# fujii-team/Henbun

Measured on AMD Instinct MI355X. Metric: elbo_samples_per_sec, higher is better.
Workload: dtype f32; 1 GPU; cfg2 SVGP ELBO step: 1-D UnitRBF, N=1e6, M=512 inducing, minibatch 8192 per GPU, diag Normal q(u), diagonal residual, Adam lr 1e-3; global_batch=8192, per_gpu_batch=8192, parallelism=dp1, N=1000000, M=512, dp_exchange=none, dp_ranks=1, contraction=native, tri_pack=False

## Files before the change

### henbun_amd/_lib.py

```python
from __future__ import annotations

import ctypes
import os
from ctypes import c_char_p, c_double, c_int, c_long, c_uint64, c_void_p

_HERE = os.path.dirname(os.path.abspath(__file__))
LIB_PATH = os.path.join(_HERE, "libhenbun_hip.so")


class HipBackendError(RuntimeError):
    """A libhenbun_hip.so entry point returned a non-zero status."""


P, L, I, D, U64 = c_void_p, c_long, c_int, c_double, c_uint64

_SIGS = {
    "hb_version": [],
    "hb_debug_set": [c_char_p, L],
    "hb_debug_clear": [],
    "hb_cholesky_inverse_ws_elems": [L, L, I],
    "hb_cholesky_persistent_shape": [L, L, I],
    "hb_mlp2_sample_supported": [L, L, L, L, L, I],
    "hb_mlp2_sample_ws_elems": [L, L, L],
    "hb_mlp2_sample_fwd_f32": [P, P, P, P, P, I, P, P, L, P, P, P, P, L, L, L, P, P],
    "hb_mlp2_sample_bwd_f32": [P, P, P, P, I, P, P, P, P, P, P, P, P, P, L, L, L, P, P],
    "hb_gram_cholesky_inverse_f32": [I, P, L, P, L, L, L, D, P, P, L, L, P, P, P, I, P],
    "hb_last_error_string": [],
    "hb_device_info": [P, I, P],
    "hb_graph_begin_capture": [P],
    "hb_graph_end_capture": [P, P],
    "hb_graph_launch": [P, P],
    "hb_graph_destroy": [P],
    "hb_rng_init": [P, L, U64, U64, P],
    "hb_rng_randint": [P, L, P, L, L, L, P],
    "hb_sgp_ws_elems": [L, L, L, L, L],
    "hb_sgp_strip_path": [L, L, L, L, L, I],
    "hb_sgp_head_units": [L, L, L, L, L, I, I, I, L],
    "hb_sgp_rider_supported": [L, L, L, L, L, I, I, I, L],
    "hb_sgp_predict_ws_elems": [L, L, L, L, L, I, I, I],
    "hb_sgp_predict_cov_ws_elems": [L, L, L, L, I, I],
    "hb_matmul_gauss_units": [L, L, L],
    "hb_matmul_gram_vjp_ok": [L, L, L, L],
    "hb_matmul_gram_vjp_ws_elems": [L, L, L],
    "hb_matmul_gram_vjp_f32": [P, P, P, L, L, L, L, L, L, L, L, L, I, I, P, L, P, L, L, L, P, P, P, P, P],
    "hb_fullrank_one_launch_shape": [L, L],
    "hb_matmul_gauss_f32": [P, L, P, L, P, P, P, P, D, P, P, P, L, L, L, L, P],
    "hb_sgp_rider_begin": [],
    "hb_sgp_rider_pending": [],
    "hb_sgp_rider_flush": [P],
    "hb_sgp_fwd_gauss_f32": [I, I, P, L, P, P, L, P, P, I, P, P, P, L, P, P, P, P, P, L, L, L, L, L, P, P, P, P, D, P, P, P, L, P],
    "hb_ewise_prog_image_bytes": [],
    "hb_ewise_prog_build": [I, P, P, I, P, P, I, P, P, P, I, P, P, P, P],
    "hb_ewise_jit_available": [],
    "hb_ewise_jit_run": [P, P],
    "hb_ewise_jit_destroy": [P],
    "hb_side_push_gather_draw_f32": [I, P, P, P, L, P, L, L, L, P, P, L, P, P],
    "hb_side_push_diag_fwd_f32": [P, P, P, P, L, P, P, P, L, L, L, L, P, P],
    "hb_side_push_diag_bwd_f32": [P, P, P, P, P, P, P, L, L, L, L, P],
    "hb_side_pending": [],
    "hb_side_flush": [P],
    "hb_side_discard": [],
    "hb_chain_begin": [],
    "hb_chain_end": [P],
    "hb_chain_discard": [],
    "hb_chain_source": [P, L],
    "hb_chain_compile_dry": [],
    "hb_comm_available": [],
    "hb_comm_unique_id": [P],
    "hb_comm_init": [P, I, I, P],
    "hb_comm_destroy": [P],
}
_RESTYPES = {"hb_last_error_string": c_char_p, "hb_sgp_ws_elems": c_long, "hb_ewise_prog_image_bytes": c_long,
             "hb_sgp_head_units": c_long, "hb_matmul_gauss_units": c_long, "hb_matmul_gram_vjp_ws_elems": c_long, "hb_cholesky_inverse_ws_elems": c_long, "hb_mlp2_sample_ws_elems": c_long,
             "hb_sgp_predict_ws_elems": c_long, "hb_sgp_predict_cov_ws_elems": c_long}

_TYPED = {
    "hb_ewise": [I, I, P, P, I, P, I, P, P, P],
    "hb_ewise_prog": [I, P, P, I, P, P, I, P, P, P, I, P, P],
    "hb_ewise_prog_run": [P, L, I, P],
    "hb_ewise_jit_build": [I, P, P, I, P, P, I, P, P, P, I, P, P, P, P, P, L],
    "hb_ewise_colprog_build": [I, P, P, I, P, P, I, P, P, P, L, L, P, P, L],
    "hb_gauss_ll": [P, P, P, P, L, P, P, P, P, P, L, P],
    "hb_gauss_ll_post": [P, P, P, P, L, P, P, P, P, D, P, P, L, P],
    "hb_gauss_ll_fold": [P, L, P, P, P, P],
    "hb_reduce": [I, P, P, L, L, L, P, L, P],
    "hb_copy_nd": [P, P, P, P, I, P, P],
    "hb_fill": [P, L, D, P],
    "hb_gather_rows": [P, L, L, P, P, L, P, P, P],
    "hb_gather_rows_multi": [I, P, P, P, L, P, P, L, P, P],
    "hb_gather_rows_multi_draw": [I, P, P, P, L, P, L, L, L, P, P, L, P, P],
    "hb_matutil": [P, P, L, L, L, I, L, L, D, P],
    "hb_rng_normal": [P, L, P, L, P],
    "hb_diag_sample_kl_fwd": [P, P, P, P, L, P, P, P, L, L, L, L, P, P],
    "hb_diag_sample_kl_bwd": [P, P, P, P, P, P, P, L, L, L, L, P],
    "hb_fullrank_sample_kl_fwd": [P, P, P, P, L, P, P, P, L, L, I, P, P],
    "hb_fullrank_sample_kl_fwd1": [P, P, P, P, L, P, P, P, L, L, I, P, P, P],
    "hb_fullrank_sample_kl_bwd": [P, P, P, P, P, P, P, L, L, I, P],
    "hb_vec_to_tri": [P, P, L, L, P],
    "hb_tri_to_vec": [P, P, L, L, P],
    "hb_gram_fwd": [I, P, L, P, L, P, L, L, P, L, L, L, L, D, P],
    "hb_gram_bwd": [I, P, L, P, L, P, L, L, P, P, P, P, L, L, L, L, P, P],
    "hb_gram_ell_fold": [P, L, L, L, L, P, P],
    "hb_matmul": [P, P, P, L, L, L, L, L, L, L, L, L, L, I, I, D, D, P, L, I, I, P, L, P],
    "hb_matmul_colsum": [P, P, P, P, L, L, L, L, L, L, P, L, P],
    "hb_cholesky": [P, P, L, L, P, P],
    "hb_cholesky_inverse": [P, P, P, L, L, P, P, P, I, P],
    "hb_trinv": [P, P, L, L, P, P],
    "hb_sgp_A": [I, P, L, P, P, L, P, P, I, P, L, L, L, L, P],
    "hb_sgp_fwd": [I, I, P, L, P, P, L, P, P, I, P, P, P, L, P, P, P, P, P, L, L, L, L, L, P, P],
    "hb_sgp_bwd": [I, I, P, L, P, P, L, P, P, I, P, P, P, P, P, P, P, P, P, P, P, P, P, L, L, L, L, L, P, P],
    "hb_sgp_predict": [I, P, L, P, P, L, P, P, P, P, I, I, D, P, P, L, L, L, L, L, P, P],
    "hb_sgp_predict_cov": [I, P, L, P, P, L, P, P, P, I, I, D, P, L, L, L, L, L, P, P],
    "hb_adam_step": [P, P, P, P, L, D, D, D, D, D, P, I, P, L, P, P, P],
    "hb_allreduce_sum": [P, L, P, P],
    "hb_dp_pack": [P, P, P, L, P],
}


def declared_symbols():
    names = list(_SIGS)
    for base in _TYPED:
        names += [base + "_f32", base + "_f64"]
    return names


class _Lib:
    def __init__(self, path: str):
        if not os.path.exists(path):
            raise ImportError(
                "henbun_amd: %s is missing.  Build it with `python -m henbun_amd._build` "
                "(hipcc, gfx950).  There is no CPU fallback." % path
            )
        import torch

        self._dll = ctypes.CDLL(path)
        self._fns = {}
        for name, args in _SIGS.items():
            self._bind(name, args, _RESTYPES.get(name, c_int))
        for base, args in _TYPED.items():
            for suf in ("_f32", "_f64"):
                self._bind(base + suf, args, c_int)
        if self.raw("hb_version")() != 2:
            raise ImportError("henbun_amd: ABI version mismatch in " + path)

    def _bind(self, name, args, restype):
        fn = getattr(self._dll, name)
        fn.argtypes = args
        fn.restype = restype
        self._fns[name] = fn

    def raw(self, name):
        return self._fns[name]

    def last_error(self) -> str:
        s = self._fns["hb_last_error_string"]()
        return s.decode() if s else ""

    def call(self, name, *args):
        rc = self._fns[name](*args)
        if rc != 0:
            raise HipBackendError("%s failed (status %d): %s" % (name, rc, self.last_error()))
        return 0


_lib = None


def lib() -> _Lib:
    global _lib
    if _lib is None:
        _lib = _Lib(LIB_PATH)
    return _lib
```

### henbun_amd/csrc/sgp.hip

```cpp
#include "common.cuh"
#include "sgp_strip.cuh"
#include "chain.cuh"
#include "chol_persist.cuh"
#include <type_traits>
#include "gemm_tile.cuh"
#include "rng_pairs.cuh"
#include "../../include/henbun_hip.h"

#define SGP_BM 64
#define SGP_BN 128
#define SGP_DREG 4

extern "C" int hb_matmul_f32(const float*, const float*, float*, long, long, long, long, long, long, long, long, long,
                             long, int, int, double, double, const float*, long, int, int, float*, long, void*);
extern "C" int hb_matmul_f64(const double*, const double*, double*, long, long, long, long, long, long, long, long,
                             long, long, int, int, double, double, const double*, long, int, int, double*, long,
                             void*);

template <typename T>
struct SgpArgs {
  const T* x;
  long sx;
  const T* z;
  const T* ell;
// ... 540 lines not shown
    const int c = tid & 31, kq = tid >> 5;
    const int cc = col0 + c < n ? col0 + c : n - 1;
    float sc[D], xs[D];
#pragma unroll
    for (int dd = 0; dd < D; ++dd) {
      sc[dd] = float(SGP_EXP2_SCALE) / ell[a.dl == 1 ? 0 : dd];
      xs[dd] = x[cc * D + dd];
    }
    constexpr int NTH = SGP_STRIP_THREADS;
    constexpr int ZIT = (SGP_SM_MAX * D) / NTH, UIT = SGP_SM_MAX / NTH;
    float zt[ZIT], ut[4][UIT];
    const int npu = a.part ? ((int)a.P < 4 ? (int)a.P : 4) : 0;
#pragma unroll
    for (int it = 0; it < ZIT; ++it) {
      const int i = tid + NTH * it;
      zt[it] = z[i < M * D ? i : 0];
    }
#pragma unroll
    for (int p = 0; p < 4; ++p)
#pragma unroll
      for (int it = 0; it < UIT; ++it) {
        const int i = tid + NTH * it;
        ut[p][it] = p < npu ? a.u[e * a.P * a.M + (long)p * M + (i < M ? i : 0)] : 0.f;
      }
#pragma unroll
    for (int it = 0; it < ZIT; ++it) {
      const int i = tid + NTH * it;
      if (i < M * D) zs[i] = zt[it];
    }
#pragma unroll
    for (int p = 0; p < 4; ++p)
#pragma unroll
      for (int it = 0; it < UIT; ++it) {
        const int i = tid + NTH * it;
        if (p < npu && i < M) us[p][i] = ut[p][it];
      }
    __syncthreads();
#pragma unroll 4
    for (int k4 = kq * 4; k4 < M; k4 += NTH / 8) {
      float zq[4 * D];
#pragma unroll
      for (int q = 0; q < 4 * D; q += 4) {
        const V4 zz = *reinterpret_cast<const V4*>(&zs[k4 * D + q]);
#pragma unroll
        for (int s = 0; s < 4; ++s) zq[q + s] = zz[s];
      }
      V4 v;
#pragma unroll
      for (int q = 0; q < 4; ++q) {
        float r2 = 0.f;
#pragma unroll
        for (int dd = 0; dd < D; ++dd) {
          const float tt = (zq[q * D + dd] - xs[dd]) * sc[dd];
          r2 += tt * tt;
        }
        v[q] = hb_exp2_neg<float>(r2);
      }
      *reinterpret_cast<V4*>(&Ks[c][k4]) = v;
    }
  }
  __syncthreads();
  HB_SSTAMP(1);

  const int nT = M / 32;
  const int t1 = nT - 1 - w, t0 = w;
  const int d0 = w < t1 ? w + 1 : 0;
  const int d1 = w <= t1 ? t1 + 1 : 0;
  const int nts = d0 + d1;
  const int npart = a.part ? (int)a.P : 0;
  float cs[5] = {0.f, 0.f, 0.f, 0.f, 0.f};
  const int gc = col0 + li;
  typename MM::Acc acc;
#pragma unroll
  for (int r = 0; r < 16; ++r) acc[r] = 0.f;

  auto load = [&](V4 (&f)[4], int ts) {
    const int tc = ts < nts ? ts : nts - 1;
    const int tile = tc < d0 ? t0 : t1, Q = tc < d0 ? tc : tc - d0;
    const float* p = Wf + ((long)(tile * nT + Q) << 10) + 4 * lane;
#pragma unroll
    for (int v = 0; v < 4; ++v) f[v] = *reinterpret_cast<const V4*>(p + 256 * v);
  };
  auto compute = [&](const V4 (&f)[4], int ts) {
    if (ts >= nts) return;
    const int tile = ts < d0 ? t0 : t1, Q = ts < d0 ? ts : ts - d0;
    V4 bv[4];
#pragma unroll
    for (int v = 0; v < 4; ++v) bv[v] = *reinterpret_cast<const V4*>(&Ks[li][32 * Q + 16 * h + 4 * v]);
#pragma unroll
    for (int v = 0; v < 4; ++v)
#pragma unroll
      for (int s = 0; s < 4; ++s) acc = MM::mma(f[v][s], bv[v][s], acc);
    if (ts == d0 - 1 || ts == nts - 1) {
      if (a.Af) sgp_store_frag_tile(a.Af, Tw[w], acc, e, nT, (n + SGP_SN - 1) / SGP_SN, tile, bx, col0, n, lane);
#pragma unroll
      for (int r = 0; r < 16; ++r) {
        const int row = 32 * tile + MM::acc_row(lane, r);
        const float v = acc[r];
        if (a.A && gc < n) A[(long)row * n + gc] = v;
        if (a.part) {
          cs[0] += v * v;
#pragma unroll
          for (int p = 0; p < 4; ++p)
            if (p < npart) cs[1 + p] += us[p][row] * v;
        }
        acc[r] = 0.f;
      }
    }
  };
  if (nts > 0) {
    V4 fa[4], fb[4];
    load(fa, 0);
#pragma nounroll
    for (int ts = 0; ts < nts; ts += 2) {
      load(fb, ts + 1);
      __builtin_amdgcn_sched_barrier(0);
      compute(fa, ts);
      __builtin_amdgcn_sched_barrier(0);
      load(fa, ts + 2);
      __builtin_amdgcn_sched_barrier(0);
      compute(fb, ts + 1);
      __builtin_amdgcn_sched_barrier(0);
    }
  }
  HB_SSTAMP(2);

  if (a.part) {
#pragma unroll
    for (int q = 0; q < 5; ++q) cs[q] += __shfl_xor(cs[q], 32);
    __syncthreads();
    float* red = &Ks[0][0];
    if (lane < 32) {
#pragma unroll
      for (int q = 0; q < 5; ++q) red[(w * 5 + q) * 32 + lane] = cs[q];
    }
    __syncthreads();
    if (tid < 32 && col0 + tid < n) {
      float* pp = a.part + e * 5 * a.n + col0 + tid;
      for (int q = 0; q < 1 + npart; ++q) {
        float sum = 0.f;
#pragma unroll
        for (int ww = 0; ww < SGP_STRIP_THREADS / 64; ++ww) sum += red[(ww * 5 + q) * 32 + tid];
        pp[(long)q * n] = sum;
      }
    }
  }
  HB_SSTAMP(3);
}

__device__ __forceinline__ float sgp_ag_load(const float* p) {
  return __hip_atomic_load(const_cast<float*>(p), __ATOMIC_RELAXED, __HIP_MEMORY_SCOPE_AGENT);
}

#define SGP_RED_LD 260
template <bool AG, bool L16 = false>
__device__ __forceinline__ void sgp_2t_epilogue(const SgpArgs<float>& a, float* lds_raw, const float (&csq)[16], const float (&cu)[16],
                                                const long e, const int bx, const int col0, const int n, const bool means) {
  typedef float V4 __attribute__((ext_vector_type(4)));
  const int tid = threadIdx.x, lane = tid & 63, w = __builtin_amdgcn_readfirstlane(tid >> 6), li = lane & 31, h = lane >> 5;
  if (a.part) {
    __syncthreads();
    float* red = lds_raw;
    if (L16) {
#pragma unroll
      for (int r = 0; r < 8; ++r) {
        const int c = 16 * (r >> 2) + 4 * (lane >> 4) + (r & 3);
        red[(0 * SGP_SN + c) * SGP_RED_LD + 16 * w + (lane & 15)] = csq[r];
        if (means) red[(1 * SGP_SN + c) * SGP_RED_LD + 16 * w + (lane & 15)] = cu[r];
      }
    } else {
#pragma unroll
      for (int r = 0; r < 16; ++r) {
        const int c = (r & 3) + 8 * (r >> 2) + 4 * h;
        red[(0 * SGP_SN + c) * SGP_RED_LD + 32 * w + li] = csq[r];
        if (means) red[(1 * SGP_SN + c) * SGP_RED_LD + 32 * w + li] = cu[r];
      }
    }
    __syncthreads();
    if (L16 && tid >= 512) return;
    const int pair = tid >> 3, g = tid & 7;
    const float* rp = red + pair * SGP_RED_LD + 32 * g;
    float sum = 0.f;
#pragma unroll
    for (int i = 0; i < 8; ++i) {
      const V4 q = *reinterpret_cast<const V4*>(rp + 4 * i);
      sum += (q[0] + q[1]) + (q[2] + q[3]);
    }
    sum += __shfl_xor(sum, 1);
    sum += __shfl_xor(sum, 2);
    sum += __shfl_xor(sum, 4);
    const int q = pair >> 5, c = pair & 31;
    if (!a.fin) {
      if (g == 0 && col0 + c < n && (q == 0 || means)) a.part[e * 5 * a.n + (long)q * n + col0 + c] = sum;
      return;
    }
    __syncthreads();
    float* tot = lds_raw;
    if (g == 0) tot[q * 32 + c] = (q == 0 || means) ? sum : 0.f;
    __syncthreads();
    float h_ll = 0.f, h_sc = 0.f, h_vr = 0.f;
    if (tid < 16) {
      const long j0 = col0 + 2 * tid;
      if (j0 < n) {
        const long idx0 = e * (long)a.n + j0, pidx = idx0 >> 1;
        float z0 = 0.f, z1 = 0.f;
        if (a.fin_rng) {
          HbRng gen = rng_load(a.fin_rng, a.fin_lanes, pidx);
          gen.normal2(z0, z1);
          rng_store(a.fin_rng, a.fin_lanes, pidx, gen);
        } else if (a.fin_eps_in) {
          z0 = AG ? sgp_ag_load(a.fin_eps_in + idx0) : a.fin_eps_in[idx0];
          z1 = AG ? sgp_ag_load(a.fin_eps_in + idx0 + 1) : a.fin_eps_in[idx0 + 1];
        }
#pragma unroll
        for (int i = 0; i < 2; ++i) {
          const float s2 = 0.f + tot[2 * tid + i];
          const float vv = 1.f - s2;
          const float zi = i ? z1 : z0;
          a.fin_v[idx0 + i] = vv;
          if (a.fin_eps_out && a.fin_eps_out != a.fin_eps_in) a.fin_eps_out[idx0 + i] = zi;
          const float scale = a.fin_diag ? hb_sqrt(hb_abs(vv)) * zi : 0.f;
          const float fj = (0.f + tot[32 + 2 * tid + i]) + scale;
          if (a.P > 0) a.fin_f[(e * a.P) * (long)a.n + j0 + i] = fj;
          if (a.head) {
            const float hs = a.hscale ? a.hscale[0] : 1.f, hv = a.hvar[0];
            const float iv = 1.f / hv, lc = -0.91893853320467274178f - 0.5f * hb_log(hv);
            float gg;
            hb_gauss_point<float>(AG ? sgp_ag_load(a.hy + idx0 + i) : a.hy[idx0 + i], fj, hs, iv, lc, gg, h_ll, h_sc, h_vr);
            a.hdmu[idx0 + i] = gg;
            if (a.hfbar) a.hfbar[idx0 + i] = hs * (a.hpost * gg);
          }
        }
      }
    }
    if (a.head && tid < 64) {
#pragma unroll
      for (int off = 8; off > 0; off >>= 1) {
        h_ll += __shfl_xor(h_ll, off, 16);
        h_sc += __shfl_xor(h_sc, off, 16);
        h_vr += __shfl_xor(h_vr, off, 16);
      }
      if (tid == 0) {
        const long unit = e * (long)((n + SGP_SN - 1) / SGP_SN) + bx;
        a.hpart[unit] = h_ll;
        a.hpart[a.hunits + unit] = h_sc;
        a.hpart[2 * a.hunits + unit] = h_vr;
      }
    }
  }
}

template <int D>
__global__ void __launch_bounds__(SGP_STRIP_THREADS, 4) sgp_A_strip2t_kernel(SgpArgs<float> a) {
  typedef float V4 __attribute__((ext_vector_type(4)));
  typedef Mma<float> MM;
  constexpr int KS_FLOATS = SGP_SN * SGP_SLD, RED_FLOATS = 2 * SGP_SN * SGP_RED_LD;
  __shared__ __attribute__((aligned(16))) float lds_raw[KS_FLOATS > RED_FLOATS ? KS_FLOATS : RED_FLOATS];
  __shared__ __attribute__((aligned(16))) float zs[SGP_SM_MAX * D];
  float (*Ks)[SGP_SLD] = reinterpret_cast<float (*)[SGP_SLD]>(lds_raw);
  long e;
  int bx;
  sgp_block(a.efast, e, bx);
  const float* __restrict__ x = a.x + e * a.sx;
  const float* __restrict__ z = a.z + e * a.M * D;
  const float* __restrict__ ell = a.ell + e * a.dl;
  const float* __restrict__ Wf = a.Wf + e * a.M * a.M;
  float* __restrict__ A = a.A ? a.A + e * a.M * a.n : nullptr;
  const int M = (int)a.M, n = (int)a.n;
  const int col0 = bx * SGP_SN;
  const int tid = threadIdx.x, lane = tid & 63, w = __builtin_amdgcn_readfirstlane(tid >> 6), li = lane & 31, h = lane >> 5;
  const int nT = M / 32;
  const int t1 = nT - 1 - w, t0 = w;
  const int d0 = w < t1 ? w + 1 : 0;
  const int d1 = w <= t1 ? t1 + 1 : 0;
  const int nts = d0 + d1;
  const bool means = a.part && a.P > 0;
  HB_SSTAMP(0);
  float u0 = 0.f, u1 = 0.f;
  if (means) {
    const float* up = a.u + e * a.P * a.M;
    if (d0) u0 = up[32 * t0 + li];
    if (d1) u1 = up[32 * t1 + li];
  }
  {
    const int c = tid & 31, kq = tid >> 5;
    const int cc = col0 + c < n ? col0 + c : n - 1;
    float sc[D], xs[D];
#pragma unroll
    for (int dd = 0; dd < D; ++dd) {
      sc[dd] = float(SGP_EXP2_SCALE) / ell[a.dl == 1 ? 0 : dd];
      xs[dd] = x[cc * D + dd];
    }
    constexpr int NTH = SGP_STRIP_THREADS;
    constexpr int ZIT = (SGP_SM_MAX * D) / NTH;
    float zt[ZIT];
#pragma unroll
    for (int it = 0; it < ZIT; ++it) {
      const int i = tid + NTH * it;
      zt[it] = z[i < M * D ? i : 0];
    }
#pragma unroll
    for (int it = 0; it < ZIT; ++it) {
      const int i = tid + NTH * it;
      if (i < M * D) zs[i] = zt[it];
    }
    __syncthreads();
#pragma unroll 4
    for (int k4 = kq * 4; k4 < M; k4 += NTH / 8) {
      float zq[4 * D];
#pragma unroll
      for (int q = 0; q < 4 * D; q += 4) {
        const V4 zz = *reinterpret_cast<const V4*>(&zs[k4 * D + q]);
#pragma unroll
        for (int s = 0; s < 4; ++s) zq[q + s] = zz[s];
      }
      V4 v;
#pragma unroll
      for (int q = 0; q < 4; ++q) {
        float r2 = 0.f;
#pragma unroll
        for (int dd = 0; dd < D; ++dd) {
          const float tt = (zq[q * D + dd] - xs[dd]) * sc[dd];
          r2 += tt * tt;
        }
        v[q] = hb_exp2_neg<float>(r2);
      }
      *reinterpret_cast<V4*>(&Ks[c][k4]) = v;
    }
  }
  __syncthreads();
  HB_SSTAMP(1);

  float csq[16], cu[16];
#pragma unroll
  for (int r = 0; r < 16; ++r) csq[r] = 0.f, cu[r] = 0.f;
  typename MM::Acc acc;
#pragma unroll
  for (int r = 0; r < 16; ++r) acc[r] = 0.f;
  const int nS = (n + SGP_SN - 1) / SGP_SN;

  auto load = [&](V4 (&f)[4], int ts) {
    const int tc = ts < nts ? ts : nts - 1;
    const int tile = tc < d0 ? t0 : t1, Q = tc < d0 ? tc : tc - d0;
    const float* p = Wf + ((long)(tile * nT + Q) << 10) + 4 * lane;
#pragma unroll
    for (int v = 0; v < 4; ++v) f[v] = *reinterpret_cast<const V4*>(p + 256 * v);
  };
  auto compute = [&](const V4 (&f)[4], int ts) {
    if (ts >= nts) return;
    const int tile = ts < d0 ? t0 : t1, Q = ts < d0 ? ts : ts - d0;
    V4 bv[4];
#pragma unroll
    for (int v = 0; v < 4; ++v) bv[v] = *reinterpret_cast<const V4*>(&Ks[li][32 * Q + 16 * h + 4 * v]);
#pragma unroll
    for (int v = 0; v < 4; ++v)
#pragma unroll
      for (int s = 0; s < 4; ++s) acc = MM::mma(bv[v][s], f[v][s], acc);
    if (ts == d0 - 1 || ts == nts - 1) {
      if (a.part) {
        typedef float V2 __attribute__((ext_vector_type(2)));
        const float um = ts < d0 ? u0 : u1;
        const V2 um2 = {um, um};
#pragma unroll
        for (int r = 0; r < 16; r += 2) {
          const V2 av = {acc[r], acc[r + 1]};
          const V2 q2 = __builtin_elementwise_fma(av, av, V2{csq[r], csq[r + 1]});
          const V2 m2 = __builtin_elementwise_fma(um2, av, V2{cu[r], cu[r + 1]});
          csq[r] = q2[0], csq[r + 1] = q2[1];
          cu[r] = m2[0], cu[r + 1] = m2[1];
        }
      }
      sgp_acc_t_settle(acc);
      float row16[16];
      sgp_acc_t_rows(acc, row16);
      if (a.Af) sgp_store_frag_rows(a.Af, row16, e, nT, nS, tile, bx, col0, n, lane);
      if (A) {
        float* ap = A + (long)(32 * tile + li) * n + col0 + 16 * h;
        if ((n & 3) == 0 && col0 + SGP_SN <= n) {
#pragma unroll
          for (int v = 0; v < 4; ++v) {
            V4 q;
#pragma unroll
            for (int s2 = 0; s2 < 4; ++s2) q[s2] = row16[4 * v + s2];
            *reinterpret_cast<V4*>(ap + 4 * v) = q;
          }
        } else {
#pragma unroll
          for (int i = 0; i < 16; ++i)
            if (col0 + 16 * h + i < n) ap[i] = row16[i];
        }
      }
#pragma unroll
      for (int r = 0; r < 16; ++r) acc[r] = 0.f;
    }
  };
  if (nts > 0) {
    V4 fa[4], fb[4];
    load(fa, 0);
#pragma nounroll
    for (int ts = 0; ts < nts; ts += 2) {
      load(fb, ts + 1);
      __builtin_amdgcn_sched_barrier(0);
      compute(fa, ts);
      __builtin_amdgcn_sched_barrier(0);
      load(fa, ts + 2);
      __builtin_amdgcn_sched_barrier(0);
      compute(fb, ts + 1);
      __builtin_amdgcn_sched_barrier(0);
    }
  }

  HB_SSTAMP(2);
  sgp_2t_epilogue<false>(a, lds_raw, csq, cu, e, bx, col0, n, means);
  HB_SSTAMP(3);
}

#define SGP_S16_THREADS 1024
template <int D>
__global__ void __launch_bounds__(SGP_S16_THREADS, 4) sgp_A_strip16_kernel(SgpArgs<float> a) {
  typedef float V4 __attribute__((ext_vector_type(4)));
  constexpr int KS_FLOATS = SGP_SN * SGP_SLD, RED_FLOATS = 2 * SGP_SN * SGP_RED_LD;
  __shared__ __attribute__((aligned(16))) float lds_raw[KS_FLOATS > RED_FLOATS ? KS_FLOATS : RED_FLOATS];
  __shared__ __attribute__((aligned(16))) float zs[SGP_SM_MAX * D];
  float (*Ks)[SGP_SLD] = reinterpret_cast<float (*)[SGP_SLD]>(lds_raw);
  long e;
  int bx;
  sgp_block(a.efast, e, bx);
  const float* __restrict__ x = a.x + e * a.sx;
  const float* __restrict__ z = a.z + e * a.M * D;
  const float* __restrict__ ell = a.ell + e * a.dl;
  const float* __restrict__ Wf = a.Wf + e * a.M * a.M;
  float* __restrict__ A = a.A ? a.A + e * a.M * a.n : nullptr;
  const int M = (int)a.M, n = (int)a.n;
  const int col0 = bx * SGP_SN;
  const int tid = threadIdx.x, lane = tid & 63, m16 = lane & 15, g4 = lane >> 4;
  const int w = __builtin_amdgcn_readfirstlane(tid >> 6);
  const int nT = M / 32, nS16 = M / 16;
  const bool means = a.part && a.P > 0;
  const int nS = (n + SGP_SN - 1) / SGP_SN;

  {
    const int c = tid & 31, kq = tid >> 5;
    const int cc = col0 + c < n ? col0 + c : n - 1;
    float sc[D], xs[D];
#pragma unroll
    for (int dd = 0; dd < D; ++dd) {
      sc[dd] = float(SGP_EXP2_SCALE) / ell[a.dl == 1 ? 0 : dd];
      xs[dd] = x[cc * D + dd];
    }
    constexpr int NTH = SGP_S16_THREADS;
    for (int i = tid; i < M * D; i += NTH) zs[i] = z[i];
    __syncthreads();
#pragma unroll 4
    for (int k4 = kq * 4; k4 < M; k4 += NTH / 8) {
      float zq[4 * D];
#pragma unroll
      for (int q = 0; q < 4 * D; q += 4) {
        const V4 zz = *reinterpret_cast<const V4*>(&zs[k4 * D + q]);
#pragma unroll
        for (int s2 = 0; s2 < 4; ++s2) zq[q + s2] = zz[s2];
      }
      V4 v;
#pragma unroll
      for (int q = 0; q < 4; ++q) {
        float r2 = 0.f;
#pragma unroll
        for (int dd = 0; dd < D; ++dd) {
          const float tt = (zq[q * D + dd] - xs[dd]) * sc[dd];
          r2 += tt * tt;
        }
        v[q] = hb_exp2_neg<float>(r2);
      }
      *reinterpret_cast<V4*>(&Ks[c][k4]) = v;
    }
  }
  __syncthreads();

  float csq[16], cu[16];
#pragma unroll
  for (int r = 0; r < 16; ++r) csq[r] = 0.f, cu[r] = 0.f;
  V4 acc[2];
  const V4 zero4 = {0.f, 0.f, 0.f, 0.f};
  acc[0] = zero4, acc[1] = zero4;

  auto load = [&](V4 (&f)[2], int s, int Q) {
    const float* p = Wf + ((long)((s >> 1) * nT + Q) << 10) + (g4 * 64 + 16 * (s & 1) + m16) * 4;
    f[0] = *reinterpret_cast<const V4*>(p);
    f[1] = *reinterpret_cast<const V4*>(p + 128);
  };
  auto mma_step = [&](const V4 (&f)[2], int Q) {
    V4 kf[2][2];
#pragma unroll
    for (int jb = 0; jb < 2; ++jb)
#pragma unroll
      for (int b = 0; b < 2; ++b) kf[jb][b] = *reinterpret_cast<const V4*>(&Ks[16 * jb + m16][32 * Q + 16 * b + 4 * g4]);
#pragma unroll
    for (int b = 0; b < 2; ++b)
#pragma unroll
      for (int ee = 0; ee < 4; ++ee) {
        acc[0] = __builtin_amdgcn_mfma_f32_16x16x4f32(kf[0][b][ee], f[b][ee], acc[0], 0, 0, 0);
        acc[1] = __builtin_amdgcn_mfma_f32_16x16x4f32(kf[1][b][ee], f[b][ee], acc[1], 0, 0, 0);
      }
  };
  auto retire = [&](int s) {
    const int T = s >> 1, li = 16 * (s & 1) + m16;
    if (a.part) {
      const float um = means ? (a.u + e * a.P * a.M)[16 * s + m16] : 0.f;
#pragma unroll
      for (int jb = 0; jb < 2; ++jb)
#pragma unroll
        for (int r = 0; r < 4; ++r) {
          csq[4 * jb + r] += acc[jb][r] * acc[jb][r];
          cu[4 * jb + r] += um * acc[jb][r];
        }
    }
#pragma unroll
    for (int jb = 0; jb < 2; ++jb) {
      V4 q = acc[jb];
#pragma unroll
      for (int r = 0; r < 4; ++r)
        if (col0 + 16 * jb + 4 * g4 + r >= n) q[r] = 0.f;
      if (a.Af) *reinterpret_cast<V4*>(a.Af + ((((long)e * nT + T) * nS + bx) << 10) + (g4 * 64 + 32 * jb + li) * 4) = q;
      if (A) {
        float* ap = A + (long)(32 * T + li) * n + col0 + 16 * jb + 4 * g4;
        if ((n & 3) == 0 && col0 + SGP_SN <= n) {
          *reinterpret_cast<V4*>(ap) = q;
        } else {
#pragma unroll
          for (int r = 0; r < 4; ++r)
            if (col0 + 16 * jb + 4 * g4 + r < n) ap[r] = q[r];
        }
      }
    }
    acc[0] = zero4, acc[1] = zero4;
  };
#pragma unroll 1
  for (int pr = w; pr < nS16 / 2; pr += SGP_S16_THREADS / 64) {
    const int s0 = pr, s1 = nS16 - 1 - pr;
    const int d0 = (s0 >> 1) + 1, nts = d0 + (s1 >> 1) + 1;
    auto at = [&](int ts, int& s, int& Q) {
      const int tc = ts < nts ? ts : nts - 1;
      s = tc < d0 ? s0 : s1;
      Q = tc < d0 ? tc : tc - d0;
    };
    V4 fa[2], fb[2];
    int s, Q;
    at(0, s, Q);
    load(fa, s, Q);
#pragma nounroll
    for (int ts = 0; ts < nts; ts += 2) {
      at(ts + 1, s, Q);
      load(fb, s, Q);
      __builtin_amdgcn_sched_barrier(0);
      at(ts, s, Q);
      mma_step(fa, Q);
      if (ts == d0 - 1 || ts == nts - 1) retire(s);
      __builtin_amdgcn_sched_barrier(0);
      at(ts + 2, s, Q);
      load(fa, s, Q);
      __builtin_amdgcn_sched_barrier(0);
      if (ts + 1 < nts) {
        at(ts + 1, s, Q);
        mma_step(fb, Q);
        if (ts + 1 == d0 - 1 || ts + 1 == nts - 1) retire(s);
      }
      __builtin_amdgcn_sched_barrier(0);
    }
// ... 539 lines not shown
      hipLaunchKernelGGL((sgp_A_strip2_kernel<D_>), grid, dim3(SGP_STRIP_THREADS), 0, stream, a);             \
    else                                                                                                      \
      hipLaunchKernelGGL((sgp_A_strip_kernel<D_, false>), grid, dim3(SGP_STRIP_THREADS), 0, stream, a);       \
  } while (0)
  if (a.d == 1)
    HB_STRIP(1);
  else if (a.d == 2)
    HB_STRIP(2);
  else if (a.d == 3)
    HB_STRIP(3);
  else
    HB_STRIP(4);
#undef HB_STRIP
  HB_LAUNCH_CHECK();
  return 0;
}
static int sgp_A_strip_launch(SgpArgs<double>, long, hipStream_t) { return -1; }

template <typename T>
static int sgp_A_launch(const SgpArgs<T>& a, dim3 grid, hipStream_t stream) {
  const bool lds_z = a.d <= SGP_DREG && a.M * a.d <= SGP_ZS_MAX;
  const bool vec = lds_z && a.M % 16 == 0 && ((uintptr_t)a.W % 16 == 0);
#define HB_SGP_A(D_)                                                                          \
  do {                                                                                        \
    if (vec)                                                                                  \
      hipLaunchKernelGGL((sgp_A_kernel<T, D_, true>), grid, dim3(256), 0, stream, a);         \
    else                                                                                      \
      hipLaunchKernelGGL((sgp_A_kernel<T, D_, false>), grid, dim3(256), 0, stream, a);        \
  } while (0)
  if (lds_z && a.d == 1)
    HB_SGP_A(1);
  else if (lds_z && a.d == 2)
    HB_SGP_A(2);
  else if (lds_z && a.d == 3)
    HB_SGP_A(3);
  else if (lds_z && a.d == 4)
    HB_SGP_A(4);
  else
    hipLaunchKernelGGL((sgp_A_kernel<T, 0, false>), grid, dim3(256), 0, stream, a);
#undef HB_SGP_A
  HB_LAUNCH_CHECK();
  return 0;
}

template <typename T>
__global__ void __launch_bounds__(256) sgp_finish_kernel(const T* __restrict__ A, const T* __restrict__ u,
                                                         const T* __restrict__ eps, T* __restrict__ f,
                                                         T* __restrict__ v, long n, long M, long P, int mode) {
  __shared__ T red[5][8][33];
  const long e = blockIdx.y;
  A += e * M * n;
  u += e * P * M;
  f += e * P * n;
  v += e * n;
  if (eps) eps += e * n;
  const int cx = threadIdx.x & 31, ry = threadIdx.x >> 5;
  const long j = (long)blockIdx.x * 32 + cx;
  const bool ok = j < n;
  const long jc = ok ? j : n - 1;
  T scale = T(0);
  for (long p0 = 0; p0 < P || p0 == 0; p0 += 4) {
    const int np = (int)((P - p0) < 4 ? (P - p0) : 4);
    T sq = T(0), mac[4] = {T(0), T(0), T(0), T(0)};
#pragma unroll 4
    for (long m = ry; m < M; m += 8) {
      const T av = A[m * n + jc];
      sq += av * av;
#pragma unroll
      for (int q = 0; q < 4; ++q)
        if (q < np) mac[q] += u[(p0 + q) * M + m] * av;
    }
    red[4][ry][cx] = sq;
#pragma unroll
    for (int q = 0; q < 4; ++q) red[q][ry][cx] = mac[q];
    __syncthreads();
    if (ry == 0 && ok) {
      if (p0 == 0) {
        T ssum = T(0);
#pragma unroll
        for (int q = 0; q < 8; ++q) ssum += red[4][q][cx];
        const T vv = T(1) - ssum;
        v[j] = vv;
        if (mode == HB_SGP_DIAGONAL) scale = hb_sqrt(hb_abs(vv)) * eps[j];
      }
      for (int q = 0; q < np; ++q) {
        T mean = T(0);
#pragma unroll
        for (int w = 0; w < 8; ++w) mean += red[q][w][cx];
        f[(p0 + q) * n + j] = mean + scale;
      }
    }
    __syncthreads();
  }
}

template <typename T>
__global__ void __launch_bounds__(256) sgp_finish_part_kernel(const T* __restrict__ part, int gy,
                                                              const T* __restrict__ eps_in, uint64_t* rng,
                                                              long nlanes, T* __restrict__ eps_out, T* __restrict__ f,
                                                              T* __restrict__ v, long total, long n, long P, int mode) {
  hb_sgp_finish_body<T>(part, gy, eps_in, rng, nlanes, eps_out, f, v, total, n, P, mode == HB_SGP_DIAGONAL,
                        (long)blockIdx.x * blockDim.x + threadIdx.x, (long)gridDim.x * blockDim.x);
}

template <typename T>
__global__ void __launch_bounds__(256) sgp_rng_fill_kernel(uint64_t* state, long nlanes, T* out, long n) {
  const long t = (long)blockIdx.x * blockDim.x + threadIdx.x;
  const long npairs = (n + 1) / 2;
  if (t >= nlanes || t >= npairs) return;
  HbRng g = rng_load(state, nlanes, t);
  for (long p = t; p < npairs; p += nlanes) {
    T z0, z1;
    g.normal2(z0, z1);
    out[2 * p] = (T)z0;
    if (2 * p + 1 < n) out[2 * p + 1] = (T)z1;
  }
  rng_store(state, nlanes, t, g);
}

extern "C" long hb_sgp_ws_elems(long E, long n, long M, long d, long P) {
  (void)P;
  const long gy = (M + SGP_BM - 1) / SGP_BM;
  const long mm = 32 * E * M * M, part = 5 * E * gy * n;
  return E * n + E * M * d + (mm > part ? mm : part);
}

static inline int sgp_grid_y(long E, long n, int nRB) {
  const long paired = (long)hb_cdiv(n, SGP_BN) * ((nRB + 1) / 2) * E;
  return (paired < 384 && nRB > 1) ? nRB : (nRB + 1) / 2;
}

template <typename T>
struct SgpHead {
  const T* y = nullptr;
  const T* scale = nullptr;
  const T* var = nullptr;
  double post = 0.0;
  T* dmu = nullptr;
  T* fbar = nullptr;
  T* part = nullptr;
  long units = 0;
};
static inline bool sgp_fused_finish_ok(long E, long n, long M, long d, long P, int prec, bool has_wfrag, bool draw, long rng_lanes) {
  const bool nofuse = hb_debug_get("sgp_no_fused_finish", 0) != 0 || hb_debug_get("sgp_strip_form2", 0) != 0;
  return !nofuse && has_wfrag && prec == HB_PREC_NATIVE && hb_sgp_strip_path(E, n, M, d, P, prec) && P <= 1 && n % 2 == 0 &&
         (!draw || rng_lanes >= (E * n + 1) / 2);
}
extern "C" long hb_sgp_head_units(long E, long n, long M, long d, long P, int prec, int has_wfrag, int draw, long rng_lanes) {
  if (P != 1 || !sgp_fused_finish_ok(E, n, M, d, P, prec, has_wfrag != 0, draw != 0, rng_lanes)) return 0;
  return E * hb_cdiv(n, SGP_SN);
}

template <typename T>
static int sgp_fwd(int kind, int mode, const T* x, long sx, const T* z, const T* ell, long dl, const T* W, const T* Wf,
                   int prec, const T* u, const T* eps_in, uint64_t* rng, long rng_lanes, T* eps_out, T* A, T* A_frag, T* f,
                   T* v, long E, long n, long M, long d, long P, T* ws, hipStream_t stream, const SgpHead<T>* head = nullptr) {
  HB_REQUIRE(!A_frag || (sizeof(T) == 4 && Wf && ws && hb_sgp_strip_path(E, n, M, d, P, prec)),
             "hb_sgp_fwd: a fragment-major A needs the column-strip form (fp32, Wfrag, hb_sgp_strip_path)");
  if (hb_chain_recording()) {
    const int crc = hb_chain_flush(stream);
    if (crc) return crc;
  }
  HB_REQUIRE(prec == HB_PREC_NATIVE || prec == HB_PREC_BF16X3, "hb_sgp_fwd: unknown precision %d", prec);
  HB_REQUIRE(prec == HB_PREC_NATIVE || (sizeof(T) == 4 && Wf && M % 32 == 0 && M <= SGP_SM_MAX && d <= SGP_DREG && P <= 4 && ws),
             "hb_sgp_fwd: bf16x3 needs fp32, the bf16 images in Wfrag, M %% 32 == 0, M <= %d, d <= %d, P <= 4", SGP_SM_MAX, SGP_DREG);
  HB_REQUIRE(kind == HB_KERN_RBF, "hb_sgp_fwd: only the UnitRBF kernel is fused (kind=%d)", kind);
  HB_REQUIRE(mode == HB_SGP_NEGLECTED || mode == HB_SGP_DIAGONAL, "hb_sgp_fwd: unknown mode %d", mode);
  HB_REQUIRE(E >= 0 && n >= 0 && M >= 0 && d >= 1 && P >= 0, "hb_sgp_fwd: bad extents");
  HB_REQUIRE(dl == 1 || dl == d, "hb_sgp_fwd: lengthscales must have 1 or d entries");
  HB_REQUIRE(x && z && ell && W && u && (A || A_frag) && f && v, "hb_sgp_fwd: NULL pointer");
  HB_REQUIRE(E <= 65535, "hb_sgp_fwd: too many experts");
  HB_REQUIRE(M * n < 2147483647L && M * M < 2147483647L && n * d < 2147483647L, "hb_sgp_fwd: matrix too large for 32-bit indexing");
  if (E * n == 0) return 0;
  const bool draw = mode == HB_SGP_DIAGONAL && !eps_in;
  if (draw) HB_REQUIRE(rng && rng_lanes > 0 && eps_out, "hb_sgp_fwd: need eps_in, or rng and eps_out");
  HB_REQUIRE(!head || (M > 0 && P == 1 && ws && Wf), "hb_sgp_fwd_gauss: needs Wfrag, a workspace and P == 1");
  const int nRB = hb_cdiv(M, SGP_BM);
  const int gy = sgp_grid_y(E, n, nRB);
  if (M > 0 && P <= 4 && ws) {
    SgpArgs<T> a;
    a.x = x; a.sx = sx; a.z = z; a.ell = ell; a.dl = dl; a.W = W; a.Wf = Wf; a.u = u; a.A = A;
    a.n = n; a.M = M; a.d = d; a.P = P;
    a.W3 = prec == HB_PREC_BF16X3 ? (const void*)(Wf + 2 * E * M * M) : nullptr;
    a.plane3 = E * M * M;
    a.Af = A_frag;
    a.part = ws + E * n + E * M * d;
    const bool strip = sizeof(T) == 4 && ((Wf && hb_sgp_strip_path(E, n, M, d, P, prec)) ||
                                          (sgp_strip_ok(E, n, M, d, W) && !hb_sgp_no_strip()));
    const int gyp = strip ? 1 : gy;
    int rc;
    a.fin = 0;
    if (strip) {
      if (sizeof(T) == 4 && sgp_fused_finish_ok(E, n, M, d, P, prec, a.Wf != nullptr && !a.W3, draw, rng_lanes)) {
        a.fin = 1;
        a.fin_diag = mode == HB_SGP_DIAGONAL;
        a.fin_eps_in = mode == HB_SGP_DIAGONAL ? eps_in : (const T*)nullptr;
        a.fin_rng = draw ? rng : (uint64_t*)nullptr;
        a.fin_lanes = rng_lanes;
        a.fin_eps_out = mode == HB_SGP_DIAGONAL ? eps_out : (T*)nullptr;
        a.fin_f = f;
        a.fin_v = v;
        if (head) {
          HB_REQUIRE(P == 1 && head->units == E * hb_cdiv(n, SGP_SN), "hb_sgp_fwd_gauss: units must be hb_sgp_head_units(...)");
          a.head = 1;
          a.hy = head->y, a.hscale = head->scale, a.hvar = head->var;
          a.hdmu = head->dmu, a.hfbar = head->fbar, a.hpost = (T)head->post;
          a.hpart = head->part, a.hunits = head->units;
        }
      }
      HB_REQUIRE(!head || a.fin, "hb_sgp_fwd_gauss: this call cannot carry the head (hb_sgp_head_units(...) == 0)");
      if constexpr (std::is_same<T, float>::value) {
        if (g_rider.armed) {
          HB_REQUIRE(a.fin && !a.W3 && d <= SGP_E_DMAX, "hb_sgp_fwd after hb_sgp_rider_begin: this call cannot ride (hb_sgp_rider_supported)");
          sgp_grid(hb_cdiv(a.n, SGP_SN), 1, E, a.efast);
          g_rider.a = a, g_rider.E = E, g_rider.valid = true, g_rider.armed = false;
          return 0;
        }
      }
      rc = sgp_A_strip_launch(a, E, stream);
      if (rc) return rc;
      if (a.fin) return 0;
    } else {
      dim3 grid = sgp_grid(hb_cdiv(n, SGP_BN), gy, E, a.efast);
      rc = sgp_A_launch<T>(a, grid, stream);
    }
    if (rc) return rc;
    const long total = E * n;
    if (hb_chain_recording() && total <= HB_CHAIN_FINISH_MAX_N) {
      HbChainJob j;
      j.kind = HB_CHAIN_SGP_FINISH;
      j.is64 = sizeof(T) == 8;
      j.p[0] = a.part;
      j.p[1] = mode == HB_SGP_DIAGONAL ? eps_in : (const T*)nullptr;
      j.p[2] = draw ? rng : (uint64_t*)nullptr;
      j.p[3] = mode == HB_SGP_DIAGONAL ? eps_out : (T*)nullptr;
      j.p[4] = f;
      j.p[5] = v;
      j.l[0] = gyp, j.l[1] = rng_lanes, j.l[2] = total, j.l[3] = n, j.l[4] = P, j.l[5] = mode == HB_SGP_DIAGONAL;
      return hb_chain_push(j, stream);
    }
    const int fgrid = draw ? hb_cdiv(rng_lanes, 256) : hb_stream_grid((total + 1) / 2, 256);
    hipLaunchKernelGGL(sgp_finish_part_kernel<T>, dim3(fgrid), dim3(256), 0, stream, a.part, gyp,
                       mode == HB_SGP_DIAGONAL ? eps_in : (const T*)nullptr, draw ? rng : (uint64_t*)nullptr, rng_lanes,
                       mode == HB_SGP_DIAGONAL ? eps_out : (T*)nullptr, f, v, total, n, P, mode);
    HB_LAUNCH_CHECK();
    return 0;
  }
  const T* eps = eps_in;
  if (mode == HB_SGP_DIAGONAL) {
    if (draw) {
      hipLaunchKernelGGL(sgp_rng_fill_kernel<T>, dim3(hb_cdiv(rng_lanes, 256)), dim3(256), 0, stream, rng, rng_lanes,
                         eps_out, E * n);
      HB_LAUNCH_CHECK();
      eps = eps_out;
    } else if (eps_out && eps_out != eps_in) {
      HB_HIP(hb_copy_async(eps_out, eps_in, sizeof(T) * E * n, stream));
    }
  }
  if (M > 0) {
    SgpArgs<T> a;
    a.x = x; a.sx = sx; a.z = z; a.ell = ell; a.dl = dl; a.W = W; a.Wf = nullptr; a.u = u; a.A = A;
    a.n = n; a.M = M; a.d = d; a.P = P;
    a.W3 = nullptr; a.plane3 = 0; a.Af = nullptr;
    a.part = nullptr;
    dim3 grid = sgp_grid(hb_cdiv(n, SGP_BN), gy, E, a.efast);
    int rc = sgp_A_launch<T>(a, grid, stream);
    if (rc) return rc;
  }
  hipLaunchKernelGGL(sgp_finish_kernel<T>, dim3(hb_cdiv(n, 32), (unsigned)E), dim3(256), 0, stream, A, u, eps, f, v, n,
                     M, P, mode);
  HB_LAUNCH_CHECK();
  return 0;
}

template <typename T>
static int sgp_A_only(int kind, const T* x, long sx, const T* z, const T* ell, long dl, const T* W, const T* Wf, int prec,
                      T* A, long E, long n, long M, long d, hipStream_t stream) {
  HB_REQUIRE(prec == HB_PREC_NATIVE || prec == HB_PREC_BF16X3, "hb_sgp_A: unknown precision %d", prec);
  HB_REQUIRE(prec == HB_PREC_NATIVE || (sizeof(T) == 4 && Wf && M % 32 == 0 && M <= SGP_SM_MAX && d <= SGP_DREG),
             "hb_sgp_A: bf16x3 needs fp32, the bf16 images in Wfrag, M %% 32 == 0, M <= %d, d <= %d", SGP_SM_MAX, SGP_DREG);
  HB_REQUIRE(kind == HB_KERN_RBF, "hb_sgp_A: only the UnitRBF kernel is fused (kind=%d)", kind);
  HB_REQUIRE(E >= 0 && n >= 0 && M >= 0 && d >= 1, "hb_sgp_A: bad extents");
  HB_REQUIRE(dl == 1 || dl == d, "hb_sgp_A: lengthscales must have 1 or d entries");
  HB_REQUIRE(x && z && ell && W && A, "hb_sgp_A: NULL pointer");
  HB_REQUIRE(E <= 65535, "hb_sgp_A: too many experts");
  HB_REQUIRE(M * n < 2147483647L && M * M < 2147483647L && n * d < 2147483647L, "hb_sgp_A: matrix too large");
  if (E * n * M == 0) return 0;
  SgpArgs<T> a;
  a.x = x; a.sx = sx; a.z = z; a.ell = ell; a.dl = dl; a.W = W; a.Wf = Wf; a.u = nullptr; a.A = A;
  a.n = n; a.M = M; a.d = d; a.P = 0;
  a.W3 = prec == HB_PREC_BF16X3 ? (const void*)(Wf + 2 * E * M * M) : nullptr;
  a.plane3 = E * M * M;
  a.Af = nullptr;
  a.part = nullptr;
  if (sizeof(T) == 4 && ((sgp_strip_ok(E, n, M, d, W) && !hb_sgp_no_strip()) || prec == HB_PREC_BF16X3))
    return sgp_A_strip_launch(a, E, stream);
  const int nRB = hb_cdiv(M, SGP_BM);
  dim3 grid = sgp_grid(hb_cdiv(n, SGP_BN), sgp_grid_y(E, n, nRB), E, a.efast);
  return sgp_A_launch<T>(a, grid, stream);
}
extern "C" int hb_sgp_A_f32(int kind, const float* x, long sx, const float* z, const float* ell, long dl,
                            const float* W, const float* Wfrag, int prec, float* A, long E, long n, long M, long d,
                            void* stream) {
  return sgp_A_only<float>(kind, x, sx, z, ell, dl, W, Wfrag, prec, A, E, n, M, d, (hipStream_t)stream);
}
extern "C" int hb_sgp_A_f64(int kind, const double* x, long sx, const double* z, const double* ell, long dl,
                            const double* W, const double* Wfrag, int prec, double* A, long E, long n, long M, long d,
                            void* stream) {
  return sgp_A_only<double>(kind, x, sx, z, ell, dl, W, Wfrag, prec, A, E, n, M, d, (hipStream_t)stream);
}

extern "C" int hb_sgp_fwd_f32(int kind, int mode, const float* x, long sx, const float* z, const float* ell, long dl,
                              const float* W, const float* Wfrag, int prec, const float* u, const float* eps_in,
                              uint64_t* rng, long rng_lanes, float* eps_out, float* A, float* A_frag, float* f, float* v,
                              long E, long n, long M, long d, long P, float* ws, void* stream) {
  return sgp_fwd<float>(kind, mode, x, sx, z, ell, dl, W, Wfrag, prec, u, eps_in, rng, rng_lanes, eps_out, A, A_frag, f, v,
                        E, n, M, d, P, ws, (hipStream_t)stream);
}
extern "C" int hb_sgp_fwd_f64(int kind, int mode, const double* x, long sx, const double* z, const double* ell,
                              long dl, const double* W, const double* Wfrag, int prec, const double* u,
                              const double* eps_in, uint64_t* rng, long rng_lanes, double* eps_out, double* A,
                              double* A_frag, double* f, double* v, long E, long n, long M, long d, long P, double* ws,
                              void* stream) {
  return sgp_fwd<double>(kind, mode, x, sx, z, ell, dl, W, Wfrag, prec, u, eps_in, rng, rng_lanes, eps_out, A, A_frag, f,
                         v, E, n, M, d, P, ws, (hipStream_t)stream);
}

extern "C" int hb_sgp_fwd_gauss_f32(int kind, int mode, const float* x, long sx, const float* z, const float* ell, long dl,
                                    const float* W, const float* Wfrag, int prec, const float* u, const float* eps_in,
                                    uint64_t* rng, long rng_lanes, float* eps_out, float* A, float* A_frag, float* f, float* v,
                                    long E, long n, long M, long d, long P, float* ws, const float* y, const float* scale,
                                    const float* var, double post, float* dmu, float* fbar, float* head_part, long units,
                                    void* stream) {
  HB_REQUIRE(y && var && dmu && head_part && units > 0, "hb_sgp_fwd_gauss: NULL pointer");
  SgpHead<float> h;
  h.y = y, h.scale = scale, h.var = var, h.post = post, h.dmu = dmu, h.fbar = fbar, h.part = head_part, h.units = units;
  return sgp_fwd<float>(kind, mode, x, sx, z, ell, dl, W, Wfrag, prec, u, eps_in, rng, rng_lanes, eps_out, A, A_frag, f, v,
                        E, n, M, d, P, ws, (hipStream_t)stream, &h);
}

template <typename T>
__device__ __forceinline__ T sgp_resid_coef(const T* __restrict__ eps, const T* __restrict__ v,
                                            const T* __restrict__ fbar, long n, long P, int mode, long j) {
  if (mode != HB_SGP_DIAGONAL) return T(0);
  T cs = T(0);
  for (long p = 0; p < P; ++p) cs += fbar[p * n + j];
  const T vv = v[j];
  const T av = hb_abs(vv);
  return av > T(0) ? -eps[j] * hb_sign(vv) / hb_sqrt(av) * cs : T(0);
}

template <typename T>
struct SgpBwdArgs {
  const T* W;
  const T* u;
  const T* A;
  const T* fbar;
  const T* eps;
  const T* v;
  T* Kbar;
  long n, M, P;
  int mode;
  long efast;
  const T* x;
  long sx;
  const T* z;
  const T* ell;
  long dl, d;
  const T* WTf;
  const void* WT3;
  long plane3;
  T* part;
  const T* Af;
  T* Kf;
};

template <typename T>
struct SgpRawB {
  T a, u;
};
template <typename T>
struct SgpRawB4 {
  typedef T VT __attribute__((ext_vector_type(16 / sizeof(T))));
  VT a;
  T u;
};

template <typename T, bool FAST>
__global__ void __launch_bounds__(256) sgp_kbar_kernel(SgpBwdArgs<T> a) {
  typedef TileGemm<T, SGP_BM, SGP_BN, 16, 2, 2> G;
  __shared__ __attribute__((aligned(16))) T lds[G::LDS_ELEMS];
  long e;
  int bx;
  sgp_block(a.efast, e, bx);
  const T* W = a.W + e * a.M * a.M;
  const T* u = a.u + e * a.P * a.M;
  const T* A = a.A + e * a.M * a.n;
  const T* fbar = a.fbar + e * a.P * a.n;
  const T* eps = a.eps ? a.eps + e * a.n : nullptr;
  const T* vres = a.v + e * a.n;
  T* Kbar = a.Kbar + e * a.M * a.n;
  const int M = (int)a.M, n = (int)a.n;
  const int col0 = bx * SGP_BN;
  const int nRB = (M + SGP_BM - 1) / SGP_BM;
  const int jcol = col0 + (threadIdx.x % SGP_BN);
  const bool jok = jcol < n;
  const int jc = jok ? jcol : n - 1;
  const int Mm1 = M - 1;
  const T cj = sgp_resid_coef<T>(eps, vres, fbar, a.n, a.P, a.mode, jc);
  const bool preg = a.P == 1;
  const T fb0 = a.P > 0 ? fbar[jc] : T(0);
  constexpr int VECK = TileGemm<T, SGP_BM, SGP_BN, 16, 2, 2>::VEC;
  const int n4 = col0 + (threadIdx.x % (SGP_BN / VECK)) * VECK;
  const int n4c = n4 + VECK <= n ? n4 : (n >= VECK ? n - VECK : 0);
  T c4[VECK], f4[VECK];
#pragma unroll
  for (int q = 0; q < VECK; ++q) {
    const bool ok = FAST && (n4 + q < n);
    c4[q] = ok ? sgp_resid_coef<T>(eps, vres, fbar, a.n, a.P, a.mode, n4 + q) : T(0);
    f4[q] = ok ? fbar[n4 + q] : T(0);
  }

  for (int half = 0; half < 2; ++half) {
    int rb;
    if (!sgp_row_block(half, nRB, rb)) break;
    const int row0 = rb * SGP_BM;
    G g;
    g.zero();
    auto la = [&](int m, int k) -> T {
      const int r = row0 + m;
      return W[k * M + (r < M ? r : Mm1)];
    };
    auto fa = [&](T raw, int m, int k) -> T {
      const int r = row0 + m;
      return ((r < M) & (k >= r)) ? raw : T(0);
    };
    auto lb = [&](int k, int nn) -> SgpRawB<T> {
      SgpRawB<T> r;
      r.a = A[k * n + jc];
      r.u = u[k];
      return r;
    };
    auto fb = [&](SgpRawB<T> raw, int k, int nn) -> T {
      T val = raw.a * cj;
      if (preg) {
        val += raw.u * fb0;
      } else {
        for (long p = 0; p < a.P; ++p) val += u[p * M + k] * fbar[p * n + jc];
      }
      return jok ? val : T(0);
    };
    if constexpr (FAST) {
      typedef typename G::VT VT;
      constexpr int VEC = G::VEC;
      auto la4 = [&](int m, int k) -> VT {
        const int r = row0 + m;
        return *reinterpret_cast<const VT*>(&W[k * M + (r < M ? r : M - VEC)]);
      };
      auto fa4 = [&](VT raw, int m, int k) -> VT {
        VT v;
#pragma unroll
        for (int q = 0; q < VEC; ++q) v[q] = ((row0 + m + q < M) & (k >= row0 + m + q)) ? raw[q] : T(0);
        return v;
      };
      auto lb4 = [&](int k, int nn) -> SgpRawB4<T> {
        SgpRawB4<T> r;
        r.a = *reinterpret_cast<const typename SgpRawB4<T>::VT*>(&A[k * n + n4c]);
        r.u = u[k];
        return r;
      };
      auto fb4 = [&](SgpRawB4<T> raw, int k, int nn) -> VT {
        VT v;
#pragma unroll
        for (int q = 0; q < VEC; ++q) v[q] = raw.a[q] * c4[q] + raw.u * f4[q];
        return v;
      };
      g.template run_vec<HB_MC, HB_MC>(row0, M, la4, fa4, lb4, fb4, lds);
    } else {
      g.template run<false, false>(row0, M, la, fa, lb, fb, lds);
    }
    g.for_each([&](int row, int col, T v) {
      const int r = row0 + row, cc = col0 + col;
      if (r < M && cc < n) Kbar[(long)r * n + cc] = v;
    });
  }
}

__device__ __forceinline__ float hb_half_wave_sum_dpp(float v) {
  auto dpp = [](float x, int ctrl_unused) { return x; };
  (void)dpp;
  int vi;
#define HB_DPP_ADD(CTRL, ROWMASK)                                                                        \
  vi = __builtin_amdgcn_update_dpp(0, __builtin_bit_cast(int, v), CTRL, ROWMASK, 0xF, true);             \
  v += __builtin_bit_cast(float, vi);
  HB_DPP_ADD(0xB1, 0xF)
  HB_DPP_ADD(0x4E, 0xF)
  HB_DPP_ADD(0x141, 0xF)
  HB_DPP_ADD(0x140, 0xF)
  HB_DPP_ADD(0x142, 0xA)
#undef HB_DPP_ADD
  return v;
}

template <int D, bool BF3>
__global__ void __launch_bounds__(SGP_STRIP_THREADS, (BF3 || D >= 3) ? 2 : 4) sgp_kbar_strip_kernel(SgpBwdArgs<float> a) {
  typedef float V4 __attribute__((ext_vector_type(4)));
  typedef __bf16 B8 __attribute__((ext_vector_type(8)));
  typedef Mma<float> MM;
  constexpr int KS_BYTES = BF3 ? 3 * SGP_SN * SGP_S3LD * 2 : SGP_SN * SGP_SLD * 4;
  __shared__ __attribute__((aligned(16))) unsigned char ks_raw[KS_BYTES];
  __shared__ float lred[(SGP_STRIP_THREADS / 64) * D];
  __shared__ __attribute__((aligned(16))) float zs[SGP_SM_MAX * D];
  __shared__ __attribute__((aligned(16))) float xss[SGP_SN * D];
  __shared__ float us[4][SGP_SM_MAX];
  __shared__ float cjs[SGP_SN], fbs[4][SGP_SN];
  float (*Ks)[SGP_SLD] = reinterpret_cast<float (*)[SGP_SLD]>(ks_raw);
  __bf16 (*K3)[SGP_SN][SGP_S3LD] = reinterpret_cast<__bf16 (*)[SGP_SN][SGP_S3LD]>(ks_raw);
  long e;
  int bx;
  sgp_block(a.efast, e, bx);
  const float* __restrict__ x = a.x + e * a.sx;
  const float* __restrict__ z = a.z + e * a.M * D;
  const float* __restrict__ ell = a.ell + e * a.dl;
  const float* __restrict__ A = a.A ? a.A + e * a.M * a.n : nullptr;
  const float* __restrict__ fbar = a.fbar + e * a.P * a.n;
  float* __restrict__ Kbar = a.Kbar ? a.Kbar + e * a.M * a.n : nullptr;
  const int M = (int)a.M, n = (int)a.n, P = (int)a.P;
  const int col0 = bx * SGP_SN, nS = (n + SGP_SN - 1) / SGP_SN;
  const int tid = threadIdx.x, lane = tid & 63, w = __builtin_amdgcn_readfirstlane(tid >> 6), li = lane & 31, h = lane >> 5;
  const int nq = 2 * D + P;
  float* __restrict__ part = a.part + ((e * nS + bx) * (long)nq) * M;

  float sc[D];
#pragma unroll
  for (int dd = 0; dd < D; ++dd) sc[dd] = float(SGP_EXP2_SCALE) / ell[a.dl == 1 ? 0 : dd];
  {
    constexpr int NTH = SGP_STRIP_THREADS;
    constexpr int ZIT = (SGP_SM_MAX * D) / NTH, UIT = SGP_SM_MAX / NTH;
    float zt[ZIT], ut[4][UIT];
#pragma unroll
    for (int it = 0; it < ZIT; ++it) {
      const int i = tid + NTH * it;
      zt[it] = z[i < M * D ? i : 0];
    }
#pragma unroll
    for (int p = 0; p < 4; ++p)
#pragma unroll
      for (int it = 0; it < UIT; ++it) {
        const int i = tid + NTH * it;
        ut[p][it] = p < P ? a.u[e * a.P * a.M + (long)p * M + (i < M ? i : 0)] : 0.f;
      }
    if (tid < SGP_SN) {
      const int cc = col0 + tid;
      const bool ok = cc < n;
      const int cj = ok ? cc : n - 1;
      cjs[tid] = ok ? sgp_resid_coef<float>(a.eps ? a.eps + e * a.n : nullptr, a.v + e * a.n, fbar, a.n, a.P, a.mode, cj) : 0.f;
#pragma unroll
      for (int p = 0; p < 4; ++p) fbs[p][tid] = (ok && p < P) ? fbar[(long)p * n + cj] : 0.f;
#pragma unroll
      for (int dd = 0; dd < D; ++dd) xss[tid * D + dd] = x[cj * D + dd];
    }
#pragma unroll
    for (int it = 0; it < ZIT; ++it) {
      const int i = tid + NTH * it;
      if (i < M * D) zs[i] = zt[it];
    }
#pragma unroll
    for (int p = 0; p < 4; ++p)
#pragma unroll
      for (int it = 0; it < UIT; ++it) {
        const int i = tid + NTH * it;
        if (p < P && i < M) us[p][i] = ut[p][it];
      }
  }
  __syncthreads();

  if (a.Af) {
    const int nTp = M / 32;
    const long fplane = (long)a.plane3 / a.M * 32 * nS;
    for (int t = w; t < nTp; t += SGP_STRIP_THREADS / 64) {
      float avals[16];
      if (BF3) {
        const __bf16* blk = reinterpret_cast<const __bf16*>(a.Af) + ((((long)e * nTp + t) * nS + bx) << 10) + 8 * lane;
        B8 pl[3][2];
#pragma unroll
        for (int p = 0; p < 3; ++p)
#pragma unroll
          for (int q = 0; q < 2; ++q) pl[p][q] = *reinterpret_cast<const B8*>(blk + p * fplane + 512 * q);
#pragma unroll
        for (int q = 0; q < 2; ++q)
#pragma unroll
          for (int j = 0; j < 8; ++j) avals[8 * q + j] = ((float)pl[2][q][j] + (float)pl[1][q][j]) + (float)pl[0][q][j];
      } else {
        const float* blk = a.Af + ((((long)e * nTp + t) * nS + bx) << 10) + 4 * lane;
        V4 av[4];
#pragma unroll
        for (int v = 0; v < 4; ++v) av[v] = *reinterpret_cast<const V4*>(blk + 256 * v);
#pragma unroll
        for (int v = 0; v < 4; ++v)
#pragma unroll
          for (int s2 = 0; s2 < 4; ++s2) avals[4 * v + s2] = av[v][s2];
      }
      const int k = 32 * t + li;
      float uk[4], usum[4] = {0.f, 0.f, 0.f, 0.f};
#pragma unroll
      for (int p = 0; p < 4; ++p) uk[p] = p < P ? us[p][k] : 0.f;
#pragma unroll
      for (int v = 0; v < 4; ++v) {
        const V4 cj4 = *reinterpret_cast<const V4*>(&cjs[16 * h + 4 * v]);
        V4 fb4[4];
#pragma unroll
        for (int p = 0; p < 4; ++p) fb4[p] = *reinterpret_cast<const V4*>(&fbs[p][16 * h + 4 * v]);
#pragma unroll
        for (int s2 = 0; s2 < 4; ++s2) {
          const int c = 16 * h + 4 * v + s2;
          const float aval = avals[4 * v + s2];
          float val = aval * cj4[s2];
#pragma unroll
          for (int p = 0; p < 4; ++p)
            if (p < P) {
              val += uk[p] * fb4[p][s2];
              usum[p] += fb4[p][s2] * aval;
            }
          if (BF3) {
            const __bf16 b0 = (__bf16)val;
            const float r1 = val - (float)b0;
            const __bf16 b1 = (__bf16)r1;
            K3[0][c][k] = b0, K3[1][c][k] = b1, K3[2][c][k] = (__bf16)(r1 - (float)b1);
          } else {
            Ks[c][k] = val;
          }
        }
      }
#pragma unroll
      for (int p = 0; p < 4; ++p)
        if (p < P) {
          const float tsum = usum[p] + __shfl_xor(usum[p], 32);
          if (h == 0) part[(long)(2 * D + p) * M + k] = tsum;
        }
    }
  } else {
    constexpr int G = BF3 ? 8 : 4;
    const int c = tid & 31, kq = tid >> 5;
    const bool cok = col0 + c < n;
    const int cc = cok ? col0 + c : n - 1;
    const float cj = cjs[c];
    float fb[4];
#pragma unroll
    for (int p = 0; p < 4; ++p) fb[p] = fbs[p][c];
    constexpr int NG = SGP_SM_MAX / (16 * G);
    float av[NG][G];
#pragma unroll
    for (int it = 0; it < NG; ++it)
#pragma unroll
      for (int i = 0; i < G; ++i) {
        const int k = G * (kq + 16 * it) + i;
// ... 63 lines not shown
    sgp_acc_t_settle(acc);
    float kb[16];
    sgp_acc_t_rows(acc, kb);
    if (col0 + SGP_SN > n) {
#pragma unroll
      for (int i = 0; i < 16; ++i)
        if (col0 + 16 * h + i >= n) kb[i] = 0.f;
    }
    if (a.Kbar) {
      float* kp = Kbar + (long)(32 * tile + li) * n + col0 + 16 * h;
      if ((n & 3) == 0 && col0 + SGP_SN <= n) {
#pragma unroll
        for (int v = 0; v < 4; ++v) {
          V4 q;
#pragma unroll
          for (int s2 = 0; s2 < 4; ++s2) q[s2] = kb[4 * v + s2];
          *reinterpret_cast<V4*>(kp + 4 * v) = q;
        }
      } else {
#pragma unroll
        for (int i = 0; i < 16; ++i)
          if (col0 + 16 * h + i < n) kp[i] = kb[i];
      }
    }
    if (a.Kf && !BF3) sgp_store_frag_rows(a.Kf, kb, e, nT, nS, tile, bx, col0, n, lane);
    if (BF3 && a.Kf)
      sgp_store_frag3_row(reinterpret_cast<__bf16*>(a.Kf), (long)a.plane3 / a.M * 32 * nS, kb, e, nT, nS, tile, bx, lane);
    const int row = 32 * tile + li;
    float zr[D], zacc[D], lacc[D];
#pragma unroll
    for (int dd = 0; dd < D; ++dd) zr[dd] = zs[row * D + dd], zacc[dd] = 0.f, lacc[dd] = 0.f;
#pragma unroll
    for (int i = 0; i < 16; ++i) {
      const int c = 16 * h + i;
      float tt[D], r2 = 0.f;
#pragma unroll
      for (int dd = 0; dd < D; ++dd) {
        tt[dd] = (zr[dd] - xss[c * D + dd]) * sc[dd];
        r2 += tt[dd] * tt[dd];
      }
      const float gk = kb[i] * hb_exp2_neg<float>(r2);
#pragma unroll
      for (int dd = 0; dd < D; ++dd) {
        zacc[dd] -= gk * tt[dd];
        lacc[dd] += gk * tt[dd] * tt[dd];
      }
    }
#pragma unroll
    for (int dd = 0; dd < D; ++dd) {
      zacc[dd] += __shfl_xor(zacc[dd], 32);
      if (h == 0) part[(long)dd * M + row] = zacc[dd] * sc[dd] * float(1.0 / (SGP_EXP2_SCALE * SGP_EXP2_SCALE));
      lwave[dd] += lacc[dd];
    }
#pragma unroll
    for (int r = 0; r < 16; ++r) acc[r] = 0.f;
  };

  if (!BF3) {
    const float* __restrict__ Wf = a.WTf + e * a.M * a.M;
    auto load = [&](V4 (&f)[4], int ts) {
      const int tc = ts < nts ? ts : nts - 1;
      const float* p = Wf + ((long)(tile_of(tc) * nT + chunk_of(tc)) << 10) + 4 * lane;
#pragma unroll
      for (int v = 0; v < 4; ++v) f[v] = *reinterpret_cast<const V4*>(p + 256 * v);
    };
    auto compute = [&](const V4 (&f)[4], int ts) {
      if (ts >= nts) return;
      const int Q = chunk_of(ts);
      V4 bv[4];
#pragma unroll
      for (int v = 0; v < 4; ++v) bv[v] = *reinterpret_cast<const V4*>(&Ks[li][32 * Q + 16 * h + 4 * v]);
#pragma unroll
      for (int v = 0; v < 4; ++v)
#pragma unroll
        for (int s2 = 0; s2 < 4; ++s2) acc = MM::mma(bv[v][s2], f[v][s2], acc);
      if (ts == d0 - 1 || ts == nts - 1) retire(tile_of(ts));
    };
    if (nts > 0) {
      V4 fa[4], fb2[4];
      load(fa, 0);
#pragma nounroll
      for (int ts = 0; ts < nts; ts += 2) {
        load(fb2, ts + 1);
        __builtin_amdgcn_sched_barrier(0);
        compute(fa, ts);
        __builtin_amdgcn_sched_barrier(0);
        load(fa, ts + 2);
        __builtin_amdgcn_sched_barrier(0);
        compute(fb2, ts + 1);
        __builtin_amdgcn_sched_barrier(0);
      }
    }
  } else {
    const __bf16* __restrict__ W3 = reinterpret_cast<const __bf16*>(a.WT3) + e * a.M * a.M;
    struct Frag {
      B8 f[3][2];
    };
    auto load = [&](Frag& fr, int ts) {
      const int tc = ts < nts ? ts : nts - 1;
      const __bf16* p = W3 + ((long)(tile_of(tc) * nT + chunk_of(tc)) << 10) + 8 * lane;
#pragma unroll
      for (int t = 0; t < 3; ++t)
#pragma unroll
        for (int q = 0; q < 2; ++q) fr.f[t][q] = *reinterpret_cast<const B8*>(p + (long)t * a.plane3 + 512 * q);
    };
    auto compute = [&](const Frag& fr, int ts) {
      if (ts >= nts) return;
      const int Q = chunk_of(ts);
#pragma unroll
      for (int q = 0; q < 2; ++q) {
        B8 b[3];
#pragma unroll
        for (int t = 0; t < 3; ++t) b[t] = *reinterpret_cast<const B8*>(&K3[t][li][32 * Q + 16 * q + 8 * h]);
        acc = __builtin_amdgcn_mfma_f32_32x32x16_bf16(b[0], fr.f[2][q], acc, 0, 0, 0);
        acc = __builtin_amdgcn_mfma_f32_32x32x16_bf16(b[2], fr.f[0][q], acc, 0, 0, 0);
        acc = __builtin_amdgcn_mfma_f32_32x32x16_bf16(b[1], fr.f[1][q], acc, 0, 0, 0);
        acc = __builtin_amdgcn_mfma_f32_32x32x16_bf16(b[0], fr.f[1][q], acc, 0, 0, 0);
        acc = __builtin_amdgcn_mfma_f32_32x32x16_bf16(b[1], fr.f[0][q], acc, 0, 0, 0);
        acc = __builtin_amdgcn_mfma_f32_32x32x16_bf16(b[0], fr.f[0][q], acc, 0, 0, 0);
      }
      if (ts == d0 - 1 || ts == nts - 1) retire(tile_of(ts));
    };
    if (nts > 0) {
      Frag fa, fb2;
      load(fa, 0);
#pragma nounroll
      for (int ts = 0; ts < nts; ts += 2) {
        load(fb2, ts + 1);
        __builtin_amdgcn_sched_barrier(0);
        compute(fa, ts);
        __builtin_amdgcn_sched_barrier(0);
        load(fa, ts + 2);
        __builtin_amdgcn_sched_barrier(0);
        compute(fb2, ts + 1);
        __builtin_amdgcn_sched_barrier(0);
      }
    }
  }
  __syncthreads();
  float* red = lred;
#pragma unroll
  for (int dd = 0; dd < D; ++dd) {
    const float t = wave_sum(lwave[dd]);
    if (lane == 0) red[w * D + dd] = t;
  }
  __syncthreads();
#pragma unroll
  for (int dd = 0; dd < D; ++dd)
    if (tid == dd) {
      float t = 0.f;
      for (int ww = 0; ww < SGP_STRIP_THREADS / 64; ++ww) t += red[ww * D + dd];
      part[(long)(D + dd) * M] = t * sc[dd] * float(1.0 / (SGP_EXP2_SCALE * SGP_EXP2_SCALE * SGP_EXP2_SCALE));
    }
}

#ifndef HB_LSTAMP
#define HB_LSTAMP(i)
#endif
template <bool BF3>
__global__ void __launch_bounds__(256) sgp_lbar_frag_kernel(const float* __restrict__ Kf, const float* __restrict__ Af,
                                                            float* __restrict__ slabs, int M, int nS, int S, long E,
                                                            int pairs) {
  typedef __bf16 B8 __attribute__((ext_vector_type(8)));
  typedef float V4 __attribute__((ext_vector_type(4)));
  typedef Mma<float> MM;
  __shared__ float red[4][32][33];
  const int nT = M / 32, nB = (nT + 1) / 2;
  const int U = gridDim.x, xcd = blockIdx.x & 7, kx = blockIdx.x >> 3;
  const int uq = U >> 3, ur = U & 7;
  const int unit = xcd * uq + (xcd < ur ? xcd : ur) + kx;
  const int group = unit / pairs, pair = unit - group * pairs;
  const int slab = group % S;
  const long e = group / S;
  int bi = (int)((sqrtf(8.f * (float)pair + 1.f) - 1.f) * 0.5f);
  while (bi * (bi + 1) / 2 > pair) --bi;
  while ((bi + 1) * (bi + 2) / 2 <= pair) ++bi;
  const int bj = pair - bi * (bi + 1) / 2;
  (void)nB;
  const int tid = threadIdx.x, lane = tid & 63, w = __builtin_amdgcn_readfirstlane(tid >> 6);
  const int base = nS / S, rem = nS % S;
  const int sb = slab * base + (slab < rem ? slab : rem), se = sb + base + (slab < rem ? 1 : 0);
  const int cnt = se - sb, wq = cnt / 4, wr = cnt % 4;
  const int s0 = sb + w * wq + (w < wr ? w : wr), s1 = s0 + wq + (w < wr ? 1 : 0);
  const int ti0 = 2 * bi, ti1 = 2 * bi + 1 < nT ? 2 * bi + 1 : ti0, tj0 = 2 * bj, tj1 = 2 * bj + 1 < nT ? 2 * bj + 1 : tj0;
  const bool has_i1 = 2 * bi + 1 < nT, has_j1 = 2 * bj + 1 < nT;
  const bool upper01 = bi == bj;
  const long tstride = (long)nS << 10;
  const float* __restrict__ kbase = Kf + (long)e * nT * tstride + 4 * lane;
  const float* __restrict__ abase = Af + (long)e * nT * tstride + 4 * lane;
  HB_LSTAMP(0);
  typename MM::Acc acc[4];
#pragma unroll
  for (int q = 0; q < 4; ++q)
#pragma unroll
    for (int r = 0; r < 16; ++r) acc[q][r] = 0.f;
  if (!BF3) {
    struct Frag {
      V4 a0[4], a1[4], b0[4], b1[4];
    };
    auto load = [&](Frag& f, int sidx) {
      const int sc = sidx < s1 ? sidx : (s1 > s0 ? s1 - 1 : s0);
      const long off = (long)sc << 10;
#pragma unroll
      for (int v = 0; v < 4; ++v) {
        f.a0[v] = *reinterpret_cast<const V4*>(kbase + ti0 * tstride + off + 256 * v);
        f.a1[v] = *reinterpret_cast<const V4*>(kbase + ti1 * tstride + off + 256 * v);
        f.b0[v] = *reinterpret_cast<const V4*>(abase + tj0 * tstride + off + 256 * v);
        f.b1[v] = *reinterpret_cast<const V4*>(abase + tj1 * tstride + off + 256 * v);
      }
    };
    auto compute = [&](const Frag& f, int sidx) {
      if (sidx >= s1) return;
#pragma unroll
      for (int v = 0; v < 4; ++v)
#pragma unroll
        for (int s2 = 0; s2 < 4; ++s2) {
          acc[0] = MM::mma(f.a0[v][s2], f.b0[v][s2], acc[0]);
          acc[2] = MM::mma(f.a1[v][s2], f.b0[v][s2], acc[2]);
          acc[3] = MM::mma(f.a1[v][s2], f.b1[v][s2], acc[3]);
        }
      if (!upper01) {
#pragma unroll
        for (int v = 0; v < 4; ++v)
#pragma unroll
          for (int s2 = 0; s2 < 4; ++s2) acc[1] = MM::mma(f.a0[v][s2], f.b1[v][s2], acc[1]);
      }
    };
    if (s1 > s0) {
      Frag fa, fb;
      load(fa, s0);
#pragma nounroll
      for (int sidx = s0; sidx < s1; sidx += 2) {
        load(fb, sidx + 1);
        __builtin_amdgcn_sched_barrier(0);
        compute(fa, sidx);
        __builtin_amdgcn_sched_barrier(0);
        load(fa, sidx + 2);
        __builtin_amdgcn_sched_barrier(0);
        compute(fb, sidx + 1);
        __builtin_amdgcn_sched_barrier(0);
      }
    }
  } else {
    const long plane = (long)E * nT * tstride;
    const __bf16* __restrict__ k3 = reinterpret_cast<const __bf16*>(Kf) + (long)e * nT * tstride + 8 * lane;
    const __bf16* __restrict__ a3 = reinterpret_cast<const __bf16*>(Af) + (long)e * nT * tstride + 8 * lane;
    struct Frag3 {
      B8 a0[3][2], a1[3][2], b0[3][2], b1[3][2];
    };
    auto load = [&](Frag3& f, int sidx) {
      const int sc = sidx < s1 ? sidx : (s1 > s0 ? s1 - 1 : s0);
      const long off = (long)sc << 10;
#pragma unroll
      for (int p = 0; p < 3; ++p)
#pragma unroll
        for (int q = 0; q < 2; ++q) {
          f.a0[p][q] = *reinterpret_cast<const B8*>(k3 + p * plane + ti0 * tstride + off + 512 * q);
          f.a1[p][q] = *reinterpret_cast<const B8*>(k3 + p * plane + ti1 * tstride + off + 512 * q);
          f.b0[p][q] = *reinterpret_cast<const B8*>(a3 + p * plane + tj0 * tstride + off + 512 * q);
          f.b1[p][q] = *reinterpret_cast<const B8*>(a3 + p * plane + tj1 * tstride + off + 512 * q);
        }
    };
    auto six = [&](const B8 (&x)[3][2], const B8 (&y)[3][2], int q, typename MM::Acc c) {
      c = __builtin_amdgcn_mfma_f32_32x32x16_bf16(x[2][q], y[0][q], c, 0, 0, 0);
      c = __builtin_amdgcn_mfma_f32_32x32x16_bf16(x[0][q], y[2][q], c, 0, 0, 0);
      c = __builtin_amdgcn_mfma_f32_32x32x16_bf16(x[1][q], y[1][q], c, 0, 0, 0);
      c = __builtin_amdgcn_mfma_f32_32x32x16_bf16(x[1][q], y[0][q], c, 0, 0, 0);
      c = __builtin_amdgcn_mfma_f32_32x32x16_bf16(x[0][q], y[1][q], c, 0, 0, 0);
      c = __builtin_amdgcn_mfma_f32_32x32x16_bf16(x[0][q], y[0][q], c, 0, 0, 0);
      return c;
    };
    auto compute = [&](const Frag3& f, int sidx) {
      if (sidx >= s1) return;
#pragma unroll
      for (int q = 0; q < 2; ++q) {
        acc[0] = six(f.a0, f.b0, q, acc[0]);
        acc[2] = six(f.a1, f.b0, q, acc[2]);
        acc[3] = six(f.a1, f.b1, q, acc[3]);
        if (!upper01) acc[1] = six(f.a0, f.b1, q, acc[1]);
      }
    };
    if (s1 > s0) {
      Frag3 fa, fb;
      load(fa, s0);
#pragma nounroll
      for (int sidx = s0; sidx < s1; sidx += 2) {
        load(fb, sidx + 1);
        __builtin_amdgcn_sched_barrier(0);
        compute(fa, sidx);
        __builtin_amdgcn_sched_barrier(0);
        load(fa, sidx + 2);
        __builtin_amdgcn_sched_barrier(0);
        compute(fb, sidx + 1);
        __builtin_amdgcn_sched_barrier(0);
      }
    }
  }
  HB_LSTAMP(1);
  float* out = slabs + (((long)slab * E + e) * M) * M;
#pragma unroll
  for (int q = 0; q < 4; ++q) {
    const int ti = (q >> 1) ? ti1 : ti0, tj = (q & 1) ? tj1 : tj0;
    const bool live = ((q >> 1) == 0 || has_i1) && ((q & 1) == 0 || has_j1) && !(q == 1 && upper01);
    if (!live) continue;
#pragma unroll
    for (int r = 0; r < 16; ++r) red[w][MM::acc_row(lane, r)][lane & 31] = acc[q][r];
// ... 306 lines not shown
  }
  T uacc[4] = {T(0), T(0), T(0), T(0)};
  T zacc[D], lacc[D];
#pragma unroll
  for (int q = 0; q < D; ++q) zacc[q] = lacc[q] = T(0);
  const long ngroups = n / VEC;
#pragma unroll 4
  for (long g = threadIdx.x; g < ngroups; g += 256) {
    const long j0 = g * VEC;
    const VT av = *reinterpret_cast<const VT*>(A + j0);
    const VT kv = *reinterpret_cast<const VT*>(Kbar + j0);
    T xq[VEC][D];
    if (D == 1) {
      const VT xv = *reinterpret_cast<const VT*>(x + j0);
#pragma unroll
      for (int c = 0; c < VEC; ++c) xq[c][0] = xv[c];
    } else {
#pragma unroll
      for (int c = 0; c < VEC; ++c)
#pragma unroll
        for (int q = 0; q < D; ++q) xq[c][q] = x[(j0 + c) * D + q];
    }
#pragma unroll
    for (int p = 0; p < 4; ++p)
      if (p < np) {
        const VT fv = *reinterpret_cast<const VT*>(fbar + p * n + j0);
#pragma unroll
        for (int c = 0; c < VEC; ++c) uacc[p] += fv[c] * av[c];
      }
#pragma unroll
    for (int c = 0; c < VEC; ++c) {
      T tt[D], r2 = T(0);
#pragma unroll
      for (int q = 0; q < D; ++q) {
        tt[q] = zm[q] - xq[c][q] * il[q];
        r2 += tt[q] * tt[q];
      }
      const T gk = kv[c] * hb_exp_fast<T>(T(-0.5) * r2);
#pragma unroll
      for (int q = 0; q < D; ++q) {
        zacc[q] -= gk * tt[q];
        lacc[q] += gk * tt[q] * tt[q];
      }
    }
  }
  for (int p = 0; p < np; ++p) {
    const T us = block_sum(uacc[p], smem);
    if (threadIdx.x == 0) ubar[(e * P + p) * M + m] = us;
  }
#pragma unroll
  for (int q = 0; q < D; ++q) {
    const T zs = block_sum(zacc[q], smem) * il[q];
    const T ls = block_sum(lacc[q], smem) * il[q];
    if (threadIdx.x == 0) {
      zbar[(e * M + m) * D + q] = zs;
      ellpart[(e * M + m) * D + q] = ls;
    }
  }
}

template <typename T>
__global__ void __launch_bounds__(256) sgp_ell_finish_kernel(const T* __restrict__ part, long M, long d, long dl,
                                                             T* __restrict__ ellbar) {
  __shared__ T smem[16];
  const long e = blockIdx.y, c = blockIdx.x;
  part += e * M * d;
  T acc = T(0);
  if (dl == 1) {
#pragma unroll 4
    for (long t = threadIdx.x; t < M * d; t += blockDim.x) acc += part[t];
  } else {
#pragma unroll 4
    for (long m = threadIdx.x; m < M; m += blockDim.x) acc += part[m * d + c];
  }
  acc = block_sum(acc, smem);
  if (threadIdx.x == 0) ellbar[e * dl + c] = acc;
}

template <typename T>
__global__ void __launch_bounds__(256) sgp_xbar_kernel(const T* __restrict__ x, long sx, const T* __restrict__ z,
                                                       const T* __restrict__ ell, long dl, const T* __restrict__ Kbar,
                                                       T* __restrict__ xbar, long n, long M, long d) {
  const long e = blockIdx.y;
  x += e * sx;
  z += e * M * d;
  ell += e * dl;
  Kbar += e * M * n;
  xbar += e * n * d;
  const long j = (long)blockIdx.x * blockDim.x + threadIdx.x;
  if (j >= n) return;
  const T* xj = x + j * d;
  for (long q0 = 0; q0 < d; q0 += SGP_DREG) {
    T acc[SGP_DREG];
#pragma unroll
    for (int q = 0; q < SGP_DREG; ++q) acc[q] = T(0);
    for (long m = 0; m < M; ++m) {
      const T* zm = z + m * d;
      T r2 = T(0);
      for (long q = 0; q < d; ++q) {
        const T t = (zm[q] - xj[q]) / ell[dl == 1 ? 0 : q];
        r2 += t * t;
      }
      const T gk = Kbar[m * n + j] * hb_exp(T(-0.5) * r2);
#pragma unroll
      for (int q = 0; q < SGP_DREG; ++q) {
        if (q0 + q < d) {
          const T il = T(1) / ell[dl == 1 ? 0 : q0 + q];
          acc[q] += gk * (zm[q0 + q] - xj[q0 + q]) * il * il;
        }
      }
    }
#pragma unroll
    for (int q = 0; q < SGP_DREG; ++q)
      if (q0 + q < d) xbar[j * d + q0 + q] = acc[q];
  }
}

static inline int sgp_matmul(const float* A, const float* B, float* C, long batch, long M, long N, long K, long lda,
                             long ldb, long ldc, long sA, long sB, long sC, int tA, int tB, double alpha, int flags,
                             float* ws, long wse, void* stream) {
  return hb_matmul_f32(A, B, C, batch, M, N, K, lda, ldb, ldc, sA, sB, sC, tA, tB, alpha, 0.0, nullptr, 0, HB_ACT_NONE,
                       flags, ws, wse, stream);
}
static inline int sgp_matmul(const double* A, const double* B, double* C, long batch, long M, long N, long K, long lda,
                             long ldb, long ldc, long sA, long sB, long sC, int tA, int tB, double alpha, int flags,
                             double* ws, long wse, void* stream) {
  return hb_matmul_f64(A, B, C, batch, M, N, K, lda, ldb, ldc, sA, sB, sC, tA, tB, alpha, 0.0, nullptr, 0, HB_ACT_NONE,
                       flags, ws, wse, stream);
}

static int sgp_bwd_strip_launch(SgpBwdArgs<float> a, long E, long nS, hipStream_t stream) {
  dim3 grid = sgp_grid(nS, 1, E, a.efast);
#define HB_KBS(D_)                                                                                               \
  do {                                                                                                           \
    if (a.WT3)                                                                                                   \
      hipLaunchKernelGGL((sgp_kbar_strip_kernel<D_, true>), grid, dim3(SGP_STRIP_THREADS), 0, stream, a);        \
    else                                                                                                         \
      hipLaunchKernelGGL((sgp_kbar_strip_kernel<D_, false>), grid, dim3(SGP_STRIP_THREADS), 0, stream, a);       \
  } while (0)
  if (a.d == 1)
    HB_KBS(1);
  else if (a.d == 2)
    HB_KBS(2);
  else if (a.d == 3)
    HB_KBS(3);
  else
    HB_KBS(4);
#undef HB_KBS
  HB_LAUNCH_CHECK();
  return 0;
}
static int sgp_bwd_strip_launch(SgpBwdArgs<double>, long, long, hipStream_t) { return -1; }

static int sgp_lbar_frag_launch(const float* Kf, const float* Af, float* slabs, long slab_cap, long E, long M, long nS,
                                int prec, int* S_out, hipStream_t stream) {
  const int nT = (int)(M / 32);
  const long nB = (nT + 1) / 2, pairs = nB * (nB + 1) / 2;
  long S = 256 / (pairs * E);
  if (S < 1) S = hb_cdiv(2048, pairs * E);
  if (S > nS / 8) S = nS / 8;
  if (S > slab_cap) S = slab_cap;
  if (S < 1) S = 1;
  {
    const long fs = hb_debug_get("lbar_force_s", 0);
    if (fs) S = fs;
  }
  {
    const bool nolds = hb_debug_get("lbar_no_lds", 0) != 0;
    const long nB2 = (nT + 3) / 4, pairs2 = nB2 * (nB2 + 1) / 2;
    if (prec != HB_PREC_BF16X3 && !nolds && pairs * E >= 256 && nS >= 64) {
      long S2 = 512 / (pairs2 * E);
      if (S2 > nS / 8) S2 = nS / 8;
      if (S2 > slab_cap) S2 = slab_cap;
      if (S2 >= 1) {
        dim3 grid2((unsigned)(pairs2 * S2 * E), 1, 1);
        hipLaunchKernelGGL(sgp_lbar_lds_kernel, grid2, dim3(256), 0, stream, Kf, Af, slabs, (int)M, (int)nS, (int)S2, E, (int)pairs2);
        HB_LAUNCH_CHECK();
        *S_out = (int)S2;
        return 0;
      }
    }
  }
  dim3 grid((unsigned)(pairs * S * E), 1, 1);
  if (prec == HB_PREC_BF16X3)
    hipLaunchKernelGGL(sgp_lbar_frag_kernel<true>, grid, dim3(256), 0, stream, Kf, Af, slabs, (int)M, (int)nS, (int)S, E,
                       (int)pairs);
  else
    hipLaunchKernelGGL(sgp_lbar_frag_kernel<false>, grid, dim3(256), 0, stream, Kf, Af, slabs, (int)M, (int)nS, (int)S, E,
                       (int)pairs);
  HB_LAUNCH_CHECK();
  *S_out = (int)S;
  return 0;
}
static int sgp_lbar_frag_launch(const double*, const double*, double*, long, long, long, long, int, int*, hipStream_t) { return -1; }

template <typename T>
static int sgp_bwd(int kind, int mode, const T* x, long sx, const T* z, const T* ell, long dl, const T* W,
                   const T* Wfrag, int prec, const T* u, const T* eps, const T* A, const T* A_frag, const T* v,
                   const T* fbar, T* Kbar, T* Kbar_frag, T* Lbar, T* ubar, T* zbar, T* ellbar, T* xbar, long E, long n,
                   long M, long d, long P, T* ws, hipStream_t stream) {
  HB_REQUIRE(prec == HB_PREC_NATIVE || prec == HB_PREC_BF16X3, "hb_sgp_bwd: unknown precision %d", prec);
  HB_REQUIRE(kind == HB_KERN_RBF, "hb_sgp_bwd: only the UnitRBF kernel is fused (kind=%d)", kind);
  HB_REQUIRE(mode == HB_SGP_NEGLECTED || mode == HB_SGP_DIAGONAL, "hb_sgp_bwd: unknown mode %d", mode);
  HB_REQUIRE(E >= 0 && n >= 0 && M >= 0 && d >= 1 && P >= 0, "hb_sgp_bwd: bad extents");
  HB_REQUIRE(dl == 1 || dl == d, "hb_sgp_bwd: lengthscales must have 1 or d entries");
  HB_REQUIRE(x && z && ell && W && u && (A || A_frag) && v && fbar && (Kbar || Kbar_frag) && Lbar && ubar && zbar && ellbar && ws,
             "hb_sgp_bwd: NULL pointer");
  HB_REQUIRE((A_frag != nullptr) == (Kbar_frag != nullptr), "hb_sgp_bwd: A_frag and Kbar_frag go together");
  HB_REQUIRE(mode == HB_SGP_NEGLECTED || eps, "hb_sgp_bwd: eps required for the diagonal mode");
  HB_REQUIRE(E <= 65535, "hb_sgp_bwd: too many experts");
  HB_REQUIRE(M * n < 2147483647L && M * M < 2147483647L && n * d < 2147483647L, "hb_sgp_bwd: matrix too large for 32-bit indexing");
  if (E * M == 0) return 0;
  T* ellpart = ws + E * n;
  T* mmws = ellpart + E * M * d;
  const long mmws_elems = 32 * E * M * M;
  const long nS = hb_cdiv(n, SGP_SN);
  const bool strip = sizeof(T) == 4 && Wfrag && !xbar && hb_sgp_strip_path(E, n, M, d, P, prec) &&
                     nS * (2 * d + P) * M * E <= mmws_elems;
  HB_REQUIRE(!A_frag || strip, "hb_sgp_bwd: fragment-major A / Kbar need the column-strip form (see hb_sgp_strip_path)");
  HB_REQUIRE(strip || (A && Kbar), "hb_sgp_bwd: row-major A and Kbar required outside the column-strip form");
  HB_REQUIRE(prec == HB_PREC_NATIVE || strip, "hb_sgp_bwd: bf16x3 needs the column-strip form (fp32, Wfrag, M %% 32 == 0, M <= %d, "
             "d <= %d, P <= 4, no xbar)", SGP_SM_MAX, SGP_DREG);
  if (strip) {
    SgpBwdArgs<T> a;
    a.W = W; a.u = u; a.A = A; a.fbar = fbar; a.eps = eps; a.v = v; a.Kbar = Kbar;
    a.n = n; a.M = M; a.P = P; a.mode = mode;
    a.x = x; a.sx = sx; a.z = z; a.ell = ell; a.dl = dl; a.d = d;
    a.WTf = Wfrag + E * M * M;
    a.WT3 = prec == HB_PREC_BF16X3 ? (const void*)(reinterpret_cast<const unsigned short*>(Wfrag + 2 * E * M * M) + 3 * E * M * M)
                                   : nullptr;
    a.plane3 = E * M * M;
    a.part = mmws;
    a.Af = A_frag; a.Kf = Kbar_frag;
    if (A_frag) a.Kbar = nullptr;
    int rc = sgp_bwd_strip_launch(a, E, nS, stream);
    if (rc) return rc;
    if (A_frag) {
      const long npart = ((nS * (2 * d + P) * M * E + 63) / 64) * 64;
      const long slab_cap = (mmws_elems - npart) / (E * M * M);
      HB_REQUIRE(slab_cap >= 1, "hb_sgp_bwd: workspace too small for the Lbar slabs");
      int S = 0;
      rc = sgp_lbar_frag_launch(Kbar_frag, A_frag, mmws + npart, slab_cap > 32 ? 32 : slab_cap, E, M, nS, prec, &S, stream);
      if (rc) return rc;
      const int nbx = (int)hb_cdiv(M, 64), nb_strip = nbx * (int)(2 * d + P) * (int)E;
      hipLaunchKernelGGL(sgp_bwd_finish_kernel<T>, dim3((unsigned)(nb_strip + hb_stream_grid(E * M * M, 256))), dim3(256), 0, stream,
                         mmws, (int)nS, M, d, dl, P, zbar, ellbar, ubar, nb_strip, nbx, mmws + npart, S, E, Lbar);
      HB_LAUNCH_CHECK();
      return 0;
    }
    hipLaunchKernelGGL(sgp_strip_finish_kernel<T>, dim3((unsigned)hb_cdiv(M, 64), (unsigned)(2 * d + P), (unsigned)E), dim3(256), 0,
                       stream, mmws, (int)nS, M, d, dl, P, zbar, ellbar, ubar);
    HB_LAUNCH_CHECK();
    int rc2 = sgp_matmul(Kbar, A, Lbar, E, M, M, n, n, n, M, M * n, M * n, M * M, 0, 1, -1.0, HB_MM_TRIL_OUT, mmws, mmws_elems,
                         (void*)stream);
    return rc2;
  }
  if (n > 0) {
    SgpBwdArgs<T> a;
    a.W = W; a.u = u; a.A = A; a.fbar = fbar; a.eps = eps; a.v = v; a.Kbar = Kbar;
    a.n = n; a.M = M; a.P = P; a.mode = mode;
    a.x = nullptr; a.sx = 0; a.z = nullptr; a.ell = nullptr; a.dl = 0; a.d = d; a.WTf = nullptr; a.WT3 = nullptr;
    a.plane3 = 0; a.part = nullptr; a.Af = nullptr; a.Kf = nullptr;
    const int nRB = hb_cdiv(M, SGP_BM);
    dim3 grid = sgp_grid(hb_cdiv(n, SGP_BN), sgp_grid_y(E, n, nRB), E, a.efast);
    constexpr long VECH = 16 / sizeof(T);
    const bool vec = P == 1 && M % 16 == 0 && n % VECH == 0 && ((uintptr_t)W % 16 == 0) && ((uintptr_t)A % 16 == 0);
    if (vec)
      hipLaunchKernelGGL((sgp_kbar_kernel<T, true>), grid, dim3(256), 0, stream, a);
    else
      hipLaunchKernelGGL((sgp_kbar_kernel<T, false>), grid, dim3(256), 0, stream, a);
    HB_LAUNCH_CHECK();
  }
  {
    constexpr long VECR = 16 / sizeof(T);
    const bool rvec = d <= SGP_DREG && P <= 4 && n > 0 && n % VECR == 0 && ((uintptr_t)A % 16 == 0) &&
                      ((uintptr_t)Kbar % 16 == 0) && ((uintptr_t)fbar % 16 == 0) && ((uintptr_t)x % 16 == 0) &&
                      (sx * (long)sizeof(T)) % 16 == 0;
    dim3 rgrid((unsigned)M, (unsigned)E);
#define HB_SGP_ROWGRAD(D_)                                                                                           \
  hipLaunchKernelGGL((sgp_rowgrad_vec_kernel<T, D_>), rgrid, dim3(256), 0, stream, x, sx, z, ell, dl, Kbar, A, fbar, \
                     zbar, ellpart, ubar, n, M, P)
    if (rvec && d == 1)
      HB_SGP_ROWGRAD(1);
    else if (rvec && d == 2)
      HB_SGP_ROWGRAD(2);
    else if (rvec && d == 3)
      HB_SGP_ROWGRAD(3);
    else if (rvec && d == 4)
      HB_SGP_ROWGRAD(4);
    else
      hipLaunchKernelGGL(sgp_rowgrad_kernel<T>, rgrid, dim3(256), 0, stream, x, sx, z, ell, dl, Kbar, A, fbar, zbar,
                         ellpart, ubar, n, M, d, P);
#undef HB_SGP_ROWGRAD
  }
  HB_LAUNCH_CHECK();
  hipLaunchKernelGGL(sgp_ell_finish_kernel<T>, dim3((unsigned)dl, (unsigned)E), dim3(256), 0, stream, ellpart, M, d, dl,
                     ellbar);
  HB_LAUNCH_CHECK();
  if (xbar && n > 0) {
    hipLaunchKernelGGL(sgp_xbar_kernel<T>, dim3(hb_cdiv(n, 256), (unsigned)E), dim3(256), 0, stream, x, sx, z, ell, dl,
                       Kbar, xbar, n, M, d);
    HB_LAUNCH_CHECK();
  }
  if (n > 0) {
    int rc = sgp_matmul(Kbar, A, Lbar, E, M, M, n, n, n, M, M * n, M * n, M * M, 0, 1, -1.0, HB_MM_TRIL_OUT, mmws,
                        mmws_elems, (void*)stream);
    if (rc) return rc;
  } else {
    HB_HIP(hb_zero_async(Lbar, sizeof(T) * E * M * M, stream));
  }
  return 0;
}

extern "C" int hb_sgp_bwd_f32(int kind, int mode, const float* x, long sx, const float* z, const float* ell, long dl,
                              const float* W, const float* Wfrag, int prec, const float* u, const float* eps,
                              const float* A, const float* A_frag, const float* v, const float* fbar, float* Kbar,
                              float* Kbar_frag, float* Lbar, float* ubar, float* zbar, float* ellbar, float* xbar, long E,
                              long n, long M, long d, long P, float* ws, void* stream) {
  return sgp_bwd<float>(kind, mode, x, sx, z, ell, dl, W, Wfrag, prec, u, eps, A, A_frag, v, fbar, Kbar, Kbar_frag, Lbar,
                        ubar, zbar, ellbar, xbar, E, n, M, d, P, ws, (hipStream_t)stream);
}
extern "C" int hb_sgp_bwd_f64(int kind, int mode, const double* x, long sx, const double* z, const double* ell,
                              long dl, const double* W, const double* Wfrag, int prec, const double* u, const double* eps,
                              const double* A, const double* A_frag, const double* v, const double* fbar, double* Kbar,
                              double* Kbar_frag, double* Lbar, double* ubar, double* zbar, double* ellbar, double* xbar,
                              long E, long n, long M, long d, long P, double* ws, void* stream) {
  return sgp_bwd<double>(kind, mode, x, sx, z, ell, dl, W, Wfrag, prec, u, eps, A, A_frag, v, fbar, Kbar, Kbar_frag, Lbar,
                         ubar, zbar, ellbar, xbar, E, n, M, d, P, ws, (hipStream_t)stream);
}
```

### henbun_amd/graph.py

```python
from __future__ import annotations

import itertools
import math
from typing import Dict, List, Optional, Sequence, Tuple

import numpy as np

from ._lib import HipBackendError as _HipBackendError

_uid = itertools.count()



class Node:
    __slots__ = ("op", "inputs", "attrs", "outputs", "id")

    def __init__(self, op, inputs, attrs, out_shapes):
        self.op = op
        self.inputs = tuple(inputs)
        self.attrs = attrs
        self.id = next(_uid)
        self.outputs = [Tensor(self, i, tuple(int(d) for d in s)) for i, s in enumerate(out_shapes)]


# ... 1443 lines not shown
    plan.buf(node.inputs[0]), plan.out(node.outputs[0])), lambda node, gs: [None if gs[0] is None else tri_to_vec(gs[0])])
defop("tri_to_vec", lambda plan, node: (lambda a, o: plan.steps.append(lambda: plan.H.tri_to_vec(a, out=o)))(
    plan.buf(node.inputs[0]), plan.out(node.outputs[0])), lambda node, gs: [None if gs[0] is None else vec_to_tri(gs[0])])

KERN_KINDS = {"rbf": 0, "csym_rbf": 1, "sqdist": 2}


def gram(X, X2, ell, kind="rbf") -> Tensor:
    X, X2, ell = as_tensor(X), as_tensor(X2), as_tensor(ell)
    if X.shape[-1] != X2.shape[-1]:
        raise ValueError("gram: input dimensions differ")
    lead = X.shape[:-2] if len(X.shape) >= len(X2.shape) else X2.shape[:-2]
    if len(ell.shape) == 2 and ell.shape[0] > 1:
        if lead and int(np.prod(lead)) != ell.shape[0]:
            raise ValueError("gram: %d lengthscale sets for a batch of %s" % (ell.shape[0], lead))
        lead = lead or (ell.shape[0],)
    return make("gram", (X, X2, ell), {"kind": kind}, [tuple(lead) + (X.shape[-2], X2.shape[-2])]).outputs[0]


def _gram_layout(tX, tX2, tell):
    n, d = tX.shape[-2], tX.shape[-1]
    n2 = tX2.shape[-2]
    BX = int(np.prod(tX.shape[:-2])) if len(tX.shape) > 2 else 1
    BX2 = int(np.prod(tX2.shape[:-2])) if len(tX2.shape) > 2 else 1
    BE = tell.shape[0] if (len(tell.shape) == 2 and tell.shape[0] > 1) else 1
    B = max(BX, BX2, BE)
    sX = n * d if (BX == B and B > 1) else 0
    sX2 = n2 * d if (BX2 == B and B > 1) else 0
    dl = tell.size // BE
    sEll = dl if BE > 1 else 0
    return B, BX, BX2, n, n2, d, sX, sX2, sEll, dl


def _gram_emit(plan, node):
    H = plan.H
    X, X2, ell = (plan.buf(t) for t in node.inputs)
    k = KERN_KINDS[node.attrs["kind"]]
    y = node.outputs[0]
    cons = plan._consumers.get(y, [])
    if (len(cons) == 1 and cons[0].op == "matutil" and cons[0].attrs["mode"] == 1 and y.shape[-1] == y.shape[-2]
            and y not in plan.outputs and y not in plan._bind):
        jit = cons[0].attrs["alpha"]
        kj = cons[0].outputs[0]
        cc = plan._consumers.get(kj, [])
        M = y.shape[-1]
        Bk = int(np.prod(y.shape[:-2])) if len(y.shape) > 2 else 1
        from ._settings import settings as _st

        if (bool(getattr(_st.runtime, "fold_gram", True)) and node.inputs[0] is node.inputs[1] and len(cc) == 1
                and cc[0].op == "cholesky" and kj not in plan.outputs
                and kj not in plan._bind and plan.dtype == plan.torch.float32 and k in (H.KERN_RBF, H.KERN_CSYM_RBF)
                and any(c.op == "trinv" for c in plan._consumers.get(cc[0].outputs[0], ()))
                and H.cholesky_persistent_shape(Bk, M, plan.dtype)):
            plan._fused_matutil.add(cons[0].id)
            plan._gram_for_chol[cc[0].id] = (X, ell, k, jit)
            plan.note("Gram folded into the persistent Cholesky (hb_gram_cholesky_inverse)", node, True)
            return
        plan.note("Gram folded into the persistent Cholesky (hb_gram_cholesky_inverse)", node, False,
                  "needs fp32, K(z, z) with one reader (a factor + inverse), an RBF-family kernel, M % 64 == 0 and "
                  "settings.runtime.fold_gram")
        out = plan.out(cons[0].outputs[0])
        plan._fused_matutil.add(cons[0].id)
        plan.steps.append(lambda: H.gram_fwd(X, X2, ell, kind=k, out=out, diag_add=jit))
        return
    out = plan.out(y)
    plan.steps.append(lambda: H.gram_fwd(X, X2, ell, kind=k, out=out))


def _gram_vjp(node, gs):
    g = gs[0]
    if g is None:
        return [None, None, None]
    X, X2, ell = node.inputs
    if X is X2:
        n = make("gram_grad", (X, X2, ell, g), {"kind": node.attrs["kind"], "sym": True}, [X.shape, ell.shape])
        return [n.outputs[0], None, n.outputs[1]]
    n = make("gram_grad", (X, X2, ell, g), {"kind": node.attrs["kind"], "sym": False}, [X.shape, X2.shape, ell.shape])
    return list(n.outputs)


def _gram_grad_emit(plan, node):
    H = plan.H
    fused = plan._gram_in_mm.get(node.id)
    if fused is not None:
        lws, rows, d_, dl_, groups = fused
        oL = plan.out(node.outputs[1])
        plan.out(node.outputs[0])
        fold = lambda: H.gram_ell_fold(lws, rows, d_, dl_, groups, oL)
        plan.steps.append(fold)
        plan.chain_kind[id(fold)] = "full"
        return
    tX, tX2, tell, tg = node.inputs
    X, X2, ell, g = (plan.buf(t) for t in node.inputs)
    k = KERN_KINDS[node.attrs["kind"]]
    B, BX, BX2, n, n2, d, sX, sX2, sEll, dl = _gram_layout(tX, tX2, tell)
    if node.attrs.get("sym"):
        oX, oL = [plan.out(t) for t in node.outputs]
        tmp = plan.scratch((B, n, d)) if (BX == 1 and B > 1) else None
        ws = plan.scratch((max(B * n * d, 1),))

        ksym = k | (H.KERN_KBAR_SYMMETRIC if tg.node.attrs.get("sym_result") else 0)

        def sym_step():
            dst = tmp if tmp is not None else oX
            H.gram_bwd_raw(ksym, X, sX, X2, sX2, ell, sEll, dl, g, dst, dst, oL, B, n, n2, d, ws)
            if tmp is not None:
                H.reduce_mid(tmp, 1, B, n * d, out=oX)

        plan.steps.append(sym_step)
        if tmp is None:
            plan.chain_kind[id(sym_step)] = "tail"
        return
    oX, oX2, oL = [plan.out(t) for t in node.outputs]
    tmpX = plan.scratch((B, n, d)) if (BX == 1 and B > 1) else None
    tmpX2 = plan.scratch((B, n2, d)) if (BX2 == 1 and B > 1) else None
    ws = plan.scratch((max(B * n * d, 1),))

    def step():
        H.gram_bwd_raw(k, X, sX, X2, sX2, ell, sEll, dl, g, tmpX if tmpX is not None else oX,
                       tmpX2 if tmpX2 is not None else oX2, oL, B, n, n2, d, ws)
        if tmpX is not None:
            H.reduce_mid(tmpX, 1, B, n * d, out=oX)
        if tmpX2 is not None:
            H.reduce_mid(tmpX2, 1, B, n2 * d, out=oX2)

    plan.steps.append(step)
    if tmpX is None and tmpX2 is None:
        plan.chain_kind[id(step)] = "tail"


defop("gram", _gram_emit, _gram_vjp)
defop("gram_grad", _gram_grad_emit, None)

SGP_MODES = {"neglected": 0, "diagonal": 1}


def sgp_samples(x, z, ell, L, u, mode="diagonal", eps=None) -> Tuple[Tensor, Tensor, Tensor, Tensor]:
    x, z, ell, L, u = (as_tensor(t) for t in (x, z, ell, L, u))
    W = stop_gradient(trinv(L))
    M, n, P = z.shape[-2], x.shape[-2], u.shape[-2]
    lead = z.shape[:-2]
    ins = [x, z, ell, L, W, u] + ([as_tensor(eps)] if eps is not None else [])
    nd = make("sgp", tuple(ins), {"mode": mode}, [lead + (P, n), lead + (M, n), lead + (n,), lead + (n,)],
              unique=(eps is None and mode == "diagonal"))
    return tuple(nd.outputs)


def _through_stop_gradient(t):
    while t.node.op == "stop_gradient":
        t = t.node.inputs[0]
    return t


def _sgp_emit(plan, node):
    H = plan.H
    x, z, ell, L, W, u = (plan.buf(t) for t in node.inputs[:6])
    eps_in = plan.buf(node.inputs[6]) if len(node.inputs) > 6 else None
    outs = tuple(plan.out(t) for t in node.outputs)
    mode = SGP_MODES[node.attrs["mode"]]
    rng = plan.rng("local") if (eps_in is None and mode == 1) else None
    wfrag, bf3 = plan._wfrag.get(_through_stop_gradient(node.inputs[4]), (None, False))
    bf3 = bf3 and node.inputs[0].shape[-1] <= 4 and node.inputs[5].shape[-2] <= 4
    prec = H.PREC_BF16X3 if bf3 else H.PREC_NATIVE
    zsh, xsh = node.inputs[1].shape, node.inputs[0].shape
    E, M, n, d, P = int(np.prod(zsh[:-2])) if len(zsh) > 2 else 1, zsh[-2], xsh[-2], xsh[-1], node.inputs[5].shape[-2]
    a_frag, skip_a = None, False
    if wfrag is not None and _sgp_frag_exchange(plan, node, prec):
        a_frag = plan.scratch((H.sgp_frag_elems(E, n, M, prec),))
        plan._afrag[node.outputs[1]] = (a_frag, prec)
        skip_a = node.outputs[1] not in plan.outputs
    head = None
    g = plan._sgp_head.get(node.id)
    if g is not None and wfrag is not None:
        units = H.sgp_head_units(x, z, u, prec, True, eps_in is None and mode == 1, rng)
        if units > 0:
            post = plan._gll_post.get(g.id)
            def early(t):
                shp = t.shape
                while t.node.op == "reshape" and t not in plan._buf:
                    t = t.node.inputs[0]
                return plan.buf(t).view(shp)

            head = dict(y=early(g.inputs[0]), var=early(g.inputs[2]),
                        scale=early(g.inputs[3]) if len(g.inputs) > 3 else None,
                        dmu=plan.out(g.outputs[1]), post=post[0] if post else 0.0,
                        fbar=plan.out(post[1]) if post else None,
                        part=plan.scratch((3 * units,)), units=units)
            plan._gll_fused[g.id] = (head["part"], units)
            plan.pin_side_reads([g.inputs[0], g.inputs[2]] + ([g.inputs[3]] if len(g.inputs) > 3 else []))
    step = lambda: H.sgp_fwd(x, z, ell, W, u, eps_in=eps_in, rng=rng, mode=mode, out=outs, wfrag=wfrag,
                             prec=prec, a_frag=a_frag, skip_a=skip_a, head=head)
    ep = "forward contraction starts inside the persistent Cholesky's launch (hb_sgp_rider_begin)"
    cell = plan._chol_rider.get(_through_stop_gradient(node.inputs[4]))
    from ._settings import settings as _st
    if not bool(getattr(_st.runtime, "early_forward", False)):
        cell = None
    if cell is not None and cell["rider"] is None:
        if not H.sgp_rider_supported(x, z, u, prec, wfrag is not None, eps_in is None and mode == 1, rng):
            plan.note(ep, node, False, "needs the fused finishing pass (fp32, one latent function, d <= 2, M % 64 == 0)")
        else:
            reads = [node.inputs[0], node.inputs[1], node.inputs[2], node.inputs[5]] + list(node.inputs[6:])
            if head is not None:
                reads += [g.inputs[0], g.inputs[2]] + list(g.inputs[3:4])
            early_nodes = {id(nd) for nd in plan._emitted[:cell["epos"]]}

            def ready(t):
                while t.node.op in ("reshape", "stop_gradient") and t.node.inputs:
                    t = t.node.inputs[0]
                return t.node.op.startswith("leaf:") or id(t.node) in early_nodes

            if all(ready(t) for t in reads):
                cell["rider"] = step
                plan.step_labels[id(cell["step"])] = "cholesky+sgp"
                plan.step_riders[id(cell["step"])] = node
                plan.note(ep, node, True)
                return
            plan.note(ep, node, False, "an operand is produced after the factorisation has been launched")
    plan.steps.append(step)
    plan.chain_kind[id(step)] = "tail"


def _sgp_vjp(node, gs):
    gf = gs[0]
    if gf is None:
        return [None] * len(node.inputs)
    if any(g is not None for g in gs[1:3]):
        raise NotImplementedError("gradients through the A / v outputs of sgp_samples")
    x, z, ell, L, W, u = node.inputs[:6]
    f, A, v, eps = node.outputs
    n = make("sgp_grad", (x, z, ell, W, u, eps, A, v, gf), {"mode": node.attrs["mode"]},
             [L.shape, u.shape, z.shape, ell.shape, x.shape])
    Lb, ub, zb, lb, xb = n.outputs
    return [xb, zb, lb, Lb, None, ub] + [None] * (len(node.inputs) - 6)


def _sgp_grad_emit(plan, node):
    H = plan.H
    x, z, ell, W, u, eps, A, v, gf = (plan.buf(t) for t in node.inputs)
    Lb, ub, zb, lb, xb = (plan.out(t) for t in node.outputs)
    mode = SGP_MODES[node.attrs["mode"]]
    need_x = plan.needed(node.outputs[4])
    if need_x and len(node.inputs[1].shape) > 2 and len(node.inputs[0].shape) == 2:
        raise NotImplementedError("gradient w.r.t. an x shared by several experts")
    xbuf = xb.reshape((-1,) + tuple(xb.shape[-2:])) if need_x else None
    wfrag, bf3 = plan._wfrag.get(_through_stop_gradient(node.inputs[3]), (None, False))
    bf3 = bf3 and not need_x and node.inputs[0].shape[-1] <= 4 and node.inputs[4].shape[-2] <= 4
    prec = H.PREC_BF16X3 if bf3 else H.PREC_NATIVE
    a_frag, fprec = plan._afrag.get(node.inputs[6], (None, None))
    if a_frag is not None:
        prec = fprec
    kbar_frag = plan.scratch((a_frag.numel(),)) if a_frag is not None else None
    Kbar = plan.scratch(A.shape) if a_frag is None else None
    plan.steps.append(lambda: H.sgp_bwd(x, z, ell, W, u, eps, A, v, gf, mode=mode, need_xbar=need_x,
                                        out=(Kbar, Lb, ub, zb, lb, xbuf), wfrag=wfrag, prec=prec, a_frag=a_frag,
                                        kbar_frag=kbar_frag))


defop("sgp", _sgp_emit, _sgp_vjp)
defop("sgp_grad", _sgp_grad_emit, None)

SGP_PREDICT_MODES = {"neglected": 0, "diagonal": 1, "fullrank": 2}
SGP_PREDICT_S = {"diag": 0, "tril": 1}


def sgp_predict(x, z, ell, L, m, s, mode="diagonal", s_kind="diag", jitter=0.0) -> Tuple[Tensor, Tensor]:
    x, z, ell, L, m, s = (as_tensor(t) for t in (x, z, ell, L, m, s))
    W = stop_gradient(trinv(L))
    lead, P, n = z.shape[:-2], m.shape[-2], x.shape[-2]
    if tuple(m.shape) != tuple(lead) + (P, z.shape[-2]):
        raise ValueError("sgp_predict: m must be %s, got %s" % (tuple(lead) + (P, z.shape[-2]), tuple(m.shape)))
    nd = make("sgp_predict", (x, z, ell, L, W, m, s), {"mode": mode, "s_kind": s_kind, "jitter": float(jitter)},
              [lead + (P, n), lead + (P, n)])
    return nd.outputs[0], nd.outputs[1]


def _sgp_predict_emit(plan, node):
    H = plan.H
    x, z, ell, _, W, m, s = (plan.buf(t) for t in node.inputs)
    mean, var = (plan.out(t) for t in node.outputs)
    zsh, xsh = node.inputs[1].shape, node.inputs[0].shape
    E, M, n, d, P = int(np.prod(zsh[:-2])) if len(zsh) > 2 else 1, zsh[-2], xsh[-2], xsh[-1], node.inputs[5].shape[-2]
    s_kind = SGP_PREDICT_S[node.attrs["s_kind"]]
    wfrag, bf3 = plan._wfrag.get(_through_stop_gradient(node.inputs[4]), (None, False))
    from ._settings import settings as _st

    want = bool(getattr(_st.runtime, "fused_predict", True))
    fused = want and H.sgp_predict_fused(plan.dtype, E, n, M, d, P, s_kind, wfrag is not None)
    plan.note("fused streaming prediction (hb_sgp_predict, one strip kernel)", node, fused,
              "settings.runtime.fused_predict is off" if not want else
              "needs fp32, the fragment-major W images, M % 32 == 0, 32 <= M <= 512, d <= 4, P <= 4 and a full-rank S "
              "only for one latent function: column chunks (hb_sgp_A + hb_matmul + column statistics)")
    wf = wfrag if fused else None
    ws = plan.scratch((max(H.sgp_predict_ws_elems(plan.dtype, E, n, M, d, P, s_kind, wf is not None), 1),))
    mode, jit = SGP_PREDICT_MODES[node.attrs["mode"]], node.attrs["jitter"]
    plan.steps.append(lambda: H.sgp_predict(x, z, ell, W, m, s, s_kind=s_kind, mode=mode, jitter=jit, out=(mean, var),
                                            wfrag=wf, ws=ws))


def _sgp_predict_vjp(node, gs):
    if any(g is not None for g in gs):
        raise NotImplementedError("sgp_predict (SparseGP.predict_f) is forward-only: no gradient through its mean or variance")
    return [None] * len(node.inputs)


defop("sgp_predict", _sgp_predict_emit, _sgp_predict_vjp)


def sgp_predict_cov(x, z, ell, L, s, P, mode="diagonal", s_kind="diag", jitter=0.0) -> Tensor:
    x, z, ell, L, s = (as_tensor(t) for t in (x, z, ell, L, s))
    W = stop_gradient(trinv(L))
    lead, n, M = tuple(z.shape[:-2]), x.shape[-2], z.shape[-2]
    E = int(np.prod(lead)) if lead else 1
    if s_kind == "diag" and tuple(s.shape) != lead + (P, M):
        raise ValueError("sgp_predict_cov: s must be %s, got %s" % (lead + (P, M), tuple(s.shape)))
    if s_kind == "tril" and (E * P != 1 or tuple(s.shape) != (M, M)):
        raise ValueError("sgp_predict_cov: a full-rank S must be [%d, %d] for one latent function of one expert" % (M, M))
    nd = make("sgp_predict_cov", (x, z, ell, L, W, s), {"mode": mode, "s_kind": s_kind, "jitter": float(jitter), "P": int(P)},
              [lead + (P, n, n)])
    return nd.outputs[0]


def _sgp_predict_cov_emit(plan, node):
    H = plan.H
    x, z, ell, _, W, s = (plan.buf(t) for t in node.inputs)
    cov = plan.out(node.outputs[0])
    zsh, xsh = node.inputs[1].shape, node.inputs[0].shape
    E, M, n, P = int(np.prod(zsh[:-2])) if len(zsh) > 2 else 1, zsh[-2], xsh[-2], node.attrs["P"]
    s_kind = SGP_PREDICT_S[node.attrs["s_kind"]]
    wfrag, _ = plan._wfrag.get(_through_stop_gradient(node.inputs[4]), (None, False))
    plan.note("fused predictive covariance (hb_sgp_predict_cov: A, then one symmetric MFMA product)", node, True)
    ws = plan.scratch((max(H.sgp_predict_cov_ws_elems(plan.dtype, E, n, M, P, s_kind), 1),))
    mode, jit = SGP_PREDICT_MODES[node.attrs["mode"]], node.attrs["jitter"]
    plan.steps.append(lambda: H.sgp_predict_cov(x, z, ell, W, s, P, s_kind=s_kind, mode=mode, jitter=jit, out=cov,
                                                wfrag=wfrag, ws=ws))


def _sgp_predict_cov_vjp(node, gs):
    if any(g is not None for g in gs):
        raise NotImplementedError("sgp_predict_cov (SparseGP.predict_f(full_cov=True)) is forward-only: no gradient through "
                                  "the covariance or the draws built on it")
    return [None] * len(node.inputs)


defop("sgp_predict_cov", _sgp_predict_cov_emit, _sgp_predict_cov_vjp)


def topo_order(outputs: Sequence[Tensor]) -> List[Node]:
    seen, order = set(), []
    stack = [(t.node, False) for t in outputs]
    while stack:
        n, done = stack.pop()
        if done:
            order.append(n)
            continue
        if n.id in seen:
            continue
        seen.add(n.id)
        stack.append((n, True))
        for t in n.inputs:
            if t.node.id not in seen:
                stack.append((t.node, False))
    return order


def _scatter_partition(ts):
    if len(ts) < 2 or any(t.node.op != "scatter_strided" for t in ts):
        return None
    xshape = tuple(ts[0].node.attrs["xshape"])
    if len(xshape) < 1:
        return None
    cst = tuple(_contig_strides(xshape))
    parts, axis = [], None
    for t in ts:
        a = t.node.attrs
        if tuple(a["xshape"]) != xshape or len(a["shape"]) != len(xshape) or tuple(a["strides"]) != cst:
            return None
        diff = [i for i in range(len(xshape)) if a["shape"][i] != xshape[i]]
        if len(diff) != 1 or (axis is not None and diff[0] != axis):
            return None
        axis = diff[0]
        if a["offset"] % cst[axis] != 0:
            return None
        start = a["offset"] // cst[axis]
        if not 0 <= start or start + a["shape"][axis] > xshape[axis]:
            return None
        parts.append((start, a["shape"][axis], t.node.inputs[0]))
    parts.sort(key=lambda p: p[0])
    pos = 0
    for off, w, _ in parts:
        if off != pos:
            return None
        pos += w
    if pos != xshape[axis]:
        return None
    return concat([p[2] for p in parts], axis)


def add_n(ts: List[Tensor]) -> Tensor:
    packed = _scatter_partition(ts)
    if packed is not None:
# ... 194 lines not shown
    consumers = {}
    for nd in order:
        for t in nd.inputs:
            consumers.setdefault(t, []).append(nd)
    outputs = set(outputs)
    open_clusters = []

    def can_join(nd, c):
        R, n = c.R, c.n
        if len(c.nodes) >= EW_COL_MAX_NODES:
            return False
        fo = _colform(nd.outputs[0].shape, R, n)
        if nd.op == "ew":
            if nd.attrs["f"] == "GAUSS_LOGPDF_GRAD" or len(nd.outputs) != 1 or len(nd.inputs) > 3 or fo is None:
                return False
            forms = [_colform(t.shape, R, n) for t in nd.inputs]
            if any(f is None for f in forms):
                return False
            best = "full" if "full" in forms else ("row" if "row" in forms else "scalar")
            return best == fo
        if nd.op == "reduce":
            a = nd.attrs
            return (a["kind"] in ("sum", "max") and a["K1"] == 1 and a["R"] == R and a["K2"] == n
                    and _colform(nd.inputs[0].shape, R, n) == "full")
        if nd.op == "reshape":
            return member.get(nd.inputs[0].node.id) is c and fo is not None and fo == _colform(nd.inputs[0].shape, R, n)
        if nd.op == "bcast":
            return member.get(nd.inputs[0].node.id) is c and fo == "full" and _colform(nd.inputs[0].shape, R, n) in ("row", "scalar")
        if nd.op == "strided":
            return member.get(nd.inputs[0].node.id) is not c and _col_strided_view(nd, R, n) is not None
        return False

    def seed_space(nd):
        if nd.op == "ew" and nd.attrs["f"] != "GAUSS_LOGPDF_GRAD" and len(nd.outputs) == 1:
            return _col_space_of(nd.outputs[0].shape)
        if nd.op == "strided":
            sp = _col_space_of(nd.outputs[0].shape)
            return sp if sp and _col_strided_view(nd, sp[0], sp[1]) is not None else None
        if nd.op == "reduce" and nd.attrs["K1"] == 1 and nd.attrs["kind"] in ("sum", "max"):
            sp = _col_space_of(nd.inputs[0].shape)
            return sp if sp and sp == (nd.attrs["R"], nd.attrs["K2"]) else None
        return None

    for nd in order:
        joined = None
        if nd.id not in skip and nd.op in ("ew", "reduce", "reshape", "bcast", "strided"):
            cands = []
            for t in nd.inputs:
                c = member.get(t.node.id)
                if c is not None and not c.sealed and c not in cands:
                    cands.append(c)
            cands += [c for c in reversed(open_clusters) if not c.sealed and c not in cands]
            for c in cands:
                if can_join(nd, c):
                    joined = c
                    break
            if joined is None:
                sp = seed_space(nd)
                if sp is not None:
                    joined = _ColCluster(sp[0], sp[1])
                    open_clusters.append(joined)
                    if not can_join(nd, joined):
                        open_clusters.pop()
                        joined = None
            if joined is not None:
                joined.nodes.append(nd)
                member[nd.id] = joined
        for t in nd.inputs:
            c = member.get(t.node.id)
            if c is not None and c is not joined:
                c.sealed = True
    for c in open_clusters:
        changed = True
        while changed:
            changed = False
            for nd in list(c.nodes):
                if nd.op != "strided":
                    continue
                o = nd.outputs[0]
                if o in outputs or any(member.get(x.id) is not c for x in consumers.get(o, [])) or not consumers.get(o):
                    c.nodes.remove(nd)
                    del member[nd.id]
                    changed = True
        ids = {nd.id for nd in c.nodes}
        ext_in = {t for nd in c.nodes for t in nd.inputs if t.node.id not in ids}
        outs = [o for nd in c.nodes for o in nd.outputs if nd.op != "strided"
                and (o in outputs or any(x.id not in ids for x in consumers.get(o, [])))]
        keep = (any(nd.op in ("reduce", "strided") for nd in c.nodes) and sum(1 for nd in c.nodes if nd.op in ("ew", "reduce")) >= 2
                and len(ext_in) <= EW_COL_MAX_IN and 1 <= len(outs) <= EW_COL_MAX_OUT)
        if not keep:
            for nd in c.nodes:
                del member[nd.id]
            c.nodes = []
    return member


INFO_POOL_WORDS = 65536


class CholeskyError(ArithmeticError):
    """A Cholesky factorisation met a non-positive pivot (TensorFlow raises
    InvalidArgumentError from tf.cholesky at the same point)."""


class Plan:

    def __init__(self, outputs, dtype, device, leaf_resolver, rngs, binds=None, prologue=None, stream=None):
        from . import hip_ops

        import torch

        self.H = hip_ops
        self.torch = torch
        self.dtype, self.device = dtype, device
        self.outputs = list(outputs)
        self.steps: List = []
        self._buf: Dict[Tensor, object] = {}
        self._bind: Dict[Tensor, object] = {}
        self._rngs = rngs
        self._infos: List[Tuple[object, str]] = []
        self._nocap: List[str] = []
        self._graph = None
        self._graphs: Dict[object, object] = {}
        self._capture_enabled = False
        self._info_pool = None
        self._info_used = 0
        self.stream = stream
        self.side_effect_steps = set()
        self.explain = []
        self.param_only_steps = []
        self.prologue = []
        self.trail_version = None
        self.chain_kind: Dict[int, str] = {}
        self.chain_members: Dict[int, list] = {}
        self._chains_fused = False
        self.step_labels = {}
        self.step_nodes = {}
        self.noise_inputs: Dict[Tensor, object] = {}
        self._injected: Dict[Tensor, bool] = {}
        self._leaf_resolver = leaf_resolver
        order = topo_order(self.outputs)
        self._order_pos = {n.id: i for i, n in enumerate(order)}
        self._order = order
        self._needed = set()
        for n in order:
            for t in n.inputs:
                self._needed.add(t)
        for t in self.outputs:
            self._needed.add(t)
        self._extra_copies = []
        self._fused_trinv = set()
        self._wfrag: Dict[Tensor, object] = {}
        self._afrag: Dict[Tensor, object] = {}
        self._fused_matutil = set()
        self._fused_concat = set()
        self._lazy_cols: Dict[Tensor, object] = {}
        for t, b in (binds or []):
            self._prebind(t, b)
        if prologue:
            prologue(self)
        from ._settings import settings as _st

        fuse = bool(getattr(_st.runtime, "fuse_elementwise", True))
        consumers0 = {}
        for n in order:
            for t in n.inputs:
                consumers0.setdefault(t, []).append(n)
        self._gll_post: Dict[int, tuple] = {}
        self._absorbed = set()
        if fuse:
            outs_set = set(self.outputs)
            for n in order:
                if n.op == "gauss_ll":
                    post = _gauss_ll_post(n, consumers0, outs_set)
                    if post is not None and not any(m.id in self._absorbed for m in post[2]):
                        self._gll_post[n.id] = post
                        self._absorbed.update(m.id for m in post[2])
                        self.note("likelihood head writes dobjective/df (hb_gauss_ll_post)", n, True)
                    else:
                        self.note("likelihood head writes dobjective/df (hb_gauss_ll_post)", n, False,
                                  "dmu is not followed by exactly scale * (post * dmu) feeding nothing else" if post is None
                                  else "its elementwise tail is already absorbed by another head")
        else:
            self.note("elementwise fusion", None, False, "settings.runtime.fuse_elementwise is off")
        self._colclusters = cluster_columns(order, outputs=self.outputs, skip=self._absorbed,
                                            enabled=fuse and hip_ops.ewise_jit_enabled() and bool(getattr(_st.runtime, "column_programs", True)))
        self._clusters = cluster_elementwise(order, enabled=fuse, skip=set(self._colclusters) | self._absorbed,
                                             max_elems=EW_CLUSTER_MAX_ELEMS_JIT if hip_ops.ewise_jit_enabled() else EW_CLUSTER_MAX_ELEMS)
        consumers = {}
        for n in order:
            for t in n.inputs:
                consumers.setdefault(t, []).append(n)
        self._consumers = consumers
        self._sgp_head: Dict[int, Node] = {}
        self._gll_in_sgp: Dict[int, Node] = {}
        self._gll_fused: Dict[int, tuple] = {}
        self._pending: List[tuple] = []
        if fuse and bool(getattr(_st.runtime, "head_in_contraction", True)):
            hoist_mb = self.side_jobs_enabled()

            def emitted_before(t, pos):
                while t.node.op == "reshape":
                    t = t.node.inputs[0]
                nd = t.node
                if nd.op == "leaf:minibatch" and hoist_mb:
                    return True
                cl = self._clusters.get(nd.id) or self._colclusters.get(nd.id)
                last = cl.nodes[-1] if (cl is not None and len(cl.nodes) >= 2) else nd
                return self._order_pos[last.id] < pos
            for n in order:
                if n.op != "gauss_ll" or len(n.inputs[1].shape) == 0:
                    continue
                ft = n.inputs[1]
                while ft.node.op == "reshape":
                    ft = ft.node.inputs[0]
                sg = ft.node
                hp = "likelihood head inside the forward contraction (hb_sgp_fwd_gauss)"
                if sg.op != "sgp" or ft is not sg.outputs[0] or sg.id in self._sgp_head or sg.inputs[5].shape[-2] != 1:
                    self.note(hp, n, False, "f is not the single latent function of an sgp draw" if sg.op != "sgp" or ft is not sg.outputs[0]
                              else ("the draw already carries a head" if sg.id in self._sgp_head else "more than one latent function (P > 1)"))
                    continue
                if n.inputs[0].size != ft.size:
                    self.note(hp, n, False, "y and f differ in size (a broadcast)")
                    continue
                pos = self._order_pos[sg.id]
                others = [n.inputs[0], n.inputs[2]] + list(n.inputs[3:4])
                if all(emitted_before(t, pos) for t in others):
                    self._sgp_head[sg.id] = n
                    self._gll_in_sgp[n.id] = sg
                    self.note(hp, n, True)
                else:
                    self.note(hp, n, False, "y / var / scale are produced after the draw is launched")
            self._mm_head: Dict[int, Node] = {}
            if bool(getattr(_st.runtime, "head_in_decoder", True)):
                hp = "likelihood head inside the layer's product (hb_matmul_gauss)"
                for n in order:
                    if n.op != "gauss_ll" or n.id in self._gll_in_sgp or len(n.inputs[1].shape) != 2:
                        continue
                    ft, single = n.inputs[1], True
                    while ft.node.op == "reshape":
                        single = single and len(consumers.get(ft, [])) == 1
                        ft = ft.node.inputs[0]
                    mm = ft.node
                    if mm.op != "matmul" or ft is not mm.outputs[0]:
                        continue
                    at = mm.attrs
                    why = None
                    if at["ta"] or at["tb"] or at.get("actgrad") or at["act"] != "none" or len(mm.inputs[0].shape) != 2 or len(mm.inputs[1].shape) != 2:
                        why = "the product is transposed, batched or carries an activation"
                    elif not single or len(consumers.get(ft, [])) != 1 or ft in self.outputs or ft in self._bind:
                        why = "f is read by something else as well"
                    elif n.inputs[0].shape != n.inputs[1].shape or mm.id in self._mm_head:
                        why = "y and f differ in shape"
                    elif not all(emitted_before(t, self._order_pos[mm.id]) for t in [n.inputs[0], n.inputs[2]] + list(n.inputs[3:4])):
                        why = "y / var / scale are produced after the product is launched"
                    elif hip_ops.matmul_gauss_units(ft.shape[0], mm.inputs[0].shape[1], ft.shape[1], dtype) == 0:
                        why = "shape outside the row-streaming form (fp32, n >= 2048, 32 < N <= 256, K = 16 / 32 / 64 / 128)"
                    if why is None:
                        self._mm_head[mm.id] = n
                        self._gll_in_sgp[n.id] = mm
                    self.note(hp, n, why is None, why or "")
        self._place: Dict[Tensor, object] = {}
        for n in order:
            if n.op != "concat":
                continue
            o, ax = n.outputs[0], n.attrs["axis"]
            if any(d != 1 for d in o.shape[:ax]):
                continue
            dst, off = None, 0
            for t in n.inputs:
                tgt = self._place_target(t)
                if (tgt is not None and tgt not in self._bind and tgt not in self._place and tgt not in self.outputs
                        and len(consumers.get(tgt, [])) == 1):
                    if dst is None:
                        dst = self.out(o).reshape(-1)
                    self._place[tgt] = dst[off:off + t.size].view(tgt.shape)
                off += t.size
        self._gram_for_chol: Dict[int, tuple] = {}
        self._gram_in_mm: Dict[int, tuple] = {}
        self._chol_rider: Dict[Tensor, dict] = {}
        self.step_riders: Dict[int, Node] = {}
        self._mlp2: Dict[int, dict] = {}
        self._colsum_of: Dict[int, Node] = {}
        self._fused_colsum = set()
        for n in order:
            if (n.op != "matmul" or not n.attrs["ta"] or n.attrs["tb"] or n.attrs.get("actgrad") or len(n.inputs) != 2
                    or n.attrs["act"] != "none" or len(n.inputs[0].shape) != 2 or len(n.inputs[1].shape) != 2):
                continue
            gmat = n.inputs[1]
            for r in consumers.get(gmat, []):
                ra = r.attrs if r.op == "reduce" else None
                if (ra is None or r.id in self._fused_colsum or ra["kind"] != "sum" or ra["K1"] != 1
                        or ra["R"] != gmat.shape[0] or ra["K2"] != gmat.shape[1]):
                    continue
                cl = self._clusters.get(r.id)
                if cl is not None and len(cl.nodes) > 1:
                    continue
                rout = r.outputs[0]
                if any(self._order_pos[c.id] < self._order_pos[n.id] for c in consumers.get(rout, [])):
                    continue
                self._colsum_of[n.id] = r
                self._fused_colsum.add(r.id)
                self.note("weight + bias gradient from one pass (hb_matmul_colsum)", n, True)
                break
        self._emitted: List[Node] = []
        self._side_cands: List[dict] = []
# ... 543 lines not shown
```

### henbun_amd/hip_ops.py

```python
from __future__ import annotations

import ctypes
from ctypes import c_double, c_int, c_long, c_void_p

import numpy as np
import torch

from . import _lib

EW = dict(
    NEG=1, EXP=2, LOG=3, SQRT=4, SQUARE=5, ABS=6, SIGN=7, SIGMOID=8, RELU=9, SOFTPLUS=10, TANH=11,
    RECIP=12, RSQRT=13, STEP=14, AFFINE=15, CLIP=16, CLIPMASK=17, LGAMMA=18, POWC=19, LOG1P=20,
    COPY=21, DIGAMMA=22,
    ADD=32, SUB=33, MUL=34, DIV=35, MAX=36, MIN=37, POW=38, GT=39, GE=40, LT=41, LE=42, EQ=43,
    SIGMOID_GRAD=44, TANH_GRAD=45, RELU_GRAD=46, SOFTPLUS_GRAD=47, CLIP_GRAD=48,
    WHERE=64, FMA=65, GAUSS_LOGPDF=66,
    GAUSS_LOGPDF_GRAD=80,
)
RED_SUM, RED_MAX = 0, 1
KERN_RBF, KERN_CSYM_RBF, KERN_SQDIST = 0, 1, 2
KERN_KBAR_SYMMETRIC = 256
EW_PROG_SUM = 256
MM_LOWER_OUT = 1
MM_TRIL_OUT = 2
# ... 740 lines not shown
    assert X.dtype == torch.float32
    BX, M, d = _batch_view(X)
    B = BX
    if ell.dim() >= 2 and ell.shape[0] > 1:
        B = max(B, ell.shape[0])
    assert BX in (1, B)
    sX = M * d if (BX == B and B > 1) else 0
    sEll, dl = _ell_layout(ell, B, d)
    batched = X.dim() > 2 or sEll != 0
    shape = ((B,) if batched else ()) + (M, M)
    if out is None:
        out = _empty(shape, dtype=X.dtype, device=X.device)
    if inv is None:
        inv = _empty(shape, dtype=X.dtype, device=X.device)
    if info is None:
        info = _empty(max(B, 1), dtype=torch.int32, device=X.device)
    if ws is None:
        ws = cholesky_workspace(X.dtype, X.device, B, M)
    assert ws.numel() >= cholesky_ws_elems(B, M, X.dtype)
    if frag is not None:
        assert frag.numel() >= (5 if frag_bf16x3 else 2) * B * M * M and frag.dtype == X.dtype
    _lib.lib().call("hb_gram_cholesky_inverse_f32", kind, _p(X), sX, _p(ell), sEll, dl, d, float(diag_add), _p(out), _p(inv), B, M,
                    _p(info), _p(ws), _p(frag), int(bool(frag_bf16x3 and frag is not None)), stream())
    return out, inv, info


def trinv(L, out=None):
    _chk(L)
    M = L.shape[-1]
    B = L.numel() // max(M * M, 1)
    if out is None:
        out = _empty_like(L)
    ws = workspace(L.dtype, L.device, max(B * M * M, 1))
    _lib.lib().call("hb_trinv" + _suf(L), _p(L), _p(out), B, M, _p(ws), stream())
    return out


def _sgp_dims(x, z, u):
    E = z.shape[0] if z.dim() == 3 else 1
    M, d = z.shape[-2], z.shape[-1]
    n = x.shape[-2]
    P = u.shape[-2]
    sx = n * d if (x.dim() == 3 and x.shape[0] == E and E > 1) else 0
    return E, n, M, d, P, sx


def sgp_strip_path(E, n, M, d, P, prec=PREC_NATIVE):
    return bool(_lib.lib().raw("hb_sgp_strip_path")(E, n, M, d, P, int(prec)))


def sgp_frag_elems(E, n, M, prec=PREC_NATIVE):
    base = E * M * 32 * ((n + 31) // 32)
    return base * 3 // 2 if prec == PREC_BF16X3 else base


def sgp_head_units(x, z, u, prec, has_wfrag, draw, rng):
    E, n, M, d, P, _ = _sgp_dims(x, z, u)
    if x.dtype != torch.float32:
        return 0
    return int(_lib.lib().raw("hb_sgp_head_units")(E, n, M, d, P, int(prec), int(bool(has_wfrag)), int(bool(draw)),
                                                  rng.nlanes if rng is not None else 0))


def matmul_gram_vjp_ok(M, K, batch, d, dtype):
    if dtype != torch.float32:
        return False
    return bool(_lib.lib().raw("hb_matmul_gram_vjp_ok")(int(M), int(K), int(batch), int(d)))


def matmul_gram_vjp(a, b, out, transA, transB, X, sX, ell, sEll, dl, d, xbar, ell_partial, part, counters):
    M = out.shape[-1]
    batch = out.numel() // (M * M)
    K = a.shape[-2] if transA else a.shape[-1]
    sA = a.stride(0) if a.dim() == 3 and a.shape[0] > 1 else 0
    sB = b.stride(0) if b.dim() == 3 and b.shape[0] > 1 else 0
    _lib.lib().call("hb_matmul_gram_vjp_f32", _p(a), _p(b), _p(out), batch, M, K, a.stride(-2), b.stride(-2), out.stride(-2),
                    sA, sB, M * M, int(bool(transA)), int(bool(transB)), _p(X), int(sX), _p(ell), int(sEll), int(dl), int(d),
                    _p(xbar), _p(ell_partial), _p(part), _p(counters), stream())


def gram_ell_fold(partial, rows, d, dl, groups, ellbar):
    _lib.lib().call("hb_gram_ell_fold" + _suf(partial), _p(partial), int(rows), int(d), int(dl), int(groups), _p(ellbar), stream())


def matmul_gauss_units(n, K, N, dtype):
    if dtype != torch.float32:
        return 0
    return int(_lib.lib().raw("hb_matmul_gauss_units")(int(n), int(K), int(N)))


def matmul_gauss(x, w, bias, head):
    for t in (x, w):
        _chk(t)
    n, K = x.shape
    N = w.shape[1]
    _lib.lib().call("hb_matmul_gauss_f32", _p(x), x.stride(0), _p(w), w.stride(0), _p(bias), _p(head["y"]), _p(head.get("scale")),
                    _p(head["var"]), float(head.get("post") or 0.0), _p(head["dmu"]), _p(head.get("fbar")), _p(head["part"]),
                    int(head["units"]), int(n), int(K), int(N), stream())


def sgp_rider_supported(x, z, u, prec, has_wfrag, draw, rng):
    E, n, M, d, P, _ = _sgp_dims(x, z, u)
    if x.dtype != torch.float32:
        return False
    return bool(_lib.lib().raw("hb_sgp_rider_supported")(E, n, M, d, P, int(prec), int(bool(has_wfrag)), int(bool(draw)),
                                                         rng.nlanes if rng is not None else 0))


def sgp_rider_begin():
    _lib.lib().call("hb_sgp_rider_begin")


def sgp_rider_flush():
    _lib.lib().call("hb_sgp_rider_flush", stream())


def sgp_rider_pending():
    return int(_lib.lib().raw("hb_sgp_rider_pending")())


def gauss_ll_fold(part, nb, ll, ds, dv):
    _lib.lib().call("hb_gauss_ll_fold" + _suf(part), _p(part), int(nb), _p(ll), _p(ds), _p(dv), stream())


def sgp_fwd(x, z, ell, W, u, eps_in=None, rng=None, mode=SGP_DIAGONAL, out=None, wfrag=None, prec=PREC_NATIVE,
            a_frag=None, skip_a=False, head=None):
    for t in (x, z, ell, W, u):
        _chk(t)
    E, n, M, d, P, sx = _sgp_dims(x, z, u)
    lead = (E,) if z.dim() == 3 else ()
    dev, dt = x.device, x.dtype
    if out is None:
        f = _empty(lead + (P, n), dtype=dt, device=dev)
        A = _empty(lead + (M, n), dtype=dt, device=dev)
        v = _empty(lead + (n,), dtype=dt, device=dev)
        eps = _empty(lead + (n,), dtype=dt, device=dev)
    else:
        f, A, v, eps = out
    dl = ell.numel() // E
    rp, rl = _rng_args(rng)
    ws = workspace(dt, dev, int(_lib.lib().raw("hb_sgp_ws_elems")(E, n, M, d, P)))
    if head is not None:
        _lib.lib().call("hb_sgp_fwd_gauss_f32", KERN_RBF, mode, _p(x), sx, _p(z), _p(ell), dl, _p(W), _p(wfrag), int(prec), _p(u),
                        _p(eps_in), rp, rl, _p(eps), None if (skip_a and a_frag is not None) else _p(A), _p(a_frag), _p(f), _p(v),
                        E, n, M, d, P, _p(ws), _p(head["y"]), _p(head.get("scale")), _p(head["var"]), float(head.get("post") or 0.0),
                        _p(head["dmu"]), _p(head.get("fbar")), _p(head["part"]), int(head["units"]), stream())
        return f, A, v, eps
    _lib.lib().call("hb_sgp_fwd" + _suf(x), KERN_RBF, mode, _p(x), sx, _p(z), _p(ell), dl, _p(W), _p(wfrag), int(prec), _p(u), _p(eps_in),
                    rp, rl, _p(eps), None if (skip_a and a_frag is not None) else _p(A), _p(a_frag), _p(f), _p(v), E, n,
                    M, d, P, _p(ws), stream())
    return f, A, v, eps


def sgp_A(x, z, ell, W, out=None, wfrag=None, prec=PREC_NATIVE):
    E = z.shape[0] if z.dim() == 3 else 1
    M, d = z.shape[-2], z.shape[-1]
    n = x.shape[-2]
    sx = n * d if (x.dim() == 3 and x.shape[0] == E and E > 1) else 0
    if out is None:
        out = _empty(((E,) if z.dim() == 3 else ()) + (M, n), dtype=x.dtype, device=x.device)
    _lib.lib().call("hb_sgp_A" + _suf(x), KERN_RBF, _p(x), sx, _p(z), _p(ell), ell.numel() // E, _p(W), _p(wfrag), int(prec),
                    _p(out), E, n, M, d, stream())
    return out


def sgp_predict_fused(dtype, E, n, M, d, P, s_kind, has_wfrag):
    return (dtype == torch.float32 and bool(has_wfrag) and 32 <= M <= 512 and M % 32 == 0 and 1 <= d <= 4 and 1 <= P <= 4
            and n > 0 and 1 <= E <= 65535 and (s_kind == SGP_S_DIAG or E * P == 1))


def sgp_predict_ws_elems(dtype, E, n, M, d, P, s_kind, has_wfrag):
    return int(_lib.lib().raw("hb_sgp_predict_ws_elems")(int(E), int(n), int(M), int(d), int(P), int(s_kind),
                                                         int(bool(has_wfrag)), 4 if dtype == torch.float32 else 8))


def sgp_predict(x, z, ell, W, m, s, s_kind=SGP_S_DIAG, mode=SGP_DIAGONAL, jitter=0.0, out=None, wfrag=None, ws=None):
    for t in (x, z, ell, W, m, s):
        _chk(t)
    E, n, M, d, P, sx = _sgp_dims(x, z, m)
    lead = (E,) if z.dim() == 3 else ()
    dev, dt = x.device, x.dtype
    if out is None:
        mean = _empty(lead + (P, n), dtype=dt, device=dev)
        var = _empty(lead + (P, n), dtype=dt, device=dev)
    else:
        mean, var = out
    if ws is None:
        ws = workspace(dt, dev, max(sgp_predict_ws_elems(dt, E, n, M, d, P, s_kind, wfrag is not None), 1))
    _lib.lib().call("hb_sgp_predict" + _suf(x), KERN_RBF, _p(x), sx, _p(z), _p(ell), ell.numel() // E, _p(W), _p(wfrag), _p(m),
                    _p(s), int(s_kind), int(mode), float(jitter), _p(mean), _p(var), E, n, M, d, P, _p(ws), stream())
    return mean, var


def sgp_predict_cov_ws_elems(dtype, E, n, M, P, s_kind):
    return int(_lib.lib().raw("hb_sgp_predict_cov_ws_elems")(int(E), int(n), int(M), int(P), int(s_kind),
                                                             4 if dtype == torch.float32 else 8))


def sgp_predict_cov(x, z, ell, W, s, P, s_kind=SGP_S_DIAG, mode=SGP_DIAGONAL, jitter=0.0, out=None, wfrag=None, ws=None):
    for t in (x, z, ell, W, s):
        _chk(t)
    E, n, M, d, _, sx = _sgp_dims(x, z, s if s_kind == SGP_S_DIAG else z)
    lead = (E,) if z.dim() == 3 else ()
    dev, dt = x.device, x.dtype
    if out is None:
        out = _empty(lead + (int(P), n, n), dtype=dt, device=dev)
    if ws is None:
        ws = workspace(dt, dev, max(sgp_predict_cov_ws_elems(dt, E, n, M, P, s_kind), 1))
    _lib.lib().call("hb_sgp_predict_cov" + _suf(x), KERN_RBF, _p(x), sx, _p(z), _p(ell), ell.numel() // E, _p(W), _p(wfrag),
                    _p(s), int(s_kind), int(mode), float(jitter), _p(out), E, n, M, d, int(P), _p(ws), stream())
    return out


def sgp_bwd(x, z, ell, W, u, eps, A, v, fbar, mode=SGP_DIAGONAL, need_xbar=False, out=None, wfrag=None,
            prec=PREC_NATIVE, a_frag=None, kbar_frag=None):
    E, n, M, d, P, sx = _sgp_dims(x, z, u)
    dev, dt = x.device, x.dtype
    dl = ell.numel() // E
    if out is None:
        Kbar = _empty_like(A) if a_frag is None else None
        Lbar = _empty_like(W)
        ubar = _empty_like(u)
        zbar = _empty_like(z)
        ellbar = _empty_like(ell)
        xbar = _empty((E, n, d), dtype=dt, device=dev) if need_xbar else None
    else:
        Kbar, Lbar, ubar, zbar, ellbar, xbar = out
    wse = _lib.lib().raw("hb_sgp_ws_elems")(E, n, M, d, P)
    ws = workspace(dt, dev, wse)
    if a_frag is not None and kbar_frag is None:
        kbar_frag = _empty(a_frag.numel(), dtype=dt, device=dev)
    _lib.lib().call("hb_sgp_bwd" + _suf(x), KERN_RBF, mode, _p(x), sx, _p(z), _p(ell), dl, _p(W), _p(wfrag), int(prec), _p(u), _p(eps),
                    _p(A) if a_frag is None else None, _p(a_frag), _p(v), _p(fbar), _p(Kbar) if a_frag is None else None,
                    _p(kbar_frag), _p(Lbar), _p(ubar), _p(zbar), _p(ellbar), _p(xbar), E, n, M, d, P, _p(ws), stream())
    return Lbar, ubar, zbar, ellbar, xbar


def adam_step(theta, g, m, v, t, lr=1e-3, b1=0.9, b2=0.999, eps=1e-8, gscale=1.0, tick=True, info=None, dpflag=None,
              fail=None):
    assert t.dtype == torch.int64
    n_info = 0
    if info is not None:
        assert info.dtype == torch.int32 and info.is_contiguous()
        n_info = info.numel()
    if fail is not None:
        assert fail.dtype == torch.int64 and fail.numel() == 2
    if dpflag is not None:
        assert dpflag.dtype == theta.dtype and dpflag.numel() == 1
    _lib.lib().call("hb_adam_step" + _suf(theta), _p(theta), _p(g), _p(m), _p(v), theta.numel(), float(lr), float(b1),
                    float(b2), float(eps), float(gscale), _p(t), int(bool(tick)), _p(info) if n_info else None, n_info,
                    _p(dpflag) if dpflag is not None else None, _p(fail) if fail is not None else None, stream())


def allreduce_sum(flat, comm_handle):
    _chk(flat)
    _lib.lib().call("hb_allreduce_sum" + _suf(flat), _p(flat), flat.numel(), comm_handle, stream())


def dp_pack(tail, objective, info):
    assert tail.numel() == 2
    n_info = 0 if info is None else info.numel()
    _lib.lib().call("hb_dp_pack" + _suf(tail), _p(tail), _p(objective), _p(info) if n_info else None, n_info, stream())


class CapturedGraph:

    def __init__(self):
        self._exec = c_void_p(None)

    def begin(self):
        _lib.lib().call("hb_graph_begin_capture", stream())
        set_capturing(True)

    def end(self):
        set_capturing(False)
        _lib.lib().call("hb_graph_end_capture", stream(), ctypes.byref(self._exec))

    def launch(self):
        _lib.lib().call("hb_graph_launch", self._exec, stream())

    def __del__(self):
        try:
            if self._exec:
                _lib.lib().raw("hb_graph_destroy")(self._exec)
        except Exception:
            pass


def device_info():
    buf = ctypes.create_string_buffer(256)
    cus = ctypes.c_int(0)
    _lib.lib().call("hb_device_info", buf, 256, ctypes.byref(cus))
    return buf.value.decode(), cus.value
```

### include/henbun_hip.h

```cpp
#ifndef HENBUN_HIP_H
#define HENBUN_HIP_H

#include <stdint.h>

#ifdef __cplusplus
extern "C" {
#endif

#define HB_ABI_VERSION 2

int hb_version(void);
const char* hb_last_error_string(void);
int hb_debug_set(const char* key, long value);
int hb_debug_clear(void);
int hb_device_info(char* buf, int buflen, int* cu_count);

int hb_graph_begin_capture(void* stream);
int hb_graph_end_capture(void* stream, void** exec_out);
int hb_graph_launch(void* exec, void* stream);
int hb_graph_destroy(void* exec);

enum {
  HB_EW_NEG = 1, HB_EW_EXP, HB_EW_LOG, HB_EW_SQRT, HB_EW_SQUARE, HB_EW_ABS, HB_EW_SIGN,
  HB_EW_SIGMOID, HB_EW_RELU, HB_EW_SOFTPLUS, HB_EW_TANH, HB_EW_RECIP, HB_EW_RSQRT,
// ... 73 lines not shown

int hb_fill_f32(float* out, long n, double v, void* stream);
int hb_fill_f64(double* out, long n, double v, void* stream);

int hb_gather_rows_f32(const float* src, long nsrc, long row, const long* idx, const long* perm,
                       long n, float* dst, int* err, void* stream);
int hb_gather_rows_f64(const double* src, long nsrc, long row, const long* idx, const long* perm,
                       long n, double* dst, int* err, void* stream);
int hb_gather_rows_multi_f32(int narr, const float* const* srcs, const long* rows, float* const* dsts,
                             long nsrc, const long* idx, const long* perm, long n, int* err, void* stream);
int hb_gather_rows_multi_f64(int narr, const double* const* srcs, const long* rows, double* const* dsts,
                             long nsrc, const long* idx, const long* perm, long n, int* err, void* stream);

int hb_gather_rows_multi_draw_f32(int narr, const float* const* srcs, const long* rows, float* const* dsts,
                                  long nsrc, uint64_t* state, long nlanes, long lo, long hi, long* idx_out,
                                  const long* perm, long n, int* err, void* stream);
int hb_gather_rows_multi_draw_f64(int narr, const double* const* srcs, const long* rows, double* const* dsts,
                                  long nsrc, uint64_t* state, long nlanes, long lo, long hi, long* idx_out,
                                  const long* perm, long n, int* err, void* stream);

int hb_matutil_f32(const float* in, float* out, long B, long R, long C, int mode, long lower,
                   long upper, double alpha, void* stream);
int hb_matutil_f64(const double* in, double* out, long B, long R, long C, int mode, long lower,
                   long upper, double alpha, void* stream);

int hb_rng_init(uint64_t* state, long nlanes, uint64_t seed, uint64_t stream_id, void* stream);
int hb_rng_normal_f32(uint64_t* state, long nlanes, float* out, long n, void* stream);
int hb_rng_normal_f64(uint64_t* state, long nlanes, double* out, long n, void* stream);
int hb_rng_randint(uint64_t* state, long nlanes, long* out, long n, long lo, long hi, void* stream);

int hb_diag_sample_kl_fwd_f32(const float* mu, const float* s, const float* u_in, uint64_t* rng,
                              long rng_lanes, float* u_out, float* x, float* kl, long n, long L,
                              long ld_mu, long ld_s, float* ws, void* stream);
int hb_diag_sample_kl_fwd_f64(const double* mu, const double* s, const double* u_in, uint64_t* rng,
                              long rng_lanes, double* u_out, double* x, double* kl, long n, long L,
                              long ld_mu, long ld_s, double* ws, void* stream);
int hb_diag_sample_kl_bwd_f32(const float* s, const float* u, const float* x, const float* xbar,
                              const float* klbar, float* mubar, float* sbar, long n, long L, long ld_s,
                              long ld_out, void* stream);
int hb_diag_sample_kl_bwd_f64(const double* s, const double* u, const double* x, const double* xbar,
                              const double* klbar, double* mubar, double* sbar, long n, long L, long ld_s,
                              long ld_out, void* stream);
int hb_fullrank_sample_kl_fwd_f32(const float* mu, const float* S, const float* u_in, uint64_t* rng,
                                  long rng_lanes, float* u_out, float* x, float* kl, long rows,
                                  long size, int packed, float* ws, void* stream);
int hb_fullrank_sample_kl_fwd_f64(const double* mu, const double* S, const double* u_in,
                                  uint64_t* rng, long rng_lanes, double* u_out, double* x,
                                  double* kl, long rows, long size, int packed, double* ws,
                                  void* stream);
int hb_fullrank_one_launch_shape(long rows, long size);
int hb_fullrank_sample_kl_fwd1_f32(const float* mu, const float* S, const float* u_in, uint64_t* rng,
                                   long rng_lanes, float* u_out, float* x, float* kl, long rows, long size,
                                   int packed, float* ws, unsigned* sync, void* stream);
int hb_fullrank_sample_kl_fwd1_f64(const double* mu, const double* S, const double* u_in, uint64_t* rng,
                                   long rng_lanes, double* u_out, double* x, double* kl, long rows, long size,
                                   int packed, double* ws, unsigned* sync, void* stream);
int hb_fullrank_sample_kl_bwd_f32(const float* S, const float* u, const float* x, const float* xbar,
                                  const float* klbar, float* mubar, float* Sbar, long rows,
                                  long size, int packed, void* stream);
int hb_fullrank_sample_kl_bwd_f64(const double* S, const double* u, const double* x,
                                  const double* xbar, const double* klbar, double* mubar,
                                  double* Sbar, long rows, long size, int packed, void* stream);
int hb_vec_to_tri_f32(const float* v, float* tri, long B, long N, void* stream);
int hb_vec_to_tri_f64(const double* v, double* tri, long B, long N, void* stream);
int hb_tri_to_vec_f32(const float* tri, float* v, long B, long N, void* stream);
int hb_tri_to_vec_f64(const double* tri, double* v, long B, long N, void* stream);

enum { HB_KERN_RBF = 0, HB_KERN_CSYM_RBF = 1, HB_KERN_SQDIST = 2 ,
       HB_KERN_KBAR_SYMMETRIC = 256  };
int hb_gram_fwd_f32(int kind, const float* X, long sX, const float* X2, long sX2, const float* ell,
                    long sEll, long dl, float* K, long B, long n, long n2, long d, double diag_add,
                    void* stream);
int hb_gram_fwd_f64(int kind, const double* X, long sX, const double* X2, long sX2,
                    const double* ell, long sEll, long dl, double* K, long B, long n, long n2, long d,
                    double diag_add, void* stream);
int hb_gram_bwd_f32(int kind, const float* X, long sX, const float* X2, long sX2, const float* ell,
                    long sEll, long dl, const float* Kbar, float* Xbar, float* X2bar, float* ellbar,
                    long B, long n, long n2, long d, float* ws, void* stream);
int hb_gram_bwd_f64(int kind, const double* X, long sX, const double* X2, long sX2,
                    const double* ell, long sEll, long dl, const double* Kbar, double* Xbar,
                    double* X2bar, double* ellbar, long B, long n, long n2, long d, double* ws,
                    void* stream);

enum {
  HB_MM_LOWER_OUT = 1,
  HB_MM_TRIL_OUT = 2,
  HB_MM_PHI_OUT = 4,
  HB_MM_SYM_OUT = 8,
  HB_MM_ACTGRAD = 16   ,
  HB_MM_SYMLOW_OUT = 32,
  HB_MM_COLSUM_B = 64
};
enum { HB_ACT_NONE = 0, HB_ACT_SIGMOID = 1, HB_ACT_RELU = 2, HB_ACT_TANH = 3 };
int hb_matmul_f32(const float* A, const float* B, float* C, long batch, long M, long N, long K,
                  long lda, long ldb, long ldc, long sA, long sB, long sC, int transA, int transB,
                  double alpha, double beta, const float* bias, long sBias, int act, int flags,
                  float* ws, long ws_elems, void* stream);
int hb_matmul_f64(const double* A, const double* B, double* C, long batch, long M, long N, long K,
                  long lda, long ldb, long ldc, long sA, long sB, long sC, int transA, int transB,
                  double alpha, double beta, const double* bias, long sBias, int act, int flags,
                  double* ws, long ws_elems, void* stream);

int hb_matmul_colsum_f32(const float* A, const float* B, float* C, float* colsum, long M, long N, long K, long lda, long ldb,
                         long ldc, float* ws, long ws_elems, void* stream);
int hb_matmul_colsum_f64(const double* A, const double* B, double* C, double* colsum, long M, long N, long K, long lda,
                         long ldb, long ldc, double* ws, long ws_elems, void* stream);

int hb_mlp2_sample_supported(long n, long din, long hid, long nout, long rng_lanes, int has_u);
long hb_mlp2_sample_ws_elems(long n, long din, long hid);
int hb_mlp2_sample_fwd_f32(const float* y, const float* w0, const float* b0, const float* w1, const float* b1, int act,
                           const float* u_in, uint64_t* rng, long rng_lanes, float* x, float* kl, float* u_out, float* o,
                           long n, long din, long hid, float* ws, void* stream);
int hb_mlp2_sample_bwd_f32(const float* y, const float* w0, const float* b0, const float* w1, int act, const float* o,
                           const float* u, const float* x, const float* xbar, const float* klbar, float* dw0, float* db0,
                           float* dw1, float* db1, long n, long din, long hid, float* ws, void* stream);

int hb_cholesky_f32(const float* A, float* L, long B, long M, int* info, void* stream);
int hb_cholesky_f64(const double* A, double* L, long B, long M, int* info, void* stream);

long hb_cholesky_inverse_ws_elems(long B, long M, int elem_bytes);
int hb_cholesky_persistent_shape(long B, long M, int elem_bytes);
int hb_gram_cholesky_inverse_f32(int kind, const float* X, long sX, const float* ell, long sEll, long dl, long d,
                                 double diag_add, float* L, float* W, long B, long M, int* info, float* ws,
                                 float* Wfrag, int frag_bf16x3, void* stream);
int hb_cholesky_inverse_f32(const float* A, float* L, float* W, long B, long M, int* info, float* ws,
                            float* Wfrag, int frag_bf16x3, void* stream);
int hb_cholesky_inverse_f64(const double* A, double* L, double* W, long B, long M, int* info,
                            double* ws, double* Wfrag, int frag_bf16x3, void* stream);
int hb_trinv_f32(const float* L, float* W, long B, long M, float* ws, void* stream);
int hb_trinv_f64(const double* L, double* W, long B, long M, double* ws, void* stream);

enum { HB_SGP_NEGLECTED = 0, HB_SGP_DIAGONAL = 1, HB_SGP_FULLRANK = 2  };
enum { HB_SGP_S_DIAG = 0, HB_SGP_S_TRIL = 1 };
enum { HB_PREC_NATIVE = 0, HB_PREC_BF16X3 = 1 };
long hb_sgp_ws_elems(long E, long n, long M, long d, long P);
int hb_sgp_strip_path(long E, long n, long M, long d, long P, int prec);
int hb_sgp_fwd_f32(int kind, int mode, const float* x, long sx, const float* z, const float* ell,
                   long dl, const float* W, const float* Wfrag, int prec, const float* u,
                   const float* eps_in, uint64_t* rng, long rng_lanes, float* eps_out, float* A,
                   float* A_frag, float* f, float* v, long E, long n, long M, long d, long P, float* ws,
                   void* stream);
int hb_sgp_fwd_f64(int kind, int mode, const double* x, long sx, const double* z, const double* ell,
                   long dl, const double* W, const double* Wfrag, int prec, const double* u,
                   const double* eps_in, uint64_t* rng, long rng_lanes, double* eps_out, double* A,
                   double* A_frag, double* f, double* v, long E, long n, long M, long d, long P,
                   double* ws, void* stream);
long hb_sgp_head_units(long E, long n, long M, long d, long P, int prec, int has_wfrag, int draw, long rng_lanes);
int hb_sgp_fwd_gauss_f32(int kind, int mode, const float* x, long sx, const float* z, const float* ell, long dl,
                         const float* W, const float* Wfrag, int prec, const float* u, const float* eps_in,
                         uint64_t* rng, long rng_lanes, float* eps_out, float* A, float* A_frag, float* f, float* v,
                         long E, long n, long M, long d, long P, float* ws, const float* y, const float* scale,
                         const float* var, double post, float* dmu, float* fbar, float* head_part, long units,
                         void* stream);
int hb_sgp_rider_supported(long E, long n, long M, long d, long P, int prec, int has_wfrag, int draw, long rng_lanes);
int hb_sgp_rider_begin(void);
int hb_sgp_rider_pending(void);
int hb_sgp_rider_flush(void* stream);
int hb_matmul_gram_vjp_ok(long M, long K, long batch, long d);
long hb_matmul_gram_vjp_ws_elems(long batch, long M, long d);
int hb_matmul_gram_vjp_f32(const float* A, const float* B, float* C, long batch, long M, long K, long lda, long ldb,
                           long ldc, long sA, long sB, long sC, int transA, int transB, const float* X, long sX,
                           const float* ell, long sEll, long dl, long d, float* Xbar, float* ell_partial,
                           float* part, unsigned* counters, void* stream);
int hb_gram_ell_fold_f32(const float* partial, long rows, long d, long dl, long groups, float* ellbar, void* stream);
int hb_gram_ell_fold_f64(const double* partial, long rows, long d, long dl, long groups, double* ellbar, void* stream);
long hb_matmul_gauss_units(long n, long K, long N);
int hb_matmul_gauss_f32(const float* A, long lda, const float* B, long ldb, const float* bias, const float* y,
                        const float* scale, const float* var, double post, float* dmu, float* fbar, float* part,
                        long units, long n, long K, long N, void* stream);
int hb_gauss_ll_fold_f32(const float* partial, long nb, float* ll, float* dscale, float* dvar, void* stream);
int hb_gauss_ll_fold_f64(const double* partial, long nb, double* ll, double* dscale, double* dvar, void* stream);
int hb_sgp_A_f32(int kind, const float* x, long sx, const float* z, const float* ell, long dl,
                 const float* W, const float* Wfrag, int prec, float* A, long E, long n, long M, long d,
                 void* stream);
int hb_sgp_A_f64(int kind, const double* x, long sx, const double* z, const double* ell, long dl,
                 const double* W, const double* Wfrag, int prec, double* A, long E, long n, long M,
                 long d, void* stream);
long hb_sgp_predict_ws_elems(long E, long n, long M, long d, long P, int s_kind, int has_wfrag, int dtype_bytes);
int hb_sgp_predict_f32(int kind, const float* x, long sx, const float* z, const float* ell, long dl, const float* W,
                       const float* Wfrag, const float* m, const float* s, int s_kind, int mode, double jitter, float* mean,
                       float* var, long E, long n, long M, long d, long P, float* ws, void* stream);
int hb_sgp_predict_f64(int kind, const double* x, long sx, const double* z, const double* ell, long dl, const double* W,
                       const double* Wfrag, const double* m, const double* s, int s_kind, int mode, double jitter,
                       double* mean, double* var, long E, long n, long M, long d, long P, double* ws, void* stream);
long hb_sgp_predict_cov_ws_elems(long E, long n, long M, long P, int s_kind, int dtype_bytes);
int hb_sgp_predict_cov_f32(int kind, const float* x, long sx, const float* z, const float* ell, long dl, const float* W,
                           const float* Wfrag, const float* s, int s_kind, int mode, double jitter, float* cov, long E, long n,
                           long M, long d, long P, float* ws, void* stream);
int hb_sgp_predict_cov_f64(int kind, const double* x, long sx, const double* z, const double* ell, long dl, const double* W,
                           const double* Wfrag, const double* s, int s_kind, int mode, double jitter, double* cov, long E,
                           long n, long M, long d, long P, double* ws, void* stream);
int hb_sgp_bwd_f32(int kind, int mode, const float* x, long sx, const float* z, const float* ell,
                   long dl, const float* W, const float* Wfrag, int prec, const float* u, const float* eps,
                   const float* A, const float* A_frag, const float* v, const float* fbar, float* Kbar,
                   float* Kbar_frag, float* Lbar, float* ubar, float* zbar, float* ellbar, float* xbar,
                   long E, long n, long M, long d, long P, float* ws, void* stream);
int hb_sgp_bwd_f64(int kind, int mode, const double* x, long sx, const double* z, const double* ell,
                   long dl, const double* W, const double* Wfrag, int prec, const double* u,
                   const double* eps, const double* A, const double* A_frag, const double* v,
                   const double* fbar, double* Kbar, double* Kbar_frag, double* Lbar, double* ubar,
                   double* zbar, double* ellbar, double* xbar, long E, long n, long M, long d, long P,
                   double* ws, void* stream);

int hb_adam_step_f32(float* theta, const float* g, float* m, float* v, long n, double lr, double b1,
                     double b2, double eps, double gscale, long* t, int tick, const int* info,
                     long n_info, const float* dpflag, long* fail, void* stream);
int hb_adam_step_f64(double* theta, const double* g, double* m, double* v, long n, double lr,
                     double b1, double b2, double eps, double gscale, long* t, int tick,
                     const int* info, long n_info, const double* dpflag, long* fail, void* stream);

int hb_side_push_gather_draw_f32(int narr, const float* const* srcs, const long* rows, float* const* dsts, long nsrc,
                                 uint64_t* state, long nlanes, long lo, long hi, long* idx_out, const long* perm,
                                 long n, int* err, void* stream);
int hb_side_push_diag_fwd_f32(const float* mu, const float* s, const float* u_in, uint64_t* rng, long rng_lanes,
                              float* u_out, float* x, float* kl, long n, long L, long ld_mu, long ld_s, float* ws,
                              void* stream);
int hb_side_push_diag_bwd_f32(const float* s, const float* u, const float* x, const float* xbar, const float* klbar,
                              float* mubar, float* sbar, long n, long L, long ld_s, long ld_out, void* stream);
int hb_side_pending(void);
int hb_side_flush(void* stream);
int hb_side_discard(void);

int hb_chain_begin(void);
int hb_chain_end(void* stream);
int hb_chain_discard(void);
int hb_chain_source(char* out, long cap);
int hb_chain_compile_dry(void);

#define HB_COMM_ID_BYTES 128
int hb_comm_available(void);
int hb_comm_unique_id(char* id128);
int hb_comm_init(const char* id128, int rank, int world, void** comm_out);
int hb_comm_destroy(void* comm);
int hb_allreduce_sum_f32(float* buf, long n, void* comm, void* stream);
int hb_allreduce_sum_f64(double* buf, long n, void* comm, void* stream);
int hb_dp_pack_f32(float* tail, const float* objective, const int* info, long n_info, void* stream);
int hb_dp_pack_f64(double* tail, const double* objective, const int* info, long n_info, void* stream);

#ifdef __cplusplus
}
#endif
#endif
```

Measured before the change: 41.24 million samples/s.

## Fuse SGP backward Kbar strip kernel into forward gauss-head launch

```diff
diff --git a/henbun_amd/_lib.py b/henbun_amd/_lib.py
--- a/henbun_amd/_lib.py
+++ b/henbun_amd/_lib.py
@@ -49,6 +49,10 @@
     "hb_sgp_rider_pending": [],
     "hb_sgp_rider_flush": [P],
     "hb_sgp_fwd_gauss_f32": [I, I, P, L, P, P, L, P, P, I, P, P, P, L, P, P, P, P, P, L, L, L, L, L, P, P, P, P, D, P, P, P, L, P],
+    "hb_sgp_fwd_bwd_supported": [L, L, L, L, L, I, I, I, L],
+    "hb_sgp_fwd_bwd_ws_elems": [L, L, L, L, L],
+    "hb_sgp_fwd_bwd_gauss_f32": [I, I, P, L, P, P, L, P, P, I, P, P, P, L, P, P, P, P, P, L, L, L, L, L, P, P, P, P, D, P, P, P, L, P, P],
+    "hb_sgp_bwd_rest_f32": [L, L, L, L, L, L, I, P, P, P, P, P, P, P, P],
     "hb_ewise_prog_image_bytes": [],
     "hb_ewise_prog_build": [I, P, P, I, P, P, I, P, P, P, I, P, P, P, P],
     "hb_ewise_jit_available": [],
@@ -71,7 +75,7 @@
     "hb_comm_destroy": [P],
 }
 _RESTYPES = {"hb_last_error_string": c_char_p, "hb_sgp_ws_elems": c_long, "hb_ewise_prog_image_bytes": c_long,
-             "hb_sgp_head_units": c_long, "hb_matmul_gauss_units": c_long, "hb_matmul_gram_vjp_ws_elems": c_long, "hb_cholesky_inverse_ws_elems": c_long, "hb_mlp2_sample_ws_elems": c_long,
+             "hb_sgp_head_units": c_long, "hb_sgp_fwd_bwd_ws_elems": c_long, "hb_matmul_gauss_units": c_long, "hb_matmul_gram_vjp_ws_elems": c_long, "hb_cholesky_inverse_ws_elems": c_long, "hb_mlp2_sample_ws_elems": c_long,
              "hb_sgp_predict_ws_elems": c_long, "hb_sgp_predict_cov_ws_elems": c_long}
 
 _TYPED = {
diff --git a/henbun_amd/csrc/sgp.hip b/henbun_amd/csrc/sgp.hip
--- a/henbun_amd/csrc/sgp.hip
+++ b/henbun_amd/csrc/sgp.hip
@@ -716,10 +716,18 @@
   return __hip_atomic_load(const_cast<float*>(p), __ATOMIC_RELAXED, __HIP_MEMORY_SCOPE_AGENT);
 }
 
+template <typename T>
+__device__ __forceinline__ T sgp_resid_coef_v(T epsj, T vv, T cs, int mode) {
+  if (mode != HB_SGP_DIAGONAL) return T(0);
+  const T av = hb_abs(vv);
+  return av > T(0) ? -epsj * hb_sign(vv) / hb_sqrt(av) * cs : T(0);
+}
+
 #define SGP_RED_LD 260
 template <bool AG, bool L16 = false>
 __device__ __forceinline__ void sgp_2t_epilogue(const SgpArgs<float>& a, float* lds_raw, const float (&csq)[16], const float (&cu)[16],
-                                                const long e, const int bx, const int col0, const int n, const bool means) {
+                                                const long e, const int bx, const int col0, const int n, const bool means,
+                                                float* bw_cj = nullptr, float* bw_fb = nullptr) {
   typedef float V4 __attribute__((ext_vector_type(4)));
   const int tid = threadIdx.x, lane = tid & 63, w = __builtin_amdgcn_readfirstlane(tid >> 6), li = lane & 31, h = lane >> 5;
   if (a.part) {
@@ -792,9 +800,19 @@
             float gg;
             hb_gauss_point<float>(AG ? sgp_ag_load(a.hy + idx0 + i) : a.hy[idx0 + i], fj, hs, iv, lc, gg, h_ll, h_sc, h_vr);
             a.hdmu[idx0 + i] = gg;
-            if (a.hfbar) a.hfbar[idx0 + i] = hs * (a.hpost * gg);
+            const float fbj = hs * (a.hpost * gg);
+            if (a.hfbar) a.hfbar[idx0 + i] = fbj;
+            if (bw_cj) {
+              float cs = 0.f;
+              cs += fbj;
+              bw_fb[2 * tid + i] = fbj;
+              bw_cj[2 * tid + i] = sgp_resid_coef_v<float>(zi, vv, cs, a.fin_diag ? HB_SGP_DIAGONAL : HB_SGP_NEGLECTED);
+            }
           }
         }
+      } else if (bw_cj) {
+        bw_cj[2 * tid] = bw_cj[2 * tid + 1] = 0.f;
+        bw_fb[2 * tid] = bw_fb[2 * tid + 1] = 0.f;
       }
     }
     if (a.head && tid < 64) {
@@ -814,17 +832,13 @@
   }
 }
 
-template <int D>
-__global__ void __launch_bounds__(SGP_STRIP_THREADS, 4) sgp_A_strip2t_kernel(SgpArgs<float> a) {
+#define SGP_2T_LDS_FLOATS (SGP_SN * SGP_SLD > 2 * SGP_SN * SGP_RED_LD ? SGP_SN * SGP_SLD : 2 * SGP_SN * SGP_RED_LD)
+template <int D, bool KEEP>
+__device__ __forceinline__ void sgp_2t_body(const SgpArgs<float>& a, float* lds_raw, float* zs, const long e, const int bx,
+                                            float (&keep)[2][16], float (&uk)[2], float* bw_cj, float* bw_fb) {
   typedef float V4 __attribute__((ext_vector_type(4)));
   typedef Mma<float> MM;
-  constexpr int KS_FLOATS = SGP_SN * SGP_SLD, RED_FLOATS = 2 * SGP_SN * SGP_RED_LD;
-  __shared__ __attribute__((aligned(16))) float lds_raw[KS_FLOATS > RED_FLOATS ? KS_FLOATS : RED_FLOATS];
-  __shared__ __attribute__((aligned(16))) float zs[SGP_SM_MAX * D];
   float (*Ks)[SGP_SLD] = reinterpret_cast<float (*)[SGP_SLD]>(lds_raw);
-  long e;
-  int bx;
-  sgp_block(a.efast, e, bx);
   const float* __restrict__ x = a.x + e * a.sx;
   const float* __restrict__ z = a.z + e * a.M * D;
   const float* __restrict__ ell = a.ell + e * a.dl;
@@ -938,6 +952,15 @@
       float row16[16];
       sgp_acc_t_rows(acc, row16);
       if (a.Af) sgp_store_frag_rows(a.Af, row16, e, nT, nS, tile, bx, col0, n, lane);
+      if (KEEP) {
+        if (ts < d0) {
+#pragma unroll
+          for (int i = 0; i < 16; ++i) keep[0][i] = row16[i];
+        } else {
+#pragma unroll
+          for (int i = 0; i < 16; ++i) keep[1][i] = row16[i];
+        }
+      }
       if (A) {
         float* ap = A + (long)(32 * tile + li) * n + col0 + 16 * h;
         if ((n & 3) == 0 && col0 + SGP_SN <= n) {
@@ -975,8 +998,19 @@
   }
 
   HB_SSTAMP(2);
-  sgp_2t_epilogue<false>(a, lds_raw, csq, cu, e, bx, col0, n, means);
+  sgp_2t_epilogue<false>(a, lds_raw, csq, cu, e, bx, col0, n, means, bw_cj, bw_fb);
   HB_SSTAMP(3);
+  if (KEEP) uk[0] = u0, uk[1] = u1;
+}
+template <int D>
+__global__ void __launch_bounds__(SGP_STRIP_THREADS, 4) sgp_A_strip2t_kernel(SgpArgs<float> a) {
+  __shared__ __attribute__((aligned(16))) float lds_raw[SGP_2T_LDS_FLOATS];
+  __shared__ __attribute__((aligned(16))) float zs[SGP_SM_MAX * D];
+  long e;
+  int bx;
+  sgp_block(a.efast, e, bx);
+  float keep[2][16], uk[2];
+  sgp_2t_body<D, false>(a, lds_raw, zs, e, bx, keep, uk, nullptr, nullptr);
 }
 
 #define SGP_S16_THREADS 1024
@@ -1822,9 +1856,15 @@
 }
 
 template <typename T>
+struct SgpBwdArgs;
+static int sgp_fwd_bwd_strip_launch(const SgpArgs<float>& a, const SgpBwdArgs<float>* b, long E, hipStream_t stream);
+static int sgp_fwd_bwd_strip_launch(const SgpArgs<double>&, const SgpBwdArgs<double>*, long, hipStream_t) { return -1; }
+
+template <typename T>
 static int sgp_fwd(int kind, int mode, const T* x, long sx, const T* z, const T* ell, long dl, const T* W, const T* Wf,
                    int prec, const T* u, const T* eps_in, uint64_t* rng, long rng_lanes, T* eps_out, T* A, T* A_frag, T* f,
-                   T* v, long E, long n, long M, long d, long P, T* ws, hipStream_t stream, const SgpHead<T>* head = nullptr) {
+                   T* v, long E, long n, long M, long d, long P, T* ws, hipStream_t stream, const SgpHead<T>* head = nullptr,
+                   const SgpBwdArgs<T>* bwd = nullptr) {
   HB_REQUIRE(!A_frag || (sizeof(T) == 4 && Wf && ws && hb_sgp_strip_path(E, n, M, d, P, prec)),
              "hb_sgp_fwd: a fragment-major A needs the column-strip form (fp32, Wfrag, hb_sgp_strip_path)");
   if (hb_chain_recording()) {
@@ -1879,6 +1919,11 @@
         }
       }
       HB_REQUIRE(!head || a.fin, "hb_sgp_fwd_gauss: this call cannot carry the head (hb_sgp_head_units(...) == 0)");
+      if (bwd) {
+        HB_REQUIRE(a.head && a.hfbar && a.Af && !a.W3 && !g_rider.armed,
+                   "hb_sgp_fwd_bwd_gauss: needs the head with fbar, A_frag, fp32 operands, and no pending early-start record");
+        return sgp_fwd_bwd_strip_launch(a, bwd, E, stream);
+      }
       if constexpr (std::is_same<T, float>::value) {
         if (g_rider.armed) {
           HB_REQUIRE(a.fin && !a.W3 && d <= SGP_E_DMAX, "hb_sgp_fwd after hb_sgp_rider_begin: this call cannot ride (hb_sgp_rider_supported)");
@@ -2172,6 +2217,235 @@
   return v;
 }
 
+template <bool BF3>
+__device__ __forceinline__ void sgp_abar_tile(const float (&avals)[16], const int k, const float (&uk)[4], const float* cjs,
+                                              const float (*fbs)[SGP_SN], unsigned char* ks_raw, float* __restrict__ pbar,
+                                              const int P, const int M) {
+  typedef float V4 __attribute__((ext_vector_type(4)));
+  float (*Ks)[SGP_SLD] = reinterpret_cast<float (*)[SGP_SLD]>(ks_raw);
+  __bf16 (*K3)[SGP_SN][SGP_S3LD] = reinterpret_cast<__bf16 (*)[SGP_SN][SGP_S3LD]>(ks_raw);
+  const int h = (threadIdx.x & 63) >> 5;
+  float usum[4] = {0.f, 0.f, 0.f, 0.f};
+#pragma unroll
+  for (int v = 0; v < 4; ++v) {
+    const V4 cj4 = *reinterpret_cast<const V4*>(&cjs[16 * h + 4 * v]);
+    V4 fb4[4];
+#pragma unroll
+    for (int p = 0; p < 4; ++p) fb4[p] = *reinterpret_cast<const V4*>(&fbs[p][16 * h + 4 * v]);
+#pragma unroll
+    for (int s2 = 0; s2 < 4; ++s2) {
+      const int c = 16 * h + 4 * v + s2;
+      const float aval = avals[4 * v + s2];
+      float val = aval * cj4[s2];
+#pragma unroll
+      for (int p = 0; p < 4; ++p)
+        if (p < P) {
+          val += uk[p] * fb4[p][s2];
+          usum[p] += fb4[p][s2] * aval;
+        }
+      if (BF3) {
+        const __bf16 b0 = (__bf16)val;
+        const float r1 = val - (float)b0;
+        const __bf16 b1 = (__bf16)r1;
+        K3[0][c][k] = b0, K3[1][c][k] = b1, K3[2][c][k] = (__bf16)(r1 - (float)b1);
+      } else {
+        Ks[c][k] = val;
+      }
+    }
+  }
+#pragma unroll
+  for (int p = 0; p < 4; ++p)
+    if (p < P) {
+      const float tsum = usum[p] + __shfl_xor(usum[p], 32);
+      if (h == 0) pbar[(long)p * M + k] = tsum;
+    }
+}
+
+template <int D, bool BF3>
+__device__ __forceinline__ void sgp_kbar_tail(const SgpBwdArgs<float>& a, unsigned char* ks_raw, const float* zs, const float* xss,
+                                              const float (&sc)[D], float* lred, const long e, const int bx,
+                                              float* __restrict__ part) {
+  typedef float V4 __attribute__((ext_vector_type(4)));
+  typedef __bf16 B8 __attribute__((ext_vector_type(8)));
+  typedef Mma<float> MM;
+  float (*Ks)[SGP_SLD] = reinterpret_cast<float (*)[SGP_SLD]>(ks_raw);
+  __bf16 (*K3)[SGP_SN][SGP_S3LD] = reinterpret_cast<__bf16 (*)[SGP_SN][SGP_S3LD]>(ks_raw);
+  float* __restrict__ Kbar = a.Kbar ? a.Kbar + e * a.M * a.n : nullptr;
+  const int M = (int)a.M, n = (int)a.n;
+  const int col0 = bx * SGP_SN, nS = (n + SGP_SN - 1) / SGP_SN;
+  const int tid = threadIdx.x, lane = tid & 63, w = __builtin_amdgcn_readfirstlane(tid >> 6), li = lane & 31, h = lane >> 5;
+  const int nT = M / 32;
+  const int ta = nT - 1 - w, tb = w;
+  const int d0 = ta > tb ? w + 1 : 0;
+  const int d1 = tb <= ta ? nT - w : 0;
+  const int nts = d0 + d1;
+  typename MM::Acc acc;
+#pragma unroll
+  for (int r = 0; r < 16; ++r) acc[r] = 0.f;
+  const int gc = col0 + li;
+
+  auto tile_of = [&](int ts) { return ts < d0 ? ta : tb; };
+  auto chunk_of = [&](int ts) { return ts < d0 ? ta + ts : tb + (ts - d0); };
+  float lwave[D];
+#pragma unroll
+  for (int dd = 0; dd < D; ++dd) lwave[dd] = 0.f;
+
+  auto retire = [&](int tile) {
+    sgp_acc_t_settle(acc);
+    float kb[16];
+    sgp_acc_t_rows(acc, kb);
+    if (col0 + SGP_SN > n) {
+#pragma unroll
+      for (int i = 0; i < 16; ++i)
+        if (col0 + 16 * h + i >= n) kb[i] = 0.f;
+    }
+    if (a.Kbar) {
+      float* kp = Kbar + (long)(32 * tile + li) * n + col0 + 16 * h;
+      if ((n & 3) == 0 && col0 + SGP_SN <= n) {
+#pragma unroll
+        for (int v = 0; v < 4; ++v) {
+          V4 q;
+#pragma unroll
+          for (int s2 = 0; s2 < 4; ++s2) q[s2] = kb[4 * v + s2];
+          *reinterpret_cast<V4*>(kp + 4 * v) = q;
+        }
+      } else {
+#pragma unroll
+        for (int i = 0; i < 16; ++i)
+          if (col0 + 16 * h + i < n) kp[i] = kb[i];
+      }
+    }
+    if (a.Kf && !BF3) sgp_store_frag_rows(a.Kf, kb, e, nT, nS, tile, bx, col0, n, lane);
+    if (BF3 && a.Kf)
+      sgp_store_frag3_row(reinterpret_cast<__bf16*>(a.Kf), (long)a.plane3 / a.M * 32 * nS, kb, e, nT, nS, tile, bx, lane);
+    const int row = 32 * tile + li;
+    float zr[D], zacc[D], lacc[D];
+#pragma unroll
+    for (int dd = 0; dd < D; ++dd) zr[dd] = zs[row * D + dd], zacc[dd] = 0.f, lacc[dd] = 0.f;
+#pragma unroll
+    for (int i = 0; i < 16; ++i) {
+      const int c = 16 * h + i;
+      float tt[D], r2 = 0.f;
+#pragma unroll
+      for (int dd = 0; dd < D; ++dd) {
+        tt[dd] = (zr[dd] - xss[c * D + dd]) * sc[dd];
+        r2 += tt[dd] * tt[dd];
+      }
+      const float gk = kb[i] * hb_exp2_neg<float>(r2);
+#pragma unroll
+      for (int dd = 0; dd < D; ++dd) {
+        zacc[dd] -= gk * tt[dd];
+        lacc[dd] += gk * tt[dd] * tt[dd];
+      }
+    }
+#pragma unroll
+    for (int dd = 0; dd < D; ++dd) {
+      zacc[dd] += __shfl_xor(zacc[dd], 32);
+      if (h == 0) part[(long)dd * M + row] = zacc[dd] * sc[dd] * float(1.0 / (SGP_EXP2_SCALE * SGP_EXP2_SCALE));
+      lwave[dd] += lacc[dd];
+    }
+#pragma unroll
+    for (int r = 0; r < 16; ++r) acc[r] = 0.f;
+  };
+
+  if (!BF3) {
+    const float* __restrict__ Wf = a.WTf + e * a.M * a.M;
+    auto load = [&](V4 (&f)[4], int ts) {
+      const int tc = ts < nts ? ts : nts - 1;
+      const float* p = Wf + ((long)(tile_of(tc) * nT + chunk_of(tc)) << 10) + 4 * lane;
+#pragma unroll
+      for (int v = 0; v < 4; ++v) f[v] = *reinterpret_cast<const V4*>(p + 256 * v);
+    };
+    auto compute = [&](const V4 (&f)[4], int ts) {
+      if (ts >= nts) return;
+      const int Q = chunk_of(ts);
+      V4 bv[4];
+#pragma unroll
+      for (int v = 0; v < 4; ++v) bv[v] = *reinterpret_cast<const V4*>(&Ks[li][32 * Q + 16 * h + 4 * v]);
+#pragma unroll
+      for (int v = 0; v < 4; ++v)
+#pragma unroll
+        for (int s2 = 0; s2 < 4; ++s2) acc = MM::mma(bv[v][s2], f[v][s2], acc);
+      if (ts == d0 - 1 || ts == nts - 1) retire(tile_of(ts));
+    };
+    if (nts > 0) {
+      V4 fa[4], fb2[4];
+      load(fa, 0);
+#pragma nounroll
+      for (int ts = 0; ts < nts; ts += 2) {
+        load(fb2, ts + 1);
+        __builtin_amdgcn_sched_barrier(0);
+        compute(fa, ts);
+        __builtin_amdgcn_sched_barrier(0);
+        load(fa, ts + 2);
+        __builtin_amdgcn_sched_barrier(0);
+        compute(fb2, ts + 1);
+        __builtin_amdgcn_sched_barrier(0);
+      }
+    }
+  } else {
+    const __bf16* __restrict__ W3 = reinterpret_cast<const __bf16*>(a.WT3) + e * a.M * a.M;
+    struct Frag {
+      B8 f[3][2];
+    };
+    auto load = [&](Frag& fr, int ts) {
+      const int tc = ts < nts ? ts : nts - 1;
+      const __bf16* p = W3 + ((long)(tile_of(tc) * nT + chunk_of(tc)) << 10) + 8 * lane;
+#pragma unroll
+      for (int t = 0; t < 3; ++t)
+#pragma unroll
+        for (int q = 0; q < 2; ++q) fr.f[t][q] = *reinterpret_cast<const B8*>(p + (long)t * a.plane3 + 512 * q);
+    };
+    auto compute = [&](const Frag& fr, int ts) {
+      if (ts >= nts) return;
+      const int Q = chunk_of(ts);
+#pragma unroll
+      for (int q = 0; q < 2; ++q) {
+        B8 b[3];
+#pragma unroll
+        for (int t = 0; t < 3; ++t) b[t] = *reinterpret_cast<const B8*>(&K3[t][li][32 * Q + 16 * q + 8 * h]);
+        acc = __builtin_amdgcn_mfma_f32_32x32x16_bf16(b[0], fr.f[2][q], acc, 0, 0, 0);
+        acc = __builtin_amdgcn_mfma_f32_32x32x16_bf16(b[2], fr.f[0][q], acc, 0, 0, 0);
+        acc = __builtin_amdgcn_mfma_f32_32x32x16_bf16(b[1], fr.f[1][q], acc, 0, 0, 0);
+        acc = __builtin_amdgcn_mfma_f32_32x32x16_bf16(b[0], fr.f[1][q], acc, 0, 0, 0);
+        acc = __builtin_amdgcn_mfma_f32_32x32x16_bf16(b[1], fr.f[0][q], acc, 0, 0, 0);
+        acc = __builtin_amdgcn_mfma_f32_32x32x16_bf16(b[0], fr.f[0][q], acc, 0, 0, 0);
+      }
+      if (ts == d0 - 1 || ts == nts - 1) retire(tile_of(ts));
+    };
+    if (nts > 0) {
+      Frag fa, fb2;
+      load(fa, 0);
+#pragma nounroll
+      for (int ts = 0; ts < nts; ts += 2) {
+        load(fb2, ts + 1);
+        __builtin_amdgcn_sched_barrier(0);
+        compute(fa, ts);
+        __builtin_amdgcn_sched_barrier(0);
+        load(fa, ts + 2);
+        __builtin_amdgcn_sched_barrier(0);
+        compute(fb2, ts + 1);
+        __builtin_amdgcn_sched_barrier(0);
+      }
+    }
+  }
+  __syncthreads();
+  float* red = lred;
+#pragma unroll
+  for (int dd = 0; dd < D; ++dd) {
+    const float t = wave_sum(lwave[dd]);
+    if (lane == 0) red[w * D + dd] = t;
+  }
+  __syncthreads();
+#pragma unroll
+  for (int dd = 0; dd < D; ++dd)
+    if (tid == dd) {
+      float t = 0.f;
+      for (int ww = 0; ww < SGP_STRIP_THREADS / 64; ++ww) t += red[ww * D + dd];
+      part[(long)(D + dd) * M] = t * sc[dd] * float(1.0 / (SGP_EXP2_SCALE * SGP_EXP2_SCALE * SGP_EXP2_SCALE));
+    }
+}
+
 template <int D, bool BF3>
 __global__ void __launch_bounds__(SGP_STRIP_THREADS, (BF3 || D >= 3) ? 2 : 4) sgp_kbar_strip_kernel(SgpBwdArgs<float> a) {
   typedef float V4 __attribute__((ext_vector_type(4)));
@@ -2541,6 +2815,61 @@
       for (int ww = 0; ww < SGP_STRIP_THREADS / 64; ++ww) t += red[ww * D + dd];
       part[(long)(D + dd) * M] = t * sc[dd] * float(1.0 / (SGP_EXP2_SCALE * SGP_EXP2_SCALE * SGP_EXP2_SCALE));
     }
+}
+
+template <int D>
+__global__ void __launch_bounds__(SGP_STRIP_THREADS, 2) sgp_fwd_kbar_strip_kernel(SgpArgs<float> a, SgpBwdArgs<float> b) {
+  __shared__ __attribute__((aligned(16))) float lds_raw[SGP_2T_LDS_FLOATS];
+  __shared__ __attribute__((aligned(16))) float zs[SGP_SM_MAX * D];
+  __shared__ __attribute__((aligned(16))) float xss[SGP_SN * D];
+  __shared__ __attribute__((aligned(16))) float cjs[SGP_SN];
+  __shared__ __attribute__((aligned(16))) float fbs[4][SGP_SN];
+  __shared__ float lred[(SGP_STRIP_THREADS / 64) * D];
+  static_assert(SGP_2T_LDS_FLOATS * 4 >= SGP_SN * SGP_SLD * 4, "Abar takes the K block's place");
+  long e;
+  int bx;
+  sgp_block(a.efast, e, bx);
+  const int M = (int)a.M, n = (int)a.n;
+  const int col0 = bx * SGP_SN, nS = (n + SGP_SN - 1) / SGP_SN;
+  const int tid = threadIdx.x, lane = tid & 63, w = __builtin_amdgcn_readfirstlane(tid >> 6), li = lane & 31;
+  if (tid < SGP_SN) {
+    const float* __restrict__ x = b.x + e * b.sx;
+    const int cc = col0 + tid;
+    const int cj = cc < n ? cc : n - 1;
+#pragma unroll
+    for (int dd = 0; dd < D; ++dd) xss[tid * D + dd] = x[cj * D + dd];
+  } else if (tid < 4 * SGP_SN) {
+    fbs[tid / SGP_SN][tid % SGP_SN] = 0.f;
+  }
+  float keep[2][16], u01[2];
+  sgp_2t_body<D, true>(a, lds_raw, zs, e, bx, keep, u01, cjs, fbs[0]);
+  __syncthreads();
+
+  float sc[D];
+  const float* __restrict__ ell = b.ell + e * b.dl;
+#pragma unroll
+  for (int dd = 0; dd < D; ++dd) sc[dd] = float(SGP_EXP2_SCALE) / ell[b.dl == 1 ? 0 : dd];
+  const int P = (int)b.P;
+  const int nq = 2 * D + P;
+  float* __restrict__ part = b.part + ((e * nS + bx) * (long)nq) * M;
+  unsigned char* ks_raw = reinterpret_cast<unsigned char*>(lds_raw);
+  {
+    const int nT = M / 32, t1 = nT - 1 - w, t0 = w;
+    if (w < t1) {
+      float uk[4];
+#pragma unroll
+      for (int p = 0; p < 4; ++p) uk[p] = p < P && p == 0 ? u01[0] : 0.f;
+      sgp_abar_tile<false>(keep[0], 32 * t0 + li, uk, cjs, fbs, ks_raw, part + (long)(2 * D) * M, P, M);
+    }
+    if (w <= t1) {
+      float uk[4];
+#pragma unroll
+      for (int p = 0; p < 4; ++p) uk[p] = p < P && p == 0 ? u01[1] : 0.f;
+      sgp_abar_tile<false>(keep[1], 32 * t1 + li, uk, cjs, fbs, ks_raw, part + (long)(2 * D) * M, P, M);
+    }
+  }
+  __syncthreads();
+  sgp_kbar_tail<D, false>(b, ks_raw, zs, xss, sc, lred, e, bx, part);
 }
 
 #ifndef HB_LSTAMP
@@ -3153,6 +3482,23 @@
 }
 static int sgp_bwd_strip_launch(SgpBwdArgs<double>, long, long, hipStream_t) { return -1; }
 
+static int sgp_fwd_bwd_strip_launch(const SgpArgs<float>& a0, const SgpBwdArgs<float>* b0, long E, hipStream_t stream) {
+  SgpArgs<float> a = a0;
+  SgpBwdArgs<float> b = *b0;
+  dim3 grid = sgp_grid(hb_cdiv(a.n, SGP_SN), 1, E, a.efast);
+  b.efast = a.efast;
+  if (a.d == 1)
+    hipLaunchKernelGGL((sgp_fwd_kbar_strip_kernel<1>), grid, dim3(SGP_STRIP_THREADS), 0, stream, a, b);
+  else if (a.d == 2)
+    hipLaunchKernelGGL((sgp_fwd_kbar_strip_kernel<2>), grid, dim3(SGP_STRIP_THREADS), 0, stream, a, b);
+  else if (a.d == 3)
+    hipLaunchKernelGGL((sgp_fwd_kbar_strip_kernel<3>), grid, dim3(SGP_STRIP_THREADS), 0, stream, a, b);
+  else
+    hipLaunchKernelGGL((sgp_fwd_kbar_strip_kernel<4>), grid, dim3(SGP_STRIP_THREADS), 0, stream, a, b);
+  HB_LAUNCH_CHECK();
+  return 0;
+}
+
 static int sgp_lbar_frag_launch(const float* Kf, const float* Af, float* slabs, long slab_cap, long E, long M, long nS,
                                 int prec, int* S_out, hipStream_t stream) {
   const int nT = (int)(M / 32);
@@ -3194,6 +3540,25 @@
   return 0;
 }
 static int sgp_lbar_frag_launch(const double*, const double*, double*, long, long, long, long, int, int*, hipStream_t) { return -1; }
+
+template <typename T>
+static int sgp_bwd_frag_rest(const T* A_frag, const T* Kbar_frag, T* ws, long E, long n, long M, long d, long dl, long P, int prec,
+                             T* Lbar, T* ubar, T* zbar, T* ellbar, hipStream_t stream) {
+  T* mmws = ws + E * n + E * M * d;
+  const long mmws_elems = 32 * E * M * M;
+  const long nS = hb_cdiv(n, SGP_SN);
+  const long npart = ((nS * (2 * d + P) * M * E + 63) / 64) * 64;
+  const long slab_cap = (mmws_elems - npart) / (E * M * M);
+  HB_REQUIRE(slab_cap >= 1, "hb_sgp_bwd: workspace too small for the Lbar slabs");
+  int S = 0;
+  int rc = sgp_lbar_frag_launch(Kbar_frag, A_frag, mmws + npart, slab_cap > 32 ? 32 : slab_cap, E, M, nS, prec, &S, stream);
+  if (rc) return rc;
+  const int nbx = (int)hb_cdiv(M, 64), nb_strip = nbx * (int)(2 * d + P) * (int)E;
+  hipLaunchKernelGGL(sgp_bwd_finish_kernel<T>, dim3((unsigned)(nb_strip + hb_stream_grid(E * M * M, 256))), dim3(256), 0, stream,
+                     mmws, (int)nS, M, d, dl, P, zbar, ellbar, ubar, nb_strip, nbx, mmws + npart, S, E, Lbar);
+  HB_LAUNCH_CHECK();
+  return 0;
+}
 
 template <typename T>
 static int sgp_bwd(int kind, int mode, const T* x, long sx, const T* z, const T* ell, long dl, const T* W,
@@ -3236,19 +3601,7 @@
     if (A_frag) a.Kbar = nullptr;
     int rc = sgp_bwd_strip_launch(a, E, nS, stream);
     if (rc) return rc;
-    if (A_frag) {
-      const long npart = ((nS * (2 * d + P) * M * E + 63) / 64) * 64;
-      const long slab_cap = (mmws_elems - npart) / (E * M * M);
-      HB_REQUIRE(slab_cap >= 1, "hb_sgp_bwd: workspace too small for the Lbar slabs");
-      int S = 0;
-      rc = sgp_lbar_frag_launch(Kbar_frag, A_frag, mmws + npart, slab_cap > 32 ? 32 : slab_cap, E, M, nS, prec, &S, stream);
-      if (rc) return rc;
-      const int nbx = (int)hb_cdiv(M, 64), nb_strip = nbx * (int)(2 * d + P) * (int)E;
-      hipLaunchKernelGGL(sgp_bwd_finish_kernel<T>, dim3((unsigned)(nb_strip + hb_stream_grid(E * M * M, 256))), dim3(256), 0, stream,
-                         mmws, (int)nS, M, d, dl, P, zbar, ellbar, ubar, nb_strip, nbx, mmws + npart, S, E, Lbar);
-      HB_LAUNCH_CHECK();
-      return 0;
-    }
+    if (A_frag) return sgp_bwd_frag_rest<T>(A_frag, Kbar_frag, ws, E, n, M, d, dl, P, prec, Lbar, ubar, zbar, ellbar, stream);
     hipLaunchKernelGGL(sgp_strip_finish_kernel<T>, dim3((unsigned)hb_cdiv(M, 64), (unsigned)(2 * d + P), (unsigned)E), dim3(256), 0,
                        stream, mmws, (int)nS, M, d, dl, P, zbar, ellbar, ubar);
     HB_LAUNCH_CHECK();
@@ -3329,3 +3682,46 @@
   return sgp_bwd<double>(kind, mode, x, sx, z, ell, dl, W, Wfrag, prec, u, eps, A, A_frag, v, fbar, Kbar, Kbar_frag, Lbar,
                          ubar, zbar, ellbar, xbar, E, n, M, d, P, ws, (hipStream_t)stream);
 }
+
+static inline bool sgp_fwd_bwd_ok(long E, long n, long M, long d, long P, int prec, int has_wfrag, int draw, long rng_lanes) {
+  return hb_sgp_head_units(E, n, M, d, P, prec, has_wfrag, draw, rng_lanes) > 0 &&
+         hb_cdiv(n, SGP_SN) * (2 * d + P) * M * E <= 32 * E * M * M;
+}
+extern "C" int hb_sgp_fwd_bwd_supported(long E, long n, long M, long d, long P, int prec, int has_wfrag, int draw, long rng_lanes) {
+  if (!sgp_fwd_bwd_ok(E, n, M, d, P, prec, has_wfrag, draw, rng_lanes)) return 0;
+  if (hb_debug_get("sgp_fwd_bwd_force", 0) != 0) return 1;
+  static int cus = 0;
+  if (cus == 0 && (hb_device_info(nullptr, 0, &cus) || cus <= 0)) cus = 256;
+  return E * hb_cdiv(n, SGP_SN) <= cus + cus / 4 ? 1 : 0;
+}
+extern "C" long hb_sgp_fwd_bwd_ws_elems(long E, long n, long M, long d, long P) { return hb_sgp_ws_elems(E, n, M, d, P); }
+
+extern "C" int hb_sgp_fwd_bwd_gauss_f32(int kind, int mode, const float* x, long sx, const float* z, const float* ell, long dl,
+                                        const float* W, const float* Wfrag, int prec, const float* u, const float* eps_in,
+                                        uint64_t* rng, long rng_lanes, float* eps_out, float* A, float* A_frag, float* f, float* v,
+                                        long E, long n, long M, long d, long P, float* ws, const float* y, const float* scale,
+                                        const float* var, double post, float* dmu, float* fbar, float* head_part, long units,
+                                        float* Kbar_frag, void* stream) {
+  HB_REQUIRE(y && var && dmu && fbar && head_part && units > 0 && A_frag && Kbar_frag && ws, "hb_sgp_fwd_bwd_gauss: NULL pointer");
+  HB_REQUIRE(sgp_fwd_bwd_ok(E, n, M, d, P, prec, Wfrag != nullptr, mode == HB_SGP_DIAGONAL && !eps_in, rng_lanes),
+             "hb_sgp_fwd_bwd_gauss: unsupported call (fp32 strip form with the head in the forward, see hb_sgp_fwd_bwd_supported)");
+  SgpHead<float> h;
+  h.y = y, h.scale = scale, h.var = var, h.post = post, h.dmu = dmu, h.fbar = fbar, h.part = head_part, h.units = units;
+  SgpBwdArgs<float> b;
+  b.W = W; b.u = u; b.A = nullptr; b.fbar = fbar; b.eps = eps_out ? eps_out : eps_in; b.v = v; b.Kbar = nullptr;
+  b.n = n; b.M = M; b.P = P; b.mode = mode; b.efast = 0;
+  b.x = x; b.sx = sx; b.z = z; b.ell = ell; b.dl = dl; b.d = d;
+  b.WTf = Wfrag + E * M * M; b.WT3 = nullptr; b.plane3 = E * M * M;
+  b.part = ws + E * n + E * M * d;
+  b.Af = A_frag; b.Kf = Kbar_frag;
+  return sgp_fwd<float>(kind, mode, x, sx, z, ell, dl, W, Wfrag, prec, u, eps_in, rng, rng_lanes, eps_out, A, A_frag, f, v,
+                        E, n, M, d, P, ws, (hipStream_t)stream, &h, &b);
+}
+extern "C" int hb_sgp_bwd_rest_f32(long E, long n, long M, long d, long dl, long P, int prec, const float* A_frag,
+                                   const float* Kbar_frag, float* Lbar, float* ubar, float* zbar, float* ellbar, float* ws,
+                                   void* stream) {
+  HB_REQUIRE(prec == HB_PREC_NATIVE, "hb_sgp_bwd_rest: fp32 images only");
+  HB_REQUIRE(A_frag && Kbar_frag && Lbar && ubar && zbar && ellbar && ws, "hb_sgp_bwd_rest: NULL pointer");
+  HB_REQUIRE(E >= 1 && n > 0 && M >= 32 && M % 32 == 0 && d >= 1 && (dl == 1 || dl == d) && P >= 1, "hb_sgp_bwd_rest: bad extents");
+  return sgp_bwd_frag_rest<float>(A_frag, Kbar_frag, ws, E, n, M, d, dl, P, prec, Lbar, ubar, zbar, ellbar, (hipStream_t)stream);
+}
diff --git a/henbun_amd/graph.py b/henbun_amd/graph.py
--- a/henbun_amd/graph.py
+++ b/henbun_amd/graph.py
@@ -1619,6 +1619,12 @@
     return t
 
 
+def _through_reshapes(t):
+    while t.node.op == "reshape":
+        t = t.node.inputs[0]
+    return t
+
+
 def _sgp_emit(plan, node):
     H = plan.H
     x, z, ell, L, W, u = (plan.buf(t) for t in node.inputs[:6])
@@ -1662,6 +1668,31 @@
     from ._settings import settings as _st
     if not bool(getattr(_st.runtime, "early_forward", False)):
         cell = None
+    fb = "backward strip kernel inside the forward's launch (hb_sgp_fwd_bwd_gauss)"
+    grads = [c for c in plan._consumers.get(node.outputs[1], ()) if c.op == "sgp_grad"] if a_frag is not None else []
+    why = None
+    if not bool(getattr(_st.runtime, "fused_sgp_bwd", True)):
+        why = "settings.runtime.fused_sgp_bwd is off"
+    elif head is None or head["fbar"] is None:
+        why = "no likelihood head writing fbar rides in the forward"
+    elif prec != H.PREC_NATIVE:
+        why = "bf16x3 operands"
+    elif a_frag is None or len(grads) != 1:
+        why = "A is not exchanged fragment-major with one backward (or x needs a gradient)"
+    elif _through_reshapes(grads[0].inputs[8]) is not _through_reshapes(plan._gll_post[g.id][1]):
+        why = "the gradient reaching f is not the head's fbar alone"
+    elif cell is not None:
+        why = "the forward may ride in the factorisation's launch (settings.runtime.early_forward)"
+    elif not H.sgp_fwd_bwd_supported(x, z, u, prec, True, eps_in is None and mode == 1, rng):
+        why = "not supported, or not the faster form, for these extents (hb_sgp_fwd_bwd_supported)"
+    if grads or head is not None:
+        plan.note(fb, node, why is None, why or "")
+    if why is None:
+        kbar_frag = plan.scratch((a_frag.numel(),))
+        bws = plan.scratch((H.sgp_fwd_bwd_ws_elems(x, z, u),))
+        plan._sgp_fused_bwd[grads[0].id] = (a_frag, kbar_frag, bws)
+        step = lambda: H.sgp_fwd_bwd(x, z, ell, W, u, eps_in=eps_in, rng=rng, mode=mode, out=outs, wfrag=wfrag, a_frag=a_frag,
+                                     skip_a=skip_a, head=head, kbar_frag=kbar_frag, ws=bws)
     if cell is not None and cell["rider"] is None:
         if not H.sgp_rider_supported(x, z, u, prec, wfrag is not None, eps_in is None and mode == 1, rng):
             plan.note(ep, node, False, "needs the fused finishing pass (fp32, one latent function, d <= 2, M % 64 == 0)")
@@ -1713,6 +1744,11 @@
     wfrag, bf3 = plan._wfrag.get(_through_stop_gradient(node.inputs[3]), (None, False))
     bf3 = bf3 and not need_x and node.inputs[0].shape[-1] <= 4 and node.inputs[4].shape[-2] <= 4
     prec = H.PREC_BF16X3 if bf3 else H.PREC_NATIVE
+    fused = plan._sgp_fused_bwd.get(node.id)
+    if fused is not None:
+        a_frag, kbar_frag, bws = fused
+        plan.steps.append(lambda: H.sgp_bwd_rest(x, z, ell, u, a_frag, kbar_frag, bws, out=(Lb, ub, zb, lb)))
+        return
     a_frag, fprec = plan._afrag.get(node.inputs[6], (None, None))
     if a_frag is not None:
         prec = fprec
@@ -2213,6 +2249,7 @@
         self._fused_trinv = set()
         self._wfrag: Dict[Tensor, object] = {}
         self._afrag: Dict[Tensor, object] = {}
+        self._sgp_fused_bwd: Dict[int, tuple] = {}
         self._fused_matutil = set()
         self._fused_concat = set()
         self._lazy_cols: Dict[Tensor, object] = {}
diff --git a/henbun_amd/hip_ops.py b/henbun_amd/hip_ops.py
--- a/henbun_amd/hip_ops.py
+++ b/henbun_amd/hip_ops.py
@@ -916,6 +916,41 @@
     return f, A, v, eps
 
 
+def sgp_fwd_bwd_supported(x, z, u, prec, has_wfrag, draw, rng):
+    E, n, M, d, P, _ = _sgp_dims(x, z, u)
+    if x.dtype != torch.float32:
+        return False
+    return bool(_lib.lib().raw("hb_sgp_fwd_bwd_supported")(E, n, M, d, P, int(prec), int(bool(has_wfrag)), int(bool(draw)),
+                                                           rng.nlanes if rng is not None else 0))
+
+
+def sgp_fwd_bwd_ws_elems(x, z, u):
+    E, n, M, d, P, _ = _sgp_dims(x, z, u)
+    return int(_lib.lib().raw("hb_sgp_fwd_bwd_ws_elems")(E, n, M, d, P))
+
+
+def sgp_fwd_bwd(x, z, ell, W, u, eps_in=None, rng=None, mode=SGP_DIAGONAL, out=None, wfrag=None, a_frag=None, skip_a=False,
+                head=None, kbar_frag=None, ws=None):
+    for t in (x, z, ell, W, u):
+        _chk(t)
+    E, n, M, d, P, sx = _sgp_dims(x, z, u)
+    f, A, v, eps = out
+    rp, rl = _rng_args(rng)
+    _lib.lib().call("hb_sgp_fwd_bwd_gauss_f32", KERN_RBF, mode, _p(x), sx, _p(z), _p(ell), ell.numel() // E, _p(W), _p(wfrag),
+                    int(PREC_NATIVE), _p(u), _p(eps_in), rp, rl, _p(eps), None if skip_a else _p(A), _p(a_frag), _p(f), _p(v),
+                    E, n, M, d, P, _p(ws), _p(head["y"]), _p(head.get("scale")), _p(head["var"]), float(head.get("post") or 0.0),
+                    _p(head["dmu"]), _p(head["fbar"]), _p(head["part"]), int(head["units"]), _p(kbar_frag), stream())
+    return f, A, v, eps
+
+
+def sgp_bwd_rest(x, z, ell, u, a_frag, kbar_frag, ws, out):
+    E, n, M, d, P, _ = _sgp_dims(x, z, u)
+    Lbar, ubar, zbar, ellbar = out
+    _lib.lib().call("hb_sgp_bwd_rest_f32", E, n, M, d, ell.numel() // E, P, int(PREC_NATIVE), _p(a_frag), _p(kbar_frag), _p(Lbar),
+                    _p(ubar), _p(zbar), _p(ellbar), _p(ws), stream())
+    return Lbar, ubar, zbar, ellbar
+
+
 def sgp_A(x, z, ell, W, out=None, wfrag=None, prec=PREC_NATIVE):
     E = z.shape[0] if z.dim() == 3 else 1
     M, d = z.shape[-2], z.shape[-1]
diff --git a/include/henbun_hip.h b/include/henbun_hip.h
--- a/include/henbun_hip.h
+++ b/include/henbun_hip.h
@@ -249,6 +249,17 @@
                          long E, long n, long M, long d, long P, float* ws, const float* y, const float* scale,
                          const float* var, double post, float* dmu, float* fbar, float* head_part, long units,
                          void* stream);
+int hb_sgp_fwd_bwd_supported(long E, long n, long M, long d, long P, int prec, int has_wfrag, int draw, long rng_lanes);
+long hb_sgp_fwd_bwd_ws_elems(long E, long n, long M, long d, long P);
+int hb_sgp_fwd_bwd_gauss_f32(int kind, int mode, const float* x, long sx, const float* z, const float* ell, long dl,
+                             const float* W, const float* Wfrag, int prec, const float* u, const float* eps_in,
+                             uint64_t* rng, long rng_lanes, float* eps_out, float* A, float* A_frag, float* f, float* v,
+                             long E, long n, long M, long d, long P, float* ws, const float* y, const float* scale,
+                             const float* var, double post, float* dmu, float* fbar, float* head_part, long units,
+                             float* Kbar_frag, void* stream);
+int hb_sgp_bwd_rest_f32(long E, long n, long M, long d, long dl, long P, int prec, const float* A_frag,
+                        const float* Kbar_frag, float* Lbar, float* ubar, float* zbar, float* ellbar, float* ws,
+                        void* stream);
 int hb_sgp_rider_supported(long E, long n, long M, long d, long P, int prec, int has_wfrag, int draw, long rng_lanes);
 int hb_sgp_rider_begin(void);
 int hb_sgp_rider_pending(void);
```

After: 41.83 million samples/s, median of 6. 1.4% higher.
